# Fanchuana/OPUS-PLLM

Hardware: AMD Instinct MI355X
Metric: proteins_per_sec (higher is better)
Workload: dtype f16; 1 GPU; OPUS-PLLM-llama3_8b shape: batch 64/GPU, 512-residue proteins, 89-id prompt (+8 protein tokens = 96 positions), 32 new tokens, greedy (BASELINE configs[3] per-GPU shard: batch 512 over 8 GPUs); batch_per_gpu=64, residues=512, parallelism=replicas x1 (batch-sharded), all-gather of ids

## Files before the change

### include/opus_pllm.h

```cpp
#ifndef OPUS_PLLM_H
#define OPUS_PLLM_H

#include <stdint.h>

#ifdef __cplusplus
extern "C" {
#endif

#define OPUS_ABI_VERSION 10

enum opus_status {
    OPUS_OK = 0,
    OPUS_EBADARG = -1,
    OPUS_ESHAPE = -2,
    OPUS_EHIP = -3,
    OPUS_ERCCL = -4,
    OPUS_EUNSUPPORTED = -5,
    OPUS_ESTATE = -6
};

enum opus_dtype { OPUS_F16 = 0, OPUS_F32 = 1, OPUS_I32 = 2, OPUS_I64 = 3, OPUS_U8 = 4 };

typedef struct opus_config {
    int32_t enc_layers, enc_dim, enc_heads, enc_ffn, enc_vocab;
// ... 87 lines not shown
int opus_generate_greedy(opus_ctx *ctx, const void *d_embeds, const uint8_t *d_mask, int32_t B, int32_t T,
                         int32_t max_new, const int32_t *eos_ids, int32_t n_eos, int32_t pad_id,
                         int32_t *d_out_ids, int32_t *n_out, void *stream);

int opus_set_stop_sequence(opus_ctx *ctx, const int32_t *ids, int32_t n);

int opus_generate_sample(opus_ctx *ctx, const void *d_embeds, const uint8_t *d_mask, int32_t B, int32_t T,
                         int32_t max_new, const int32_t *eos_ids, int32_t n_eos, int32_t pad_id, float temperature,
                         float top_p, uint64_t seed, int32_t *d_out_ids, int32_t *n_out, void *stream);
int opus_debug_sample(opus_ctx *ctx, const float *d_logits, int32_t B, float temperature, float top_p, uint64_t seed,
                      int32_t step, int32_t *d_tokens, void *stream);

int opus_generate_scored(opus_ctx *ctx, const void *d_embeds, const uint8_t *d_mask, int32_t B, int32_t T, int32_t max_new,
                         const int32_t *eos_ids, int32_t n_eos, int32_t pad_id, float temperature, float top_p, uint64_t seed,
                         int32_t *d_out_ids, int32_t *n_out, float *d_token_logprobs, float *d_scores, float *d_logits,
                         void *stream);
int opus_debug_argmax_lse(opus_ctx *ctx, const float *d_logits, int32_t B, int32_t V, int32_t *d_idx, float *d_lse, void *stream);

int opus_set_logits_processors(opus_ctx *ctx, float repetition_penalty, int32_t no_repeat_ngram_size, int32_t min_new_tokens,
                               const int32_t *bad_ids, const int32_t *bad_offsets, int32_t n_bad);
int opus_debug_logits_process(opus_ctx *ctx, float *d_logits, int32_t B, int32_t V, const int32_t *d_hist, int32_t hist_stride,
                              int32_t hist_len, const int32_t *eos_ids, int32_t n_eos, float repetition_penalty,
                              int32_t no_repeat_ngram_size, int32_t min_new_tokens, const int32_t *bad_ids,
                              const int32_t *bad_offsets, int32_t n_bad, void *stream);

int opus_set_token_constraint(opus_ctx *ctx, int32_t n_states, const int32_t *edge_off, const int32_t *edge_tok,
                              const int32_t *edge_next, int32_t n_edges, const uint8_t *completing, const int32_t *end_ids,
                              int32_t n_end, const int32_t *start, int32_t n_start, void *stream);
int opus_debug_token_constraint(opus_ctx *ctx, float *d_logits, int32_t B, int32_t V, const int32_t *d_hist, int32_t hist_stride,
                                int32_t hist_len, int32_t *d_state_out, void *stream);

int opus_debug_gemm(opus_ctx *ctx, const void *d_A, const void *d_W, const float *d_bias, const float *d_residual,
                    void *d_C, int32_t M, int32_t N, int32_t K, int32_t epi, int32_t out_f32, void *stream);
int opus_debug_gemm_norm(opus_ctx *ctx, const float *d_A, const void *d_W, void *d_C, int32_t M, int32_t N, int32_t K,
                         int32_t epi, int32_t out_f32, float eps, void *stream);
int opus_debug_gemm_slabs(opus_ctx *ctx, const void *d_A, const void *d_W, float *d_slabs, int32_t M, int32_t N, int32_t K,
                          int32_t *ks, void *stream);
int opus_debug_knob(opus_ctx *ctx, const char *name, int32_t value);
int opus_debug_gemm_rowscale(opus_ctx *ctx, const void *d_A, const void *d_W1, float *d_X, const void *d_W2, void *d_C,
                             int32_t M, int32_t N1, int32_t K1, int32_t N2, int32_t epi, float eps, int32_t *fused,
                             void *stream);
int opus_debug_gemm_rope(opus_ctx *ctx, const void *d_A, const void *d_W, const float *d_bias, void *d_out, int32_t M,
                         int32_t D, int32_t K, int32_t T, int32_t heads, int32_t allow_fuse, int32_t *fused, void *stream);
int opus_debug_gemm_ln(opus_ctx *ctx, const void *d_A, const void *d_W1, const float *d_b1, float *d_X, float *d_part, void *d_xh,
                       float *d_stat, const void *d_W2, const float *d_c2, const float *d_colsum, void *d_C, int32_t M, int32_t N1,
                       int32_t K1, int32_t N2, int32_t epi, int32_t rms, float eps, int32_t rope_T, const int32_t *d_rope_pos,
                       int32_t *produced, int32_t *plan, void *stream);
int opus_debug_attention(opus_ctx *ctx, const void *d_Q, const void *d_K, const void *d_V, void *d_O,
                         const int32_t *d_kstart, const int32_t *d_kend, int32_t B, int32_t T, int32_t heads,
                         int32_t group, int32_t head_dim, int32_t causal, float scale, void *stream);

int opus_debug_attn_decode(opus_ctx *ctx, const void *d_qkv, const void *d_k_hist, const void *d_v_hist, const int32_t *d_kstart,
                           int32_t B, int32_t T0, int32_t step, void *d_out, void *d_k_new, void *d_v_new, void *stream);

int opus_check_error(opus_ctx *ctx, void *stream);

int opus_beam_topk(opus_ctx *ctx, const float *d_run_scores, int32_t B, int32_t K, int32_t M, float *d_scores, int32_t *d_idx,
                   void *stream);
int opus_kv_reorder(opus_ctx *ctx, const int32_t *d_src_rows, int32_t R, void *stream);
int opus_beam_sample_topk(opus_ctx *ctx, const float *d_logits, const float *d_run_scores, int32_t B, int32_t K, int32_t M,
                          float temperature, float top_p, uint64_t seed, int32_t step, float *d_scores, int32_t *d_idx, void *stream);
int opus_set_sampling_top_k(opus_ctx *ctx, int32_t k);

int opus_last_logits(opus_ctx *ctx, float *d_out, int32_t B, void *stream);

int64_t opus_stat(opus_ctx *ctx, const char *name);

int opus_timing_enable(opus_ctx *ctx, int32_t on);
int opus_timing_reset(opus_ctx *ctx);
int opus_timing_get(opus_ctx *ctx, const char *kernel_class, const char *phase, double *ms, int64_t *launches, double *bytes,
                    double *flops);
int opus_timing_names(char *buf, int32_t cap);

#ifdef __cplusplus
}
#endif
#endif
```

### opus-pllm_amd/_cabi.py

```python
from __future__ import annotations

import ctypes as C
import os
from typing import Optional

from .config import OpusConfig

_HERE = os.path.dirname(os.path.abspath(__file__))
BF16 = os.environ.get("OPUS_DTYPE", "fp16").lower() in ("bf16", "bfloat16")
LIB_PATH = os.environ.get("OPUS_LIB_PATH") or os.path.join(_HERE, "lib", "libopus_pllm_bf16.so" if BF16 else "libopus_pllm.so")
ABI_VERSION = 10

OPUS_F16, OPUS_F32, OPUS_I32, OPUS_I64, OPUS_U8 = 0, 1, 2, 3, 4


def operand_dtype():
    import torch
    return torch.bfloat16 if BF16 else torch.float16


class OpusError(RuntimeError):
    def __init__(self, code: int, msg: str):
        super().__init__(f"libopus_pllm error {code}: {msg}")
        self.code = code
# ... 19 lines not shown


_P = C.c_void_p
SIGNATURES = {
    "opus_abi_version": (C.c_int, []),
    "opus_operand_dtype": (C.c_int, []),
    "opus_last_error": (C.c_char_p, []),
    "opus_workspace_bytes": (C.c_int64, [C.POINTER(CConfig)]),
    "opus_ctx_create": (C.c_int, [C.POINTER(CConfig), C.c_int, C.POINTER(_P)]),
    "opus_ctx_destroy": (C.c_int, [_P]),
    "opus_bind_weight": (C.c_int, [_P, C.c_char_p, _P, C.c_int, C.c_int, C.POINTER(C.c_int64)]),
    "opus_weights_ready": (C.c_int, [_P]),
    "opus_lora_merge": (C.c_int, [_P, _P, _P, C.c_float, C.c_int64, C.c_int64, C.c_int32, _P]),
    "opus_fill_synth": (C.c_int, [_P, C.c_int, C.c_int64, C.c_int64, C.c_uint64, C.c_float, C.c_float,
                                  C.c_int64, C.c_int64, C.c_int64, C.c_int32, C.c_uint64, C.c_float, C.c_float, _P]),
    "opus_tile_weight": (C.c_int, [_P, _P, C.c_int64, C.c_int64, _P]),
    "opus_esm2_encode": (C.c_int, [_P, _P, _P, C.c_int32, C.c_int32, _P, _P]),
    "opus_esm2_encode_packed": (C.c_int, [_P, _P, C.POINTER(C.c_int32), C.c_int32, _P, _P]),
    "opus_esm2_last_hidden": (C.c_int, [_P, _P, C.c_int32, C.c_int32, _P]),
    "opus_projector_forward": (C.c_int, [_P, _P, C.c_int32, _P, _P, _P]),
    "opus_protein_projector": (C.c_int, [_P, _P, C.c_int32, _P, _P]),
    "opus_switch_projector": (C.c_int, [_P, _P, C.c_int32, _P, _P]),
    "opus_splice_pad": (C.c_int, [_P, _P, _P, C.c_int32, C.c_int32, _P, C.c_int32, C.c_int32, C.c_int32,
                                  _P, _P, _P, C.POINTER(C.c_int32), _P]),
    "opus_llama_prefill": (C.c_int, [_P, _P, _P, C.c_int32, C.c_int32, _P, _P]),
    "opus_llama_decode_step": (C.c_int, [_P, _P, _P, _P]),
    "opus_generate_greedy": (C.c_int, [_P, _P, _P, C.c_int32, C.c_int32, C.c_int32, C.POINTER(C.c_int32),
                                       C.c_int32, C.c_int32, _P, C.POINTER(C.c_int32), _P]),
    "opus_debug_gemm": (C.c_int, [_P, _P, _P, _P, _P, _P, C.c_int32, C.c_int32, C.c_int32, C.c_int32, C.c_int32, _P]),
    "opus_debug_gemm_norm": (C.c_int, [_P, _P, _P, _P, C.c_int32, C.c_int32, C.c_int32, C.c_int32, C.c_int32, C.c_float, _P]),
    "opus_debug_gemm_rope": (C.c_int, [_P, _P, _P, _P, _P, C.c_int32, C.c_int32, C.c_int32, C.c_int32, C.c_int32, C.c_int32, _P, _P]),
    "opus_debug_attention": (C.c_int, [_P, _P, _P, _P, _P, _P, _P, C.c_int32, C.c_int32, C.c_int32, C.c_int32,
                                       C.c_int32, C.c_int32, C.c_float, _P]),
    "opus_generate_sample": (C.c_int, [_P, _P, _P, C.c_int32, C.c_int32, C.c_int32, C.POINTER(C.c_int32), C.c_int32, C.c_int32,
                                       C.c_float, C.c_float, C.c_uint64, _P, C.POINTER(C.c_int32), _P]),
    "opus_debug_sample": (C.c_int, [_P, _P, C.c_int32, C.c_float, C.c_float, C.c_uint64, C.c_int32, _P, _P]),
    "opus_timing_enable": (C.c_int, [_P, C.c_int32]),
    "opus_timing_reset": (C.c_int, [_P]),
    "opus_timing_get": (C.c_int, [_P, C.c_char_p, C.c_char_p, C.POINTER(C.c_double), C.POINTER(C.c_int64),
                                  C.POINTER(C.c_double), C.POINTER(C.c_double)]),
    "opus_timing_names": (C.c_int, [C.c_char_p, C.c_int32]),
    "opus_last_logits": (C.c_int, [_P, _P, C.c_int32, _P]),
    "opus_check_error": (C.c_int, [_P, _P]),
    "opus_beam_topk": (C.c_int, [_P, _P, C.c_int32, C.c_int32, C.c_int32, _P, _P, _P]),
    "opus_kv_reorder": (C.c_int, [_P, _P, C.c_int32, _P]),
    "opus_beam_sample_topk": (C.c_int, [_P, _P, _P, C.c_int32, C.c_int32, C.c_int32, C.c_float, C.c_float, C.c_uint64, C.c_int32,
                                        _P, _P, _P]),
    "opus_set_sampling_top_k": (C.c_int, [_P, C.c_int32]),
    "opus_set_stop_sequence": (C.c_int, [_P, C.POINTER(C.c_int32), C.c_int32]),
    "opus_debug_gemm_slabs": (C.c_int, [_P, _P, _P, _P, C.c_int32, C.c_int32, C.c_int32, C.POINTER(C.c_int32), _P]),
    "opus_debug_knob": (C.c_int, [_P, C.c_char_p, C.c_int32]),
    "opus_stat": (C.c_int64, [_P, C.c_char_p]),
    "opus_debug_attn_decode": (C.c_int, [_P, _P, _P, _P, _P, C.c_int32, C.c_int32, C.c_int32, _P, _P, _P, _P]),
    "opus_llama_forward": (C.c_int, [_P, _P, _P, C.c_int32, C.c_int32, _P, C.c_int32, _P, _P, _P, _P, C.c_int64, _P]),
    "opus_llama_forward_scratch_bytes": (C.c_int64, [C.POINTER(CConfig), C.c_int32, C.c_int32]),
    "opus_llama_prefix": (C.c_int, [_P, _P, _P, C.c_int32, C.c_int32, _P, _P, C.POINTER(C.c_int64), _P]),
    "opus_llama_score_continuations": (C.c_int, [_P, _P, C.c_int32, C.c_int32, _P, _P, _P, C.c_int32, C.c_int64, _P, _P, _P,
                                                 C.c_int64, _P]),
    "opus_llama_score_scratch_bytes": (C.c_int64, [C.POINTER(CConfig), C.c_int32, C.c_int32]),
    "opus_debug_attn_prefix": (C.c_int, [_P, _P, _P, _P, _P, C.c_int32, C.c_int32, C.c_int32, C.c_int32, _P, _P, _P]),
    "opus_llama_score_tree": (C.c_int, [_P, _P, C.c_int32, _P, _P, _P, C.c_int32, _P, C.c_int32, _P, _P, _P, C.c_int32, _P, _P, _P,
                                        C.c_int32, _P, C.c_int32, _P, _P, C.c_int32, C.c_int64, _P, _P, C.c_int64, _P, C.c_int64, _P]),
    "opus_llama_score_tree_scratch_bytes": (C.c_int64, [C.POINTER(CConfig), C.c_int32, C.c_int32, C.c_int32, C.c_int32, C.c_int32,
                                                        C.c_int32]),
    "opus_llama_dec_rows_cap": (C.c_int64, [C.POINTER(CConfig)]),
    "opus_llama_tree_max_depth": (C.c_int32, []),
    "opus_trie_path_sums": (C.c_int, [_P, _P, _P, _P, _P, _P, C.c_int32, C.c_int32, C.c_int32, _P, _P]),
    "opus_debug_attn_tree": (C.c_int, [_P, _P, _P, _P, _P, C.c_int32, C.c_int32, C.c_int32, _P, _P, _P, _P, _P]),
    "opus_debug_xent": (C.c_int, [_P, _P, C.c_int32, C.c_int32, _P, _P, _P, _P]),
    "opus_esm2_contacts_packed": (C.c_int, [_P, _P, C.POINTER(C.c_int32), C.c_int32, _P, _P, _P, C.c_int64, _P]),
    "opus_esm2_contacts_scratch_bytes": (C.c_int64, [C.POINTER(CConfig), C.POINTER(C.c_int32), C.c_int32]),
    "opus_debug_contacts": (C.c_int, [_P, _P, _P, C.c_int64, C.POINTER(C.c_int32), C.c_int32, C.c_int32, C.c_int32, _P, _P, _P, _P,
                                      _P, C.c_int64, _P]),
    "opus_generate_scored": (C.c_int, [_P, _P, _P, C.c_int32, C.c_int32, C.c_int32, C.POINTER(C.c_int32), C.c_int32, C.c_int32,
                                       C.c_float, C.c_float, C.c_uint64, _P, C.POINTER(C.c_int32), _P, _P, _P, _P]),
    "opus_debug_argmax_lse": (C.c_int, [_P, _P, C.c_int32, C.c_int32, _P, _P, _P]),
    "opus_set_logits_processors": (C.c_int, [_P, C.c_float, C.c_int32, C.c_int32, C.POINTER(C.c_int32), C.POINTER(C.c_int32),
                                             C.c_int32]),
    "opus_debug_logits_process": (C.c_int, [_P, _P, C.c_int32, C.c_int32, _P, C.c_int32, C.c_int32, C.POINTER(C.c_int32), C.c_int32,
                                            C.c_float, C.c_int32, C.c_int32, C.POINTER(C.c_int32), C.POINTER(C.c_int32), C.c_int32,
                                            _P]),
    "opus_set_token_constraint": (C.c_int, [_P, C.c_int32, _P, _P, _P, C.c_int32, _P, _P, C.c_int32, _P, C.c_int32, _P]),
    "opus_debug_token_constraint": (C.c_int, [_P, _P, C.c_int32, C.c_int32, _P, C.c_int32, C.c_int32, _P, _P]),
    "opus_debug_gemm_rowscale": (C.c_int, [_P, _P, _P, _P, _P, _P, C.c_int32, C.c_int32, C.c_int32, C.c_int32, C.c_int32,
                                           C.c_float, C.POINTER(C.c_int32), _P]),
    "opus_debug_gemm_ln": (C.c_int, [_P, _P, _P, _P, _P, _P, _P, _P, _P, _P, _P, _P, C.c_int32, C.c_int32, C.c_int32, C.c_int32,
                                     C.c_int32, C.c_int32, C.c_float, C.c_int32, _P, C.POINTER(C.c_int32), C.POINTER(C.c_int32), _P]),
}

_lib: Optional[C.CDLL] = None


def lib() -> C.CDLL:
    global _lib
    if _lib is not None:
        return _lib
    if not os.path.exists(LIB_PATH):
        raise OpusError(-100, f"{LIB_PATH} not found: build it with `python opus-pllm_amd/build.py` "
                              "(hipcc --offload-arch=gfx950); this package has no CPU fallback")
    l = C.CDLL(LIB_PATH)
    for name, (res, args) in SIGNATURES.items():
        fn = getattr(l, name)
        fn.restype = res
        fn.argtypes = args
    v = l.opus_abi_version()
    if v != ABI_VERSION:
# ... 11 lines not shown
```

### opus-pllm_amd/csrc/api.cpp

```cpp
#include "../../include/opus_pllm.h"
#include "common.h"

#include <cmath>
#include <cstdarg>
#include <cstdio>
#include <cstdlib>
#include <cstring>
#include <algorithm>
#include <atomic>
#include <map>
#include <string>
#include <vector>

using namespace opus;

static thread_local char g_err[512] = "";
static int fail(int code, const char *fmt, ...) {
    va_list ap;
    va_start(ap, fmt);
    vsnprintf(g_err, sizeof(g_err), fmt, ap);
    va_end(ap);
    return code;
}
#define HIPC(expr)                                                                                   \
// ... 32 lines not shown
};

struct opus_ctx {
    opus_config cfg;
    int device = 0;
    std::map<std::string, Tensor> w;
    bool resolved = false;
    const half_t *enc_emb = nullptr, *dec_emb = nullptr, *lm_head = nullptr, *proj_w = nullptr, *dec_pos = nullptr;
    const float *enc_lnfw = nullptr, *enc_lnfb = nullptr, *proj_b = nullptr, *dec_lnfw = nullptr, *dec_lnfb = nullptr;
    std::vector<EncLayer> enc;
    std::vector<DecLayer> dec;
    std::vector<const half_t *> sw_w;
    std::vector<const float *> sw_b;
    char *ws = nullptr;
    size_t ws_bytes = 0;
    float *e_x, *e_hid, *p_pool_dummy, *e_part, *e_stat;
    int32_t *e_cu, *e_pos;
    std::vector<int32_t> h_cu;
    half_t *e_xn, *e_qkv, *e_ctx, *e_h1;
    half_t *p_xn, *p_y, *p_z[2];
    float *d_x, *d_xl, *d_logits, *d_pval, *gemm_ws, *d_probs, *d_zpart, *d_spart, *d_part, *d_stat;
    int32_t *d_cand_i, *d_cand_n;
    uint64_t *d_seed;
    int32_t *d_chosen;
    float samp_temp = 0.f, samp_top_p = 1.f;
    int samp_top_k = 0;
    float *d_bthr = nullptr, *d_blse = nullptr;
    int64_t gemm_ws_bytes = 0;
    half_t *d_xn, *d_qkv, *d_ctx, *d_act, *d_xln, *kc, *vc;
    float *cs_enc, *cs_dec, *cs_row;
    int32_t *d_kstart, *d_step, *d_next, *d_fin, *d_nunf, *d_eos, *d_plan, *d_pidx, *d_stop, *d_cnt;
    int n_stop = 0;
    static constexpr int POLL_RING = 4, POLL_LAG = 2;
    int32_t *h_nunf = nullptr;
    hipEvent_t poll_ev[POLL_RING] = {nullptr, nullptr, nullptr, nullptr};
    int64_t cache_sl, cache_sb, cache_sh;
    int cur_B = 0, cur_T = 0;
    bool prefilled = false;
    struct GraphEntry {
        hipGraphExec_t exec = nullptr;
        int B = -1, maxnew = -1, pad = 0, neos = -1;
        const int32_t *out = nullptr;
        float temp = 0.f, top_p = 1.f;
        int outs = 0;
        bool lproc = false;
        bool cons = false;
        uint64_t used = 0;
    };
    static constexpr int MAX_GRAPHS = 4;
    std::vector<GraphEntry> graphs;
    uint64_t graph_clock = 0;
    int64_t graph_instantiations = 0;
    int64_t graph_replays = 0;
    int64_t decode_steps = 0;
    char *gen_mem = nullptr;
    GenOutDesc *d_gen = nullptr;
    GenOutDesc h_gen{};
    float *d_gpsum = nullptr, *d_gthr = nullptr;
    int gen_outs = 0;
    bool lproc_on = false;
    LogitsProcDesc h_lproc{1.0f, 0, 0, 0, {}, {}};
    char *lproc_mem = nullptr;
    LogitsProcDesc *d_lproc = nullptr;
    int32_t *d_lstep = nullptr, *d_ridx = nullptr;
    GenOutDesc *d_gen_raw = nullptr, *d_gen_proc = nullptr;
    float *d_rlse = nullptr, *d_rawh = nullptr;
    bool cons_on = false;
    char *cons_tab = nullptr, *cons_mem = nullptr;
    size_t cons_tab_bytes = 0;
    TokenConstraintDesc *d_cons = nullptr;
    int32_t *d_cstate = nullptr, *d_cstep = nullptr;
    int32_t cons_n_start = 0, cons_max_id = -1;
    half_t *rq_xh = nullptr;
    int rq_done = 0;
    const float *rq_rope_cs = nullptr;
    const int32_t *rq_rope_pos = nullptr;
    int rq_rope_T = 0, rq_rope_cols = 0, rq_rope_qcols = 0, rq_rope_done = 0;
    float rq_rope_qscale = 1.0f;
    int rq_force_wide = 0, rq_slab_only = 0, rq_ks = 1;
    int rq_a_tiled = 0, rq_xh_tiled = 0, rq_c_tiled = 0;
    float *rq_ln_part = nullptr;
    half_t *rq_ln_xh = nullptr;
    int rq_ln_done = 0;
    const float *rq_ln_stat = nullptr, *rq_ln_colsum = nullptr;
    int *rq_pp_plan = nullptr;
    bool xln_tiled = false;
    const float *xh_src = nullptr;
    bool use_row_scale = false;
    float *d_ssq = nullptr;
    int64_t ssq_cap = 0;
    int ssq_nblk = 0;
    float row_eps = 0.f;
    bool timing = false;
    int phase = PH_OTHER;
    std::vector<TimeRec> recs;
    int proj_rows = 0;
    char *proj_big = nullptr;
    half_t *kv_tmp = nullptr;
    int64_t epoch = 0;
    std::vector<int32_t> h_kstart;
};

static std::atomic<int64_t> g_epoch{0};
static void new_epoch(opus_ctx *c) { c->epoch = ++g_epoch; }

struct ContRows {
    const int32_t *nkst;
    AttnPrefixParams attn;
    int nblocks;
};

static size_t align_up(size_t v) { return (v + 255) & ~(size_t)255; }

struct Carver {
    char *base;
    size_t off = 0;
    template <class T>
    T *take(size_t n) {
        T *p = base ? reinterpret_cast<T *>(base + off) : nullptr;
        off += align_up(n * sizeof(T));
        return p;
    }
};

static void carve(opus_ctx *c, char *base, size_t *total) {
    const opus_config &g = c->cfg;
    Carver k{base};
    const size_t Me = (size_t)g.max_batch * g.max_enc_tokens;
    const size_t De = g.enc_dim, Fe = g.enc_ffn;
    c->e_x = k.take<float>(Me * De);
    c->e_hid = k.take<float>(Me * De);
    c->e_xn = k.take<half_t>(Me * De);
    c->e_qkv = k.take<half_t>(Me * 3 * De);
    c->e_ctx = k.take<half_t>(Me * De);
    c->e_h1 = k.take<half_t>(Me * Fe);
    c->e_part = k.take<float>(Me * (De / 64 + 1) * 2);
    c->e_stat = k.take<float>(Me * 2);
    c->e_cu = k.take<int32_t>((size_t)g.max_batch + 4);
    c->e_pos = k.take<int32_t>(Me);
    const size_t B = g.max_batch, H = g.dec_dim, SW = (size_t)g.dec_dim * g.n_prot_tokens;
    const size_t PR = B;
    c->proj_rows = (int)PR;
    c->p_xn = k.take<half_t>(PR * De);
    c->p_y = k.take<half_t>(PR * (size_t)(g.has_protein_projector ? g.proj_dim : g.enc_dim));
    c->p_z[0] = k.take<half_t>(PR * SW);
    c->p_z[1] = k.take<half_t>(PR * SW);
    const size_t B16 = (B + 15) & ~(size_t)15;
    const size_t Md = B * g.max_prompt > B16 ? B * g.max_prompt : B16;
    const size_t QKV = (size_t)(g.dec_heads + 2 * g.dec_kv_heads) * g.dec_head_dim;
    const size_t QD = (size_t)g.dec_heads * g.dec_head_dim;
    c->d_x = k.take<float>(Md * H);
    c->d_xn = k.take<half_t>(Md * H);
    c->d_qkv = k.take<half_t>(Md * QKV);
    c->d_ctx = k.take<half_t>(Md * QD);
    c->d_act = k.take<half_t>(Md * g.dec_ffn);
    c->d_part = k.take<float>(Md * (H / 64 + 1) * 2);
    c->d_stat = k.take<float>(Md * 2);
// ... 270 lines not shown

struct Timed {
    opus_ctx *c;
    hipStream_t s;
    int klass;
    double bytes, flops;
    LaunchEvents ev;
    hipEvent_t b0 = nullptr, b1 = nullptr;
    Timed(opus_ctx *c_, hipStream_t s_, int k, double b, double f = 0.0) : c(c_), s(s_), klass(k), bytes(b), flops(f) {
        if (c->timing) {
            (void)hipEventCreate(&ev.main0); (void)hipEventCreate(&ev.main1);
            (void)hipEventCreate(&ev.aux0); (void)hipEventCreate(&ev.aux1);
            (void)hipEventCreate(&b0); (void)hipEventCreate(&b1);
            (void)hipEventRecord(b0, s);
            tl_launch_ev = &ev;
        }
    }
    ~Timed() {
        if (!c->timing) return;
        tl_launch_ev = nullptr;
        if (ev.main_used) {
            c->recs.push_back(TimeRec{ev.main_class >= 0 ? ev.main_class : klass, c->phase, ev.main0, ev.main1, bytes, flops});
            (void)hipEventDestroy(b0); (void)hipEventDestroy(b1);
        } else {
            (void)hipEventRecord(b1, s);
            c->recs.push_back(TimeRec{klass, c->phase, b0, b1, bytes, flops});
            (void)hipEventDestroy(ev.main0); (void)hipEventDestroy(ev.main1);
        }
        if (ev.aux_used) c->recs.push_back(TimeRec{KC_REDUCE, c->phase, ev.aux0, ev.aux1, ev.aux_bytes, 0.0});
        else { (void)hipEventDestroy(ev.aux0); (void)hipEventDestroy(ev.aux1); }
    }
};

static int gemm_any(opus_ctx *c, hipStream_t s, const half_t *A, const float *Af, float eps, int64_t lda, const half_t *W,
                    int M, int N, int K, const float *bias, int epi, const float *residual, void *C, int64_t ldc,
                    int out_f32) {
    GemmParams p;
    p.A = A; p.Af = Af; p.norm_eps = eps; p.lda = lda; p.W = W; p.M = M; p.N = N; p.K = K; p.bias = bias;
    p.residual = residual; p.ldr = ldc; p.C = C; p.ldc = ldc; p.out_f32 = out_f32; p.epi = epi;
    p.ws = c->gemm_ws; p.ws_bytes = c->gemm_ws_bytes;
    p.xh_out = c->rq_xh; p.ssq_out = c->d_ssq; p.fused_done = &c->rq_done; p.ssq_cap = c->ssq_cap; p.nblk_out = &c->ssq_nblk;
    c->rq_done = 0;
    c->rq_xh = nullptr;
    p.rope_cs = c->rq_rope_cs; p.rope_T = c->rq_rope_T; p.rope_cols = c->rq_rope_cols; p.rope_qcols = c->rq_rope_qcols;
    p.rope_qscale = c->rq_rope_qscale; p.rope_done = &c->rq_rope_done; p.rope_pos = c->rq_rope_pos;
    c->rq_rope_done = 0;
    c->rq_rope_cs = nullptr;
    c->rq_rope_pos = nullptr;
    p.row_ssq = nullptr; p.row_nblk = 0;
    if (c->use_row_scale) { p.row_ssq = c->d_ssq; p.row_nblk = c->ssq_nblk; p.norm_eps = c->row_eps; c->use_row_scale = false; }
    c->rq_ks = 1;
    p.force_wide = c->rq_force_wide; p.slab_only = c->rq_slab_only; p.ks_out = &c->rq_ks;
    c->rq_force_wide = c->rq_slab_only = 0;
    c->rq_ln_done = 0;
    if (c->rq_ln_part) { p.xh_out = c->rq_ln_xh; p.ssq_out = nullptr; p.ln_part = c->rq_ln_part; p.ln_done = &c->rq_ln_done; c->rq_ln_part = nullptr; }
    if (c->rq_ln_stat) { p.ln_stat = c->rq_ln_stat; p.ln_colsum = c->rq_ln_colsum; c->rq_ln_stat = c->rq_ln_colsum = nullptr; }
    p.combine_cnt = c->d_cnt;
    p.pp_plan = c->rq_pp_plan;
    c->rq_pp_plan = nullptr;
    p.a_tiled = c->rq_a_tiled; p.xh_tiled = c->rq_xh_tiled; p.c_tiled = c->rq_c_tiled;
    c->rq_a_tiled = c->rq_xh_tiled = c->rq_c_tiled = 0;
    const int nout = epi == EPI_SILU_GU16 ? N / 2 : N;
    const double bytes = 2.0 * N * K + (Af ? 4.0 : 2.0) * M * K + (double)M * nout * (out_f32 ? 4 : 2) +
                         (residual ? 4.0 * M * nout : 0.0);
    int klass = M <= SKINNY_MAX_M ? KC_SKINNY : KC_TILE;
    hipError_t e;
    {
        Timed t(c, s, klass, bytes, 2.0 * M * N * (double)K);
        e = launch_gemm(p, s, &klass);
    }
    if (e != hipSuccess) return fail(OPUS_EHIP, "gemm M=%d N=%d K=%d failed: %s", M, N, K, hipGetErrorString(e));
    return OPUS_OK;
}
static int gemm(opus_ctx *c, hipStream_t s, const half_t *A, int64_t lda, const half_t *W, int M, int N, int K,
                const float *bias, int epi, const float *residual, void *C, int64_t ldc, int out_f32) {
    return gemm_any(c, s, A, nullptr, 0.f, lda, W, M, N, K, bias, epi, residual, C, ldc, out_f32);
}
static bool fuse_rows() {
    static const bool off = getenv("OPUS_NO_ROW_FUSION") != nullptr;
    return !off;
}
#define KLF(klass, bytes, flops, call)                                                                \
    do {                                                                                              \
        hipError_t e_;                                                                                \
        {                                                                                             \
            Timed t_(c, s, klass, bytes, flops);                                                      \
            e_ = (call);                                                                              \
        }                                                                                             \
        if (e_ != hipSuccess) return fail(OPUS_EHIP, "%s failed: %s", #call, hipGetErrorString(e_)); \
    } while (0)
#define KL(klass, bytes, call) KLF(klass, bytes, 0.0, call)

static int gemm_norm(opus_ctx *c, hipStream_t s, const float *X, float eps, half_t *scratch, const half_t *W, int M, int N,
                     int K, int epi, void *C, int64_t ldc, int out_f32, const float *bias = nullptr) {
    static const bool no_mid = getenv("OPUS_NO_MID_GEMM") != nullptr;
    static const bool mid_v1 = getenv("OPUS_MID_V1") != nullptr;
    if (c->xh_src == X && bias == nullptr && (K & 255) == 0 && gemm_goes_wide(M, N)) {
        c->xh_src = nullptr;
        c->use_row_scale = true;
        c->row_eps = eps;
        return gemm(c, s, scratch, K, W, M, N, K, nullptr, epi, nullptr, C, ldc, out_f32);
    }
    c->xh_src = nullptr;
    const bool wide = M > SKINNY_MAX_M && N >= 16384 && !mid_v1;
    if (M <= SKINNY_MAX_M || (M <= MID_MAX_M && !no_mid && !wide))
        return gemm_any(c, s, nullptr, X, eps, K, W, M, N, K, bias, epi, nullptr, C, ldc, out_f32);
    KL(KC_NORM, 6.0 * M * K, launch_rmsnorm(X, nullptr, eps, M, K, scratch, s));
    return gemm(c, s, scratch, K, W, M, N, K, bias, epi, nullptr, C, ldc, out_f32);
}

static int need_ready(opus_ctx *c) {
    if (!c) return fail(OPUS_EBADARG, "ctx is null");
    OPC(opus_weights_ready(c));
    HIPC(hipSetDevice(c->device));
    return OPUS_OK;
}

extern "C" int opus_lora_merge(void *W, const void *A, const void *B, float scale, int64_t out_f, int64_t in_f,
                               int32_t r, void *stream) {
    if (!W || !A || !B || out_f < 1 || in_f < 1 || r < 1) return fail(OPUS_EBADARG, "lora_merge: bad argument");
    if (in_f % 8) return fail(OPUS_ESHAPE, "lora_merge: in_features must be a multiple of 8");
    HIPC(launch_lora_merge((half_t *)W, (const half_t *)A, (const half_t *)B, scale, out_f, in_f, r, (hipStream_t)stream));
    return OPUS_OK;
}

extern "C" int opus_fill_synth(void *dst, int dtype, int64_t rows, int64_t cols, uint64_t seed, float std, float mean,
                               int64_t row_block, int64_t row_stride, int64_t row_off, int32_t tiled, uint64_t fold_seed,
                               float fold_std, float fold_mean, void *stream) {
    if (!dst || rows < 1 || cols < 1 || (dtype != OPUS_F16 && dtype != OPUS_F32) || row_block < 1 || row_stride < row_block)
        return fail(OPUS_EBADARG, "fill_synth: bad argument");
    if (tiled && (cols % 64 || row_block % 16 || row_stride % 16 || row_off % 16))
        return fail(OPUS_ESHAPE, "fill_synth: tiled layout needs cols %% 64 == 0 and 16-row aligned blocks");
    HIPC(launch_fill_synth(dst, dtype, rows, cols, seed, std, mean, row_block, row_stride, row_off, tiled ? 1 : 0,
                           fold_seed, fold_std, fold_mean, (hipStream_t)stream));
    return OPUS_OK;
}

extern "C" int opus_tile_weight(const void *d_src, void *d_dst, int64_t N, int64_t K, void *stream) {
    if (!d_src || !d_dst || d_src == d_dst) return fail(OPUS_EBADARG, "tile_weight: null or aliased pointers");
    if (N < 16 || K < 64 || N % 16 || K % 64) return fail(OPUS_ESHAPE, "tile_weight: N %% 16 == 0 and K %% 64 == 0 required");
    HIPC(launch_tile_weight((const half_t *)d_src, (half_t *)d_dst, N, K, (hipStream_t)stream));
    return OPUS_OK;
}

struct ContactRun {
    const float *w, *bias;
    float *A, *vec, *part, *sw, *out;
    int n_max;
};

static int contact_layer(opus_ctx *c, hipStream_t s, const ContactRun &ct, int l, int B) {
    const opus_config &g = c->cfg;
    const int D = g.enc_dim, nh = g.enc_heads, hd = D / nh, C = g.enc_layers * nh;
    ContactParams p;
    p.Q = c->e_qkv; p.K = c->e_qkv + D; p.ld = 3 * D; p.cu = c->e_cu; p.B = B; p.heads = nh; p.w = ct.w + l * nh;
    p.A = ct.A; p.accumulate = l > 0; p.rows = ct.vec; p.vld = C; p.c0 = l * nh; p.part = ct.part;
    double n2 = 0.0, nt = 0.0;
    for (int b = 0; b < B; ++b) {
        const double n = c->h_cu[b + 1] - c->h_cu[b] - 2, t = n + 2;
        if (n > 0) { n2 += n * n; nt += n * t; }
    }
    KLF(KC_CONTACT, 8.0 * n2 + 4.0 * (c->h_cu[B]) * D, 2.0 * 2.0 * nt * hd * nh, launch_esm_contact_accum(p, hd, ct.n_max, s));
    KL(KC_CONTACT, 4.0 * n2 / 64.0 * nh * 2.0, launch_esm_contact_colsum(ct.part, c->e_cu, B, nh, ct.n_max, ct.vec, C, l * nh, 1, s));
    return OPUS_OK;
}

static int esm2_encode_rows(opus_ctx *c, hipStream_t s, const int32_t *d_tokens, const int32_t *d_lens, const int32_t *d_cu, int B, int T,
                            int M, float *d_pooled, const ContactRun *ct = nullptr) {
    const opus_config &g = c->cfg;
    c->phase = PH_ENCODE;
    const int D = g.enc_dim, F = g.enc_ffn, nh = g.enc_heads, hd = D / nh;
    const bool packed = d_cu != nullptr;
    HIPC(hipMemsetAsync(c->d_cnt, 0, HANDOFF_ERR * sizeof(int32_t), s));
    if (packed) KL(KC_OTHER, 4.0 * M * D, launch_esm_embed_packed(d_tokens, c->enc_emb, d_cu, B, T, D, c->e_x, c->e_pos, s));
    else KL(KC_OTHER, 4.0 * M * D, launch_esm_embed(d_tokens, c->enc_emb, B, T, D, c->e_x, s));
    static const bool no_ln_env = getenv("OPUS_NO_LN_FUSION") != nullptr;
    const bool no_ln_fusion = no_ln_env || g_knobs.no_ln_fusion;
    const bool qkv_pp = !no_ln_fusion && (D & 255) == 0 && gemm_goes_pp(M, 3 * D);
    const bool fc1_pp = !no_ln_fusion && (D & 255) == 0 && gemm_goes_pp(M, F);
    bool have_stat = false;
    auto finalize = [&]() -> int {
        KL(KC_NORM, 8.0 * M * (D / 64) + 8.0 * M, launch_ln_finalize(c->e_part, M, D / 64, D, g.enc_ln_eps, 0, c->e_stat, s));
        return OPUS_OK;
    };
    double attn_flops = 0.0;
    if (packed) for (int b = 0; b < B; ++b) { const double t = c->h_cu[b + 1] - c->h_cu[b]; attn_flops += 4.0 * t * t * D; }
    else attn_flops = 4.0 * B * (double)T * T * D;
    for (int l = 0; l < g.enc_layers; ++l) {
        const EncLayer &L = c->enc[l];
        if (have_stat && qkv_pp) { c->rq_ln_stat = c->e_stat; c->rq_ln_colsum = L.sqkv; }
        else KL(KC_NORM, 6.0 * M * D, launch_layernorm(c->e_x, nullptr, nullptr, g.enc_ln_eps, M, D, c->e_xn, nullptr, s));
        if (hd == 64) {
            c->rq_rope_cs = c->cs_enc; c->rq_rope_T = packed ? g.max_enc_tokens : T; c->rq_rope_cols = 2 * D; c->rq_rope_qcols = D;
            c->rq_rope_qscale = 1.0f / sqrtf((float)hd);
            c->rq_rope_pos = packed ? c->e_pos : nullptr;
        }
        OPC(gemm(c, s, c->e_xn, D, L.wqkv, M, 3 * D, D, L.bqkv, EPI_NONE, nullptr, c->e_qkv, 3 * D, 0));
        if (!c->rq_rope_done) {
            if (packed) KL(KC_OTHER, 8.0 * M * D, launch_esm_rope(c->e_qkv, c->cs_enc, 1, M, nh, hd, 1.0f / sqrtf((float)hd), s, c->e_pos));
            else KL(KC_OTHER, 8.0 * M * D, launch_esm_rope(c->e_qkv, c->cs_enc, B, T, nh, hd, 1.0f / sqrtf((float)hd), s));
        }
        if (ct) OPC(contact_layer(c, s, *ct, l, B));
        AttnParams a;
        a.Q = c->e_qkv; a.K = c->e_qkv + D; a.V = c->e_qkv + 2 * D;
        a.q_sb = a.k_sb = a.v_sb = packed ? 0 : (int64_t)T * 3 * D;
        a.q_st = a.k_st = a.v_st = 3 * D;
        a.O = c->e_ctx; a.o_sb = packed ? 0 : (int64_t)T * D; a.o_st = D;
        a.kstart = nullptr; a.kend = packed ? nullptr : d_lens; a.cu = d_cu;
        a.B = B; a.T = T; a.heads = nh; a.group = 1; a.head_dim = hd; a.causal = 0; a.scale = 1.0f;
        a.q_trim = packed && l + 1 == g.enc_layers && T > 2 && !g_knobs.enc_full_last_layer ? 1 : 0;
        KLF(KC_ATTN_PREFILL, 8.0 * M * D, attn_flops, launch_attn_prefill(a, s));
        if (fc1_pp) { c->rq_ln_part = c->e_part; c->rq_ln_xh = c->e_xn; }
        OPC(gemm(c, s, c->e_ctx, D, L.wo, M, D, D, L.bo, EPI_NONE, c->e_x, c->e_x, D, 1));
        have_stat = c->rq_ln_done != 0;
        if (have_stat) { OPC(finalize()); c->rq_ln_stat = c->e_stat; c->rq_ln_colsum = L.s1; }
        else KL(KC_NORM, 6.0 * M * D, launch_layernorm(c->e_x, nullptr, nullptr, g.enc_ln_eps, M, D, c->e_xn, nullptr, s));
        OPC(gemm(c, s, c->e_xn, D, L.w1, M, F, D, L.b1, EPI_GELU, nullptr, c->e_h1, F, 0));
        if (qkv_pp && l + 1 < g.enc_layers) { c->rq_ln_part = c->e_part; c->rq_ln_xh = c->e_xn; }
        OPC(gemm(c, s, c->e_h1, F, L.w2, M, D, F, L.b2, EPI_NONE, c->e_x, c->e_x, D, 1));
        have_stat = c->rq_ln_done != 0;
        if (have_stat) OPC(finalize());
    }
    KL(KC_NORM, 8.0 * M * D, launch_layernorm(c->e_x, c->enc_lnfw, c->enc_lnfb, g.enc_ln_eps, M, D, nullptr, c->e_hid, s));
    if (packed) KL(KC_OTHER, 4.0 * M * D, launch_masked_mean_packed(c->e_hid, d_cu, B, D, d_pooled, s));
    else KL(KC_OTHER, 4.0 * M * D, launch_masked_mean(c->e_hid, d_lens, B, T, D, d_pooled, s));
    if (ct) {
        const int C = g.enc_layers * nh;
        double n2 = 0.0, ni = 0.0;
        for (int b = 0; b < B; ++b) { const double n = c->h_cu[b + 1] - c->h_cu[b] - 2; n2 += n * n; ni += n; }
        KL(KC_CONTACT, 4.0 * ni * C, launch_esm_contact_scale(ct->vec, d_cu, B, C, ct->w, ct->sw, s));
        KLF(KC_CONTACT, 12.0 * n2 + 8.0 * ni * C * cdiv((int64_t)ct->n_max, 64), 2.0 * n2 * C,
            launch_esm_contact_finish(ct->A, ct->vec, ct->sw, d_cu, B, C, ct->n_max, ct->bias, ct->out, s));
    }
    return OPUS_OK;
}

extern "C" int opus_esm2_encode(opus_ctx *c, const int32_t *d_tokens, const int32_t *d_lens, int32_t B, int32_t T,
                                float *d_pooled, void *stream) {
    OPC(need_ready(c));
    if (!d_tokens || !d_lens || !d_pooled) return fail(OPUS_EBADARG, "esm2_encode: null pointer");
    const opus_config &g = c->cfg;
    if (B < 1 || B > g.max_batch || T < 3 || T > g.max_enc_tokens)
        return fail(OPUS_ESHAPE, "esm2_encode: B=%d T=%d exceed capacity (%d, %d)", B, T, g.max_batch, g.max_enc_tokens);
    return esm2_encode_rows(c, (hipStream_t)stream, d_tokens, d_lens, nullptr, B, T, B * T, d_pooled);
}

extern "C" int opus_esm2_encode_packed(opus_ctx *c, const int32_t *d_tokens, const int32_t *h_cu, int32_t B, float *d_pooled,
                                       void *stream) {
    OPC(need_ready(c));
    if (!d_tokens || !h_cu || !d_pooled) return fail(OPUS_EBADARG, "esm2_encode_packed: null pointer");
    const opus_config &g = c->cfg;
    if (B < 1 || B > g.max_batch) return fail(OPUS_ESHAPE, "esm2_encode_packed: B=%d exceeds max_batch=%d", B, g.max_batch);
    if (h_cu[0] != 0) return fail(OPUS_EBADARG, "esm2_encode_packed: cu[0] must be 0");
    int Tmax = 0;
    for (int b = 0; b < B; ++b) {
        const int t = h_cu[b + 1] - h_cu[b];
        if (t < 2 || t > g.max_enc_tokens)
            return fail(OPUS_ESHAPE, "esm2_encode_packed: protein %d has %d tokens (2 .. max_enc_tokens=%d)", b, t, g.max_enc_tokens);
        Tmax = t > Tmax ? t : Tmax;
    }
    const int64_t M = h_cu[B];
    if (M > (int64_t)g.max_batch * g.max_enc_tokens) return fail(OPUS_ESHAPE, "esm2_encode_packed: %lld tokens exceed the workspace", (long long)M);
    hipStream_t s = (hipStream_t)stream;
    c->h_cu.assign(h_cu, h_cu + B + 1);
    HIPC(launch_upload_i32(h_cu, B + 1, c->e_cu, s));
    return esm2_encode_rows(c, s, d_tokens, nullptr, c->e_cu, B, Tmax, (int)M, d_pooled);
}

struct ContactScratch {
    int64_t a, vec, part, sw, total;
    int n_max;
};
static ContactScratch contact_scratch(const opus_config &g, const int32_t *h_cu, int B) {
    ContactScratch z{};
// ... 65 lines not shown
    if (contact_accum_lds(heads) > 160 * 1024) return fail(OPUS_ESHAPE, "debug_contacts: %d heads exceed the workgroup's LDS", heads);
    if (h_cu[0] != 0) return fail(OPUS_EBADARG, "debug_contacts: cu[0] must be 0");
    int64_t pq = 0;
    int n_max = 0;
    for (int b = 0; b < B; ++b) {
        const int t = h_cu[b + 1] - h_cu[b];
        if (t < 2) return fail(OPUS_ESHAPE, "debug_contacts: protein %d has %d tokens (at least 2)", b, t);
        pq += (int64_t)(t - 2 + 63) / 64 * (t - 2);
        n_max = std::max(n_max, t - 2);
    }
    const int64_t need = (int64_t)align_up((size_t)(B + 1) * 4) + pq * heads * 4;
    if (scratch_bytes < need) return fail(OPUS_ESHAPE, "debug_contacts: scratch of %lld bytes, %lld needed", (long long)scratch_bytes, (long long)need);
    HIPC(hipSetDevice(c->device));
    hipStream_t s = (hipStream_t)stream;
    int32_t *d_cu = (int32_t *)d_scratch;
    float *part = (float *)((char *)d_scratch + align_up((size_t)(B + 1) * 4));
    HIPC(launch_upload_i32(h_cu, B + 1, d_cu, s));
    ContactParams p;
    p.Q = (const half_t *)d_q; p.K = (const half_t *)d_k; p.ld = ld; p.cu = d_cu; p.B = B; p.heads = heads; p.w = d_w;
    p.A = d_A; p.accumulate = 0; p.rows = d_rows; p.vld = heads; p.c0 = 0; p.part = part;
    HIPC(launch_esm_contact_accum(p, head_dim, n_max, s));
    HIPC(launch_esm_contact_colsum(part, d_cu, B, heads, n_max, d_cols, heads, 0, 0, s));
    return OPUS_OK;
}

extern "C" int opus_esm2_last_hidden(opus_ctx *c, float *d_out, int32_t B, int32_t T, void *stream) {
    if (!c || !d_out) return fail(OPUS_EBADARG, "null pointer");
    if (B < 1 || T < 1 || (int64_t)B * T > (int64_t)c->cfg.max_batch * c->cfg.max_enc_tokens) return fail(OPUS_ESHAPE, "B/T out of range");
    HIPC(hipMemcpyAsync(d_out, c->e_hid, (size_t)B * T * c->cfg.enc_dim * sizeof(float), hipMemcpyDeviceToDevice,
                        (hipStream_t)stream));
    return OPUS_OK;
}

constexpr int BIG_PROJ_ROWS = 4096;
static int ensure_proj_rows(opus_ctx *c, int B) {
    if (B <= c->proj_rows || c->proj_big) return OPUS_OK;
    const opus_config &g = c->cfg;
    const size_t PR = BIG_PROJ_ROWS > g.max_batch ? BIG_PROJ_ROWS : g.max_batch;
    const size_t De = g.enc_dim, Dm = g.has_protein_projector ? g.proj_dim : g.enc_dim, SW = (size_t)g.dec_dim * g.n_prot_tokens;
    const size_t bytes = (align_up(PR * De * 2) + align_up(PR * Dm * 2) + 2 * align_up(PR * SW * 2));
    HIPC(hipMalloc((void **)&c->proj_big, bytes));
    Carver k{c->proj_big};
    c->p_xn = k.take<half_t>(PR * De);
    c->p_y = k.take<half_t>(PR * Dm);
    c->p_z[0] = k.take<half_t>(PR * SW);
    c->p_z[1] = k.take<half_t>(PR * SW);
    c->proj_rows = (int)PR;
    return OPUS_OK;
}

static int protein_projector_rows(opus_ctx *c, hipStream_t s, const float *d_pooled, int B, half_t *d_out) {
    const opus_config &g = c->cfg;
    const int De = g.enc_dim;
    HIPC(hipMemsetAsync(c->d_cnt, 0, HANDOFF_ERR * sizeof(int32_t), s));
    if (!g.has_protein_projector) {
        KL(KC_OTHER, 6.0 * B * De, launch_f2h(d_pooled, (int64_t)B * De, d_out, s));
        return OPUS_OK;
    }
    KL(KC_NORM, 6.0 * B * De, launch_l2norm(d_pooled, B, De, c->p_xn, s));
    return gemm(c, s, c->p_xn, De, c->proj_w, B, g.proj_dim, De, c->proj_b, EPI_NONE, nullptr, d_out, g.proj_dim, 0);
}

static int switch_projector_rows(opus_ctx *c, hipStream_t s, const half_t *in, int B, half_t *d_out) {
    const opus_config &g = c->cfg;
    const int SW = g.dec_dim * g.n_prot_tokens;
    int din = g.has_protein_projector ? g.proj_dim : g.enc_dim;
    for (int i = 0; i < g.switch_depth; ++i) {
        const bool last = i + 1 == g.switch_depth;
        half_t *o = last ? d_out : c->p_z[i & 1];
        OPC(gemm(c, s, in, din, c->sw_w[i], B, SW, din, c->sw_b[i], last ? EPI_NONE : EPI_GELU, nullptr, o, SW, 0));
        in = o;
        din = SW;
    }
    return OPUS_OK;
}

extern "C" int opus_protein_projector(opus_ctx *c, const float *d_pooled, int32_t B, void *d_out, void *stream) {
    OPC(need_ready(c));
    if (!d_pooled || !d_out) return fail(OPUS_EBADARG, "protein_projector: null pointer");
    if (B < 1) return fail(OPUS_ESHAPE, "protein_projector: B=%d", B);
    const opus_config &g = c->cfg;
    const int64_t din = g.enc_dim, dout = g.has_protein_projector ? g.proj_dim : g.enc_dim;
    c->phase = PH_PROJECT;
    OPC(ensure_proj_rows(c, B));
    for (int r0 = 0; r0 < B; r0 += c->proj_rows) {
        const int n = B - r0 < c->proj_rows ? B - r0 : c->proj_rows;
        OPC(protein_projector_rows(c, (hipStream_t)stream, d_pooled + r0 * din, n, (half_t *)d_out + r0 * dout));
    }
    return OPUS_OK;
}

extern "C" int opus_switch_projector(opus_ctx *c, const void *d_in, int32_t B, void *d_out, void *stream) {
    OPC(need_ready(c));
    if (!d_in || !d_out) return fail(OPUS_EBADARG, "switch_projector: null pointer");
    if (B < 1) return fail(OPUS_ESHAPE, "switch_projector: B=%d", B);
    const opus_config &g = c->cfg;
    const int64_t din = g.has_protein_projector ? g.proj_dim : g.enc_dim, SW = (int64_t)g.dec_dim * g.n_prot_tokens;
    c->phase = PH_PROJECT;
    OPC(ensure_proj_rows(c, B));
    for (int r0 = 0; r0 < B; r0 += c->proj_rows) {
        const int n = B - r0 < c->proj_rows ? B - r0 : c->proj_rows;
        OPC(switch_projector_rows(c, (hipStream_t)stream, (const half_t *)d_in + r0 * din, n, (half_t *)d_out + r0 * SW));
    }
    return OPUS_OK;
}

extern "C" int opus_projector_forward(opus_ctx *c, const float *d_pooled, int32_t B, void *d_out, void *d_proj_out,
// ... 82 lines not shown
        4.0 * M * (double)QD * (a.Tp + a.n), a.par ? launch_attn_tree(a, cr.nblocks, s) : launch_attn_prefix(a, cr.nblocks, s));
    return OPUS_OK;
}

static int opt_layer(opus_ctx *c, hipStream_t s, const DecLayer &L, int l, float *x, half_t *xn, int M, int B, int T, bool decode,
                     const ContRows *cont = nullptr) {
    const opus_config &g = c->cfg;
    const int H = g.dec_dim, F = g.dec_ffn, nh = g.dec_heads, nkv = g.dec_kv_heads, hd = g.dec_head_dim;
    const int QKV = (nh + 2 * nkv) * hd, QD = nh * hd;
    KL(KC_NORM, 6.0 * M * H, launch_layernorm(x, L.ln1w, L.ln1b, g.dec_rms_eps, M, H, xn, nullptr, s));
    OPC(gemm(c, s, xn, H, L.wqkv, M, QKV, H, L.bqkv, EPI_NONE, nullptr, c->d_qkv, QKV, 0));
    if (decode) {
        OPC(attn_decode(c, s, l, B, T));
    } else if (cont) {
        KL(KC_OTHER, 4.0 * M * QKV, launch_dec_rope_cache(c->d_qkv, c->cs_dec, cont->nkst, B, T, nh, nkv, hd, nullptr, nullptr, 0, 0, s));
        OPC(attn_prefix(c, s, *cont, l, M));
    } else {
        KL(KC_OTHER, 4.0 * M * QKV,
           launch_dec_rope_cache(c->d_qkv, c->cs_dec, c->d_kstart, B, T, nh, nkv, hd, c->kc + l * c->cache_sl,
                                 c->vc + l * c->cache_sl, c->cache_sb, c->cache_sh, s));
        AttnParams a;
        a.Q = c->d_qkv; a.K = c->d_qkv + QD; a.V = c->d_qkv + QD + nkv * hd;
        a.q_sb = a.k_sb = a.v_sb = (int64_t)T * QKV;
        a.q_st = a.k_st = a.v_st = QKV;
        a.O = c->d_ctx; a.o_sb = (int64_t)T * QD; a.o_st = QD;
        a.kstart = c->d_kstart; a.kend = nullptr;
        a.B = B; a.T = T; a.heads = nh; a.group = nh / nkv; a.head_dim = hd; a.causal = 1;
        a.scale = 1.0f / sqrtf((float)hd);
        KLF(KC_ATTN_PREFILL, 2.0 * M * (QKV + QD), 2.0 * B * (double)T * T * QD, launch_attn_prefill(a, s));
    }
    OPC(gemm(c, s, c->d_ctx, QD, L.wo, M, H, QD, L.bo, EPI_NONE, x, x, H, 1));
    KL(KC_NORM, 6.0 * M * H, launch_layernorm(x, L.ln2w, L.ln2b, g.dec_rms_eps, M, H, xn, nullptr, s));
    if (g.dec_act == 0) {
        OPC(gemm(c, s, xn, H, L.w1, M, F, H, L.b1, EPI_GELU, nullptr, c->d_act, F, 0));
    } else {
        OPC(gemm(c, s, xn, H, L.w1, M, F, H, L.b1, EPI_NONE, nullptr, c->d_act, F, 0));
        KL(KC_OTHER, 4.0 * M * F, launch_relu_h(c->d_act, (int64_t)M * F, s));
    }
    OPC(gemm(c, s, c->d_act, F, L.w2, M, H, F, L.b2, EPI_NONE, x, x, H, 1));
    return OPUS_OK;
}

static int lm_head_opt(opus_ctx *c, hipStream_t s, int B) {
    const opus_config &g = c->cfg;
    KL(KC_NORM, 6.0 * B * g.dec_dim, launch_layernorm(c->d_xl, c->dec_lnfw, c->dec_lnfb, g.dec_rms_eps, B, g.dec_dim, c->d_xln, nullptr, s));
    return gemm(c, s, c->d_xln, g.dec_dim, c->lm_head, B, g.dec_vocab, g.dec_dim, nullptr, EPI_NONE, nullptr, c->d_logits,
                g.dec_vocab, 1);
}

static int prefill_opt(opus_ctx *c, hipStream_t s, const half_t *embeds, const uint8_t *mask, int B, int T, bool all_rows,
                       const ContRows *cont) {
    const opus_config &g = c->cfg;
    const int H = g.dec_dim, M = B * T;
    HIPC(hipMemsetAsync(c->d_cnt, 0, HANDOFF_ERR * sizeof(int32_t), s));
    if (!cont) KL(KC_OTHER, 1.0 * M, launch_mask_to_kstart(mask, B, T, c->d_kstart, s));
    KL(KC_OTHER, 6.0 * M * H, launch_h2f(embeds, c->d_x, (int64_t)M * H, s));
    KL(KC_OTHER, 10.0 * M * H, launch_add_pos(c->d_x, c->dec_pos, cont ? cont->nkst : c->d_kstart, nullptr, 0, B, T, H, g.dec_max_pos + 1, s));
    for (int l = 0; l < g.dec_layers; ++l) OPC(opt_layer(c, s, c->dec[l], l, c->d_x, c->d_xn, M, B, T, false, cont));
    if (all_rows) return OPUS_OK;
    KL(KC_OTHER, 8.0 * B * H, launch_take_last(c->d_x, B, T, H, c->d_xl, s));
    OPC(lm_head_opt(c, s, B));
    OPC(reset_step(c, s, T));
    c->cur_B = B;
    c->cur_T = T;
    c->prefilled = true;
    return OPUS_OK;
}

static int decode_step_opt(opus_ctx *c, hipStream_t s) {
    const opus_config &g = c->cfg;
    const int B = c->cur_B, T = c->cur_T, H = g.dec_dim;
    KL(KC_OTHER, 10.0 * B * H, launch_add_pos(c->d_xl, c->dec_pos, c->d_kstart, c->d_step, -1, B, 1, H, g.dec_max_pos + 1, s));
    for (int l = 0; l < g.dec_layers; ++l) OPC(opt_layer(c, s, c->dec[l], l, c->d_xl, c->d_xln, B, B, T, true));
    OPC(lm_head_opt(c, s, B));
    KL(KC_OTHER, 8.0, launch_step_advance(c->d_step, s));
    return OPUS_OK;
}

static int prefill(opus_ctx *c, hipStream_t s, const half_t *embeds, const uint8_t *mask, int B, int T, bool all_rows = false,
                   const ContRows *cont = nullptr) {
    c->phase = cont ? PH_SCORE : PH_PREFILL;
    if (cont) {
        all_rows = true;
    } else {
        new_epoch(c);
        if (all_rows) {
            c->prefilled = false;
            c->cur_B = 0;
        }
    }
    if (c->cfg.dec_arch == 1) return prefill_opt(c, s, embeds, mask, B, T, all_rows, cont);
    const opus_config &g = c->cfg;
    const int H = g.dec_dim, F = g.dec_ffn, nh = g.dec_heads, nkv = g.dec_kv_heads, hd = g.dec_head_dim;
    const int QKV = (nh + 2 * nkv) * hd, QD = nh * hd;
    const int M = B * T;
    HIPC(hipMemsetAsync(c->d_cnt, 0, HANDOFF_ERR * sizeof(int32_t), s));
    if (!cont) KL(KC_OTHER, 1.0 * M, launch_mask_to_kstart(mask, B, T, c->d_kstart, s));
    KL(KC_OTHER, 6.0 * M * H, launch_h2f(embeds, c->d_x, (int64_t)M * H, s));
    static const bool no_ln_env = getenv("OPUS_NO_LN_FUSION") != nullptr;
    const bool no_ln_fusion = no_ln_env || g_knobs.no_ln_fusion;
    const bool qkv_pp = !no_ln_fusion && (H & 255) == 0 && (QKV & 255) == 0 && gemm_goes_pp(M, QKV);
    const bool gu_pp = !no_ln_fusion && (H & 255) == 0 && (F & 127) == 0 && gemm_goes_pp(M, 2 * F);
    bool have_stat = false, last_rows_done = false;
    auto finalize = [&]() -> int {
        KL(KC_NORM, 8.0 * M * (H / 64) + 8.0 * M, launch_ln_finalize(c->d_part, M, H / 64, H, g.dec_rms_eps, 1, c->d_stat, s));
        return OPUS_OK;
    };
    for (int l = 0; l < g.dec_layers; ++l) {
        const DecLayer &L = c->dec[l];
        if (have_stat && qkv_pp) {
            c->rq_ln_stat = c->d_stat;
            OPC(gemm(c, s, c->d_xn, H, L.wqkv, M, QKV, H, L.bqkv, EPI_NONE, nullptr, c->d_qkv, QKV, 0));
        } else {
            OPC(gemm_norm(c, s, c->d_x, g.dec_rms_eps, c->d_xn, L.wqkv, M, QKV, H, EPI_NONE, c->d_qkv, QKV, 0, L.bqkv));
        }
        if (cont) {
            KL(KC_OTHER, 4.0 * M * QKV, launch_dec_rope_cache(c->d_qkv, c->cs_dec, cont->nkst, B, T, nh, nkv, hd, nullptr, nullptr, 0, 0, s));
            OPC(attn_prefix(c, s, *cont, l, M));
        } else {
            KL(KC_OTHER, 4.0 * M * QKV,
               launch_dec_rope_cache(c->d_qkv, c->cs_dec, c->d_kstart, B, T, nh, nkv, hd, c->kc + l * c->cache_sl,
                                     c->vc + l * c->cache_sl, c->cache_sb, c->cache_sh, s));
            AttnParams a;
            a.Q = c->d_qkv; a.K = c->d_qkv + QD; a.V = c->d_qkv + QD + nkv * hd;
            a.q_sb = a.k_sb = a.v_sb = (int64_t)T * QKV;
            a.q_st = a.k_st = a.v_st = QKV;
            a.O = c->d_ctx; a.o_sb = (int64_t)T * QD; a.o_st = QD;
            a.kstart = c->d_kstart; a.kend = nullptr;
            a.B = B; a.T = T; a.heads = nh; a.group = nh / nkv; a.head_dim = hd; a.causal = 1;
            a.scale = 1.0f / sqrtf((float)hd);
            KLF(KC_ATTN_PREFILL, 2.0 * M * (QKV + QD), 2.0 * B * (double)T * T * QD, launch_attn_prefill(a, s));
        }
        if (l + 1 == g.dec_layers && T > 1 && !all_rows && !g_knobs.misc[7]) {
            half_t *ctx_last = c->d_qkv;
            KL(KC_OTHER, 4.0 * B * QD, launch_take_last(reinterpret_cast<const float *>(c->d_ctx), B, T, QD / 2, reinterpret_cast<float *>(ctx_last), s));
            KL(KC_OTHER, 8.0 * B * H, launch_take_last(c->d_x, B, T, H, c->d_xl, s));
            if (fuse_rows() && B <= 96) c->rq_xh = c->d_xln;
            OPC(gemm(c, s, ctx_last, QD, L.wo, B, H, QD, nullptr, EPI_NONE, c->d_xl, c->d_xl, H, 1));
            c->xh_src = c->rq_done ? c->d_xl : nullptr;
            OPC(gemm_norm(c, s, c->d_xl, g.dec_rms_eps, c->d_xln, L.wgu, B, 2 * F, H, EPI_SILU_GU16, c->d_act, F, 0));
            if (fuse_rows() && B <= 96) c->rq_xh = c->d_xln;
            OPC(gemm(c, s, c->d_act, F, L.wd, B, H, F, nullptr, EPI_NONE, c->d_xl, c->d_xl, H, 1));
            c->xh_src = c->rq_done ? c->d_xl : nullptr;
            c->xln_tiled = false;
            last_rows_done = true;
            break;
        }
        if (gu_pp) { c->rq_ln_part = c->d_part; c->rq_ln_xh = c->d_xn; }
        else if (fuse_rows() && M <= 96) c->rq_xh = c->d_xn;
        OPC(gemm(c, s, c->d_ctx, QD, L.wo, M, H, QD, nullptr, EPI_NONE, c->d_x, c->d_x, H, 1));
        c->xh_src = c->rq_done ? c->d_x : nullptr;
        have_stat = c->rq_ln_done != 0;
        if (have_stat) {
            OPC(finalize());
            c->rq_ln_stat = c->d_stat;
            OPC(gemm(c, s, c->d_xn, H, L.wgu, M, 2 * F, H, nullptr, EPI_SILU_GU16, nullptr, c->d_act, F, 0));
        } else {
            OPC(gemm_norm(c, s, c->d_x, g.dec_rms_eps, c->d_xn, L.wgu, M, 2 * F, H, EPI_SILU_GU16, c->d_act, F, 0));
        }
        if (qkv_pp && l + 1 < g.dec_layers) { c->rq_ln_part = c->d_part; c->rq_ln_xh = c->d_xn; }
        OPC(gemm(c, s, c->d_act, F, L.wd, M, H, F, nullptr, EPI_NONE, c->d_x, c->d_x, H, 1));
        have_stat = c->rq_ln_done != 0;
        if (have_stat) OPC(finalize());
    }
    if (all_rows) {
        c->xh_src = nullptr;
        return OPUS_OK;
    }
    if (!last_rows_done) {
        KL(KC_OTHER, 8.0 * B * H, launch_take_last(c->d_x, B, T, H, c->d_xl, s));
        c->xh_src = nullptr;
    }
    OPC(lm_head(c, s, B));
    OPC(reset_step(c, s, T));
    c->cur_B = B;
    c->cur_T = T;
    c->prefilled = true;
    return OPUS_OK;
}

static int decode_step(opus_ctx *c, hipStream_t s, const int32_t *d_tok) {
    c->phase = PH_DECODE;
    const opus_config &g = c->cfg;
    const int B = c->cur_B, T = c->cur_T;
    const int H = g.dec_dim, F = g.dec_ffn, nh = g.dec_heads, nkv = g.dec_kv_heads, hd = g.dec_head_dim;
    const int QKV = (nh + 2 * nkv) * hd, QD = nh * hd;
    const int ctx_cap = g.max_prompt + g.max_new_tokens;
    const bool rowscale = g.dec_arch == 0 && fuse_rows() && B > SKINNY_MAX_M && B <= MID_MAX_M && (H & 255) == 0;
    const bool qkv_tiled = rowscale && gemm_stream_would(B, QKV, H, 1, 1, 1, c->gemm_ws_bytes);
    const bool wo_tiled = rowscale && gemm_stream_would(B, H, QD, 0, 1, 0, c->gemm_ws_bytes);
    const bool down_tiled = rowscale && (F & 63) == 0 && gemm_stream_would(B, H, F, 0, 1, 0, c->gemm_ws_bytes);
    KL(KC_OTHER, 6.0 * B * H, launch_embed_tokens(d_tok, c->dec_emb, B, H, g.dec_vocab, c->d_xl, rowscale ? c->d_xln : nullptr,
                                                  rowscale ? c->d_ssq : nullptr, qkv_tiled ? 1 : 0, c->cs_dec, c->d_kstart, c->d_step, -1,
                                                  hd / 2, c->cs_row, c->d_cnt, HANDOFF_ERR, s));
    c->xln_tiled = qkv_tiled;
    c->xh_src = rowscale ? c->d_xl : nullptr;
    if (rowscale) c->ssq_nblk = H >> 8;
    if (g.dec_arch == 1) return decode_step_opt(c, s);
    for (int l = 0; l < g.dec_layers; ++l) {
        const DecLayer &L = c->dec[l];
        if (rowscale && c->xh_src == c->d_xl) {
            c->xh_src = nullptr;
            c->rq_force_wide = 1;
            c->rq_slab_only = 1;
            c->use_row_scale = true;
            c->row_eps = g.dec_rms_eps;
            c->rq_a_tiled = c->xln_tiled ? 1 : 0;
            OPC(gemm(c, s, c->d_xln, H, L.wqkv, B, QKV, H, L.bqkv, EPI_NONE, nullptr, c->d_qkv, QKV, 0));
            OPC(attn_decode(c, s, l, B, T, c->rq_ks > 1 ? c->rq_ks : 0, L.bqkv, wo_tiled ? 1 : 0));
        } else {
            OPC(gemm_norm(c, s, c->d_xl, g.dec_rms_eps, c->d_xln, L.wqkv, B, QKV, H, EPI_NONE, c->d_qkv, QKV, 0, L.bqkv));
            OPC(attn_decode(c, s, l, B, T, 0, nullptr, wo_tiled ? 1 : 0));
        }
        c->xln_tiled = false;
        if (fuse_rows() && B <= 96) c->rq_xh = c->d_xln;
        c->rq_a_tiled = wo_tiled ? 1 : 0;
// ... 1019 lines not shown
    if (M < 1 || D < 16 || K < 64 || K % 64 || T < 1 || heads < 1 || D % heads || M % T)
        return fail(OPUS_ESHAPE, "debug_gemm_rope: M %% T == 0, D %% heads == 0, K %% 64 == 0");
    const int hd = D / heads;
    if (hd != c->cfg.enc_dim / c->cfg.enc_heads || T > c->cfg.max_enc_tokens)
        return fail(OPUS_ESHAPE, "debug_gemm_rope: head_dim / T must match the context's encoder rotary table");
    HIPC(hipSetDevice(c->device));
    hipStream_t s = (hipStream_t)stream;
    const float qs = 1.0f / sqrtf((float)hd);
    if (allow_fuse && hd == 64) {
        c->rq_rope_cs = c->cs_enc; c->rq_rope_T = T; c->rq_rope_cols = 2 * D; c->rq_rope_qcols = D; c->rq_rope_qscale = qs;
    }
    OPC(gemm(c, s, (const half_t *)A, K, (const half_t *)W, M, 3 * D, K, bias, EPI_NONE, nullptr, out, 3 * D, 0));
    *fused = c->rq_rope_done;
    if (!c->rq_rope_done) HIPC(launch_esm_rope((half_t *)out, c->cs_enc, M / T, T, heads, hd, qs, s));
    return OPUS_OK;
}

extern "C" int opus_debug_gemm_rowscale(opus_ctx *c, const void *A, const void *W1, float *X, const void *W2, void *Cp, int32_t M,
                                        int32_t N1, int32_t K1, int32_t N2, int32_t epi, float eps, int32_t *fused, void *stream) {
    if (!c || !A || !W1 || !X || !W2 || !Cp || !fused) return fail(OPUS_EBADARG, "debug_gemm_rowscale: null pointer");
    if (M < 1 || N1 < 64 || N1 % 64 || K1 < 64 || K1 % 64 || N2 < 32) return fail(OPUS_ESHAPE, "debug_gemm_rowscale: shape");
    if (epi != EPI_NONE && epi != EPI_SILU_GU16) return fail(OPUS_EBADARG, "debug_gemm_rowscale: epilogue 0 or 2");
    const opus_config &g = c->cfg;
    if ((int64_t)M * N1 > (int64_t)g.max_batch * g.max_prompt * g.dec_dim) return fail(OPUS_ESHAPE, "debug_gemm_rowscale: M * N1 exceeds the scratch");
    HIPC(hipSetDevice(c->device));
    hipStream_t s = (hipStream_t)stream;
    if (fuse_rows() && M <= 96) c->rq_xh = c->d_xn;
    OPC(gemm(c, s, (const half_t *)A, K1, (const half_t *)W1, M, N1, K1, nullptr, EPI_NONE, X, X, N1, 1));
    c->xh_src = c->rq_done ? X : nullptr;
    *fused = c->xh_src != nullptr && (N1 & 255) == 0 && gemm_goes_wide(M, N2) ? 1 : 0;
    const int nout = epi == EPI_SILU_GU16 ? N2 / 2 : N2;
    return gemm_norm(c, s, X, eps, c->d_xn, (const half_t *)W2, M, N2, N1, epi, Cp, nout, 0);
}

extern "C" int opus_debug_gemm_ln(opus_ctx *c, const void *A, const void *W1, const float *b1, float *X, float *part, void *xh,
                                  float *stat, const void *W2, const float *c2, const float *colsum, void *Cp, int32_t M, int32_t N1,
                                  int32_t K1, int32_t N2, int32_t epi, int32_t rms, float eps, int32_t rope_T,
                                  const int32_t *rope_pos, int32_t *produced, int32_t *plan, void *stream) {
    if (!c || !A || !W1 || !X || !part || !xh || !stat || !W2 || !Cp || !produced || !plan)
        return fail(OPUS_EBADARG, "debug_gemm_ln: null pointer");
    if (M < 1 || N1 < 64 || N1 % 64 || K1 < 64 || K1 % 64 || N2 < 32) return fail(OPUS_ESHAPE, "debug_gemm_ln: shape");
    if (epi != EPI_NONE && epi != EPI_GELU && epi != EPI_SILU_GU16) return fail(OPUS_EBADARG, "debug_gemm_ln: epilogue 0, 1 or 2");
    if (epi == EPI_SILU_GU16 && (!rms || c2 || colsum || N2 % 32))
        return fail(OPUS_EBADARG, "debug_gemm_ln: the gate / up epilogue is the RMSNorm form (no bias, no column sums)");
    if (rms ? colsum != nullptr : colsum == nullptr) return fail(OPUS_EBADARG, "debug_gemm_ln: column sums go with LayerNorm only");
    if (rope_pos && rope_T < 1) return fail(OPUS_EBADARG, "debug_gemm_ln: rope_pos needs rope_T");
    if (rope_T > 0 && (epi != EPI_NONE || N2 % 3 || (N2 / 3) % 64 || c->cfg.enc_dim / c->cfg.enc_heads != 64 ||
                       rope_T > c->cfg.max_enc_tokens))
        return fail(OPUS_ESHAPE, "debug_gemm_ln: rotary needs EPI_NONE, N2 = 3 D, head_dim 64 and rope_T within the context's table");
    HIPC(hipSetDevice(c->device));
    hipStream_t s = (hipStream_t)stream;
    c->phase = PH_OTHER;
    for (int i = 0; i < 2 * PP_PLAN_WORDS; ++i) plan[i] = -1;
    HIPC(hipMemsetAsync(c->d_cnt, 0, HANDOFF_ERR * sizeof(int32_t), s));
    if (gemm_goes_pp(M, N1)) { c->rq_ln_part = part; c->rq_ln_xh = (half_t *)xh; }
    c->rq_pp_plan = plan;
    OPC(gemm(c, s, (const half_t *)A, K1, (const half_t *)W1, M, N1, K1, b1, EPI_NONE, X, X, N1, 1));
    *produced = c->rq_ln_done;
    if (!c->rq_ln_done) return OPUS_OK;
    KL(KC_NORM, 8.0 * M * (N1 / 64), launch_ln_finalize(part, M, N1 / 64, N1, eps, rms, stat, s));
    c->rq_ln_stat = stat; c->rq_ln_colsum = colsum;
    c->rq_pp_plan = plan + PP_PLAN_WORDS;
    if (rope_T > 0) {
        const int D = N2 / 3;
        c->rq_rope_cs = c->cs_enc; c->rq_rope_T = rope_T; c->rq_rope_cols = 2 * D; c->rq_rope_qcols = D;
        c->rq_rope_qscale = 0.125f;
        c->rq_rope_pos = rope_pos;
    }
    const int nout = epi == EPI_SILU_GU16 ? N2 / 2 : N2;
    OPC(gemm(c, s, (const half_t *)xh, N1, (const half_t *)W2, M, N2, N1, c2, epi, nullptr, Cp, nout, 0));
    if (rope_T > 0 && !c->rq_rope_done) return fail(OPUS_ESTATE, "debug_gemm_ln: the consumer GEMM did not fuse the rotary");
    return OPUS_OK;
}

extern "C" int opus_debug_gemm_slabs(opus_ctx *c, const void *A, const void *W, float *d_slabs, int32_t M, int32_t N, int32_t K,
                                     int32_t *ks, void *stream) {
    if (!c || !A || !W || !ks) return fail(OPUS_EBADARG, "debug_gemm_slabs: null pointer");
    if (M < 1 || N < 16 || K < 64 || K % 64) return fail(OPUS_ESHAPE, "debug_gemm_slabs: shape");
    const opus_config &g = c->cfg;
    const int64_t QKVd = (int64_t)(g.dec_heads + 2 * g.dec_kv_heads) * g.dec_head_dim;
    if ((int64_t)M * N > (int64_t)g.max_batch * g.max_prompt * QKVd) return fail(OPUS_ESHAPE, "debug_gemm_slabs: M * N exceeds the scratch");
    HIPC(hipSetDevice(c->device));
    hipStream_t s = (hipStream_t)stream;
    c->rq_force_wide = 1;
    c->rq_slab_only = 1;
    c->rq_a_tiled = g_knobs.debug_a_tiled;
    OPC(gemm(c, s, (const half_t *)A, K, (const half_t *)W, M, N, K, nullptr, EPI_NONE, nullptr, c->d_qkv, N, 0));
    *ks = c->rq_ks;
    if (c->rq_ks > 1 && d_slabs)
        HIPC(hipMemcpyAsync(d_slabs, c->gemm_ws, (size_t)c->rq_ks * M * N * sizeof(float), hipMemcpyDeviceToDevice, s));
    return OPUS_OK;
}

extern "C" int opus_beam_topk(opus_ctx *c, const float *d_run_scores, int32_t B, int32_t K, int32_t M, float *d_scores,
                              int32_t *d_idx, void *stream) {
    if (!c || !d_run_scores || !d_scores || !d_idx) return fail(OPUS_EBADARG, "beam_topk: null pointer");
    if (!c->prefilled) return fail(OPUS_ESTATE, "beam_topk before prefill");
    if (B < 1 || K < 1 || B * K != c->cur_B) return fail(OPUS_ESHAPE, "beam_topk: B=%d x K=%d rows, the last step had %d", B, K, c->cur_B);
    if (M < 1 || M > 16) return fail(OPUS_ESHAPE, "beam_topk: 1 <= M <= 16 candidates per row (got %d)", M);
    HIPC(hipSetDevice(c->device));
    hipStream_t s = (hipStream_t)stream;
    c->phase = PH_DECODE;
    KL(KC_OTHER, 12.0 * c->cur_B * c->cfg.dec_vocab,
       launch_beam_topk(c->d_logits, d_run_scores, B, K, c->cfg.dec_vocab, M, c->d_zpart, d_scores, d_idx, s));
    return OPUS_OK;
}

extern "C" int opus_beam_sample_topk(opus_ctx *c, const float *d_logits, const float *d_run_scores, int32_t B, int32_t K, int32_t M,
                                     float temperature, float top_p, uint64_t seed, int32_t step, float *d_scores, int32_t *d_idx,
                                     void *stream) {
    if (!c || !d_run_scores || !d_scores || !d_idx) return fail(OPUS_EBADARG, "beam_sample_topk: null pointer");
    if (!d_logits && !c->prefilled) return fail(OPUS_ESTATE, "beam_sample_topk before prefill");
    if (B < 1 || K < 1 || B * K > c->cfg.max_batch || (!d_logits && B * K != c->cur_B))
// ... 58 lines not shown
                                    int32_t group, int32_t hd, int32_t causal, float scale, void *stream) {
    if (!c || !Q || !K || !V || !O) return fail(OPUS_EBADARG, "debug_attention: null pointer");
    if (B < 1 || T < 1 || heads < 1 || group < 1 || heads % group) return fail(OPUS_ESHAPE, "debug_attention: shape");
    HIPC(hipSetDevice(c->device));
    hipStream_t s = (hipStream_t)stream;
    AttnParams a;
    const int kvh = heads / group;
    a.Q = (const half_t *)Q; a.K = (const half_t *)K; a.V = (const half_t *)V; a.O = (half_t *)O;
    a.q_st = (int64_t)heads * hd; a.q_sb = a.q_st * T;
    a.k_st = a.v_st = (int64_t)kvh * hd; a.k_sb = a.v_sb = a.k_st * T;
    a.o_st = a.q_st; a.o_sb = a.q_sb;
    a.kstart = kstart; a.kend = kend; a.B = B; a.T = T; a.heads = heads; a.group = group; a.head_dim = hd;
    a.causal = causal; a.scale = scale;
    KLF(KC_ATTN_PREFILL, 2.0 * B * T * hd * (2.0 * heads + 2.0 * kvh), (causal ? 2.0 : 4.0) * B * (double)T * T * heads * hd,
        launch_attn_prefill(a, s));
    return OPUS_OK;
}

extern "C" int opus_debug_attn_decode(opus_ctx *c, const void *d_qkv, const void *d_k_hist, const void *d_v_hist,
                                      const int32_t *d_kstart, int32_t B, int32_t T0, int32_t step, void *d_out, void *d_k_new,
                                      void *d_v_new, void *stream) {
    if (!c || !d_qkv || !d_kstart || !d_out) return fail(OPUS_EBADARG, "debug_attn_decode: null pointer");
    const opus_config &g = c->cfg;
    const int L = T0 + step, nkv = g.dec_kv_heads, hd = g.dec_head_dim;
    if (B < 1 || B > g.max_batch || T0 < 1 || T0 > g.max_prompt || step < 0 || step >= g.max_new_tokens)
        return fail(OPUS_ESHAPE, "debug_attn_decode: B=%d T0=%d step=%d exceed the context (%d, %d, %d)", B, T0, step, g.max_batch,
                    g.max_prompt, g.max_new_tokens);
    if (L > 0 && (!d_k_hist || !d_v_hist)) return fail(OPUS_EBADARG, "debug_attn_decode: history is null");
    HIPC(hipSetDevice(c->device));
    hipStream_t s = (hipStream_t)stream;
    const size_t pitch = (size_t)c->cache_sh * sizeof(half_t), roww = (size_t)L * hd * sizeof(half_t);
    HIPC(hipMemcpy2DAsync(c->kc, pitch, d_k_hist, roww, roww, (size_t)B * nkv, hipMemcpyDeviceToDevice, s));
    HIPC(hipMemcpy2DAsync(c->vc, pitch, d_v_hist, roww, roww, (size_t)B * nkv, hipMemcpyDeviceToDevice, s));
    HIPC(hipMemcpyAsync(c->d_kstart, d_kstart, (size_t)B * sizeof(int32_t), hipMemcpyDeviceToDevice, s));
    OPC(reset_step(c, s, T0, step));
    HIPC(launch_embed_tokens(c->d_next, nullptr, B, 0, 1, c->d_xl, nullptr, nullptr, 0, c->cs_dec, c->d_kstart, c->d_step, -1, hd / 2,
                             c->cs_row, nullptr, 0, s));
    AttnDecodeParams a;
    a.qkv = (const half_t *)d_qkv; a.slabs = nullptr; a.ks = 0; a.slab_stride = 0; a.row_ssq = nullptr; a.row_nblk = 0; a.eps = 0.f; a.K = 0;
    a.bias = nullptr;
    a.cs_row = c->cs_row; a.kstart = c->d_kstart; a.step = c->d_step; a.T0 = -1; a.nh = g.dec_heads; a.nkv = nkv;
    a.kc = c->kc; a.vc = c->vc; a.cache_sb = c->cache_sb; a.cache_sh = c->cache_sh;
    a.ctx_cap = g.max_prompt + g.max_new_tokens; a.scale = 1.0f / sqrtf((float)hd); a.out = (half_t *)d_out; a.out_tiled = 0;
    c->phase = PH_DECODE;
    KL(KC_ATTN_DECODE, 4.0 * B * nkv * hd * (L + 1), launch_attn_decode(a, B, hd, s));
    const size_t one = (size_t)hd * sizeof(half_t);
    if (d_k_new) HIPC(hipMemcpy2DAsync(d_k_new, one, c->kc + (size_t)L * hd, pitch, one, (size_t)B * nkv, hipMemcpyDeviceToDevice, s));
    if (d_v_new) HIPC(hipMemcpy2DAsync(d_v_new, one, c->vc + (size_t)L * hd, pitch, one, (size_t)B * nkv, hipMemcpyDeviceToDevice, s));
    c->prefilled = false;
    new_epoch(c);
    return OPUS_OK;
}

extern "C" int opus_debug_knob(opus_ctx *c, const char *name, int32_t value) {
    if (!name) return fail(OPUS_EBADARG, "debug_knob: null name");
    if (c) drop_graphs(c);
    if (!strcmp(name, "no_stream")) g_knobs.no_stream = value;
    else if (!strcmp(name, "debug_a_tiled")) g_knobs.debug_a_tiled = value;
    else if (!strcmp(name, "no_ln_fusion")) g_knobs.no_ln_fusion = value;
    else if (!strcmp(name, "enc_full_last_layer")) g_knobs.enc_full_last_layer = value;
    else if (!strcmp(name, "poison_handoff")) {
        if (!c) return fail(OPUS_EBADARG, "poison_handoff needs a context");
        std::vector<int32_t> h(HANDOFF_ERR, 0);
        if (value) for (int i = 0; i < HANDOFF_ERR; ++i) h[i] = i < 512 ? value : ((i & 1) ? 0 : 1);
        HIPC(hipSetDevice(c->device));
        HIPC(hipDeviceSynchronize());
        HIPC(hipMemcpy(c->d_cnt, h.data(), h.size() * sizeof(int32_t), hipMemcpyHostToDevice));
    }
    else if (!strcmp(name, "pp_gm")) { if (value < 1 || value > 64) return fail(OPUS_EBADARG, "pp_gm out of range"); g_knobs.pp_gm = value; }
    else if (!strncmp(name, "misc", 4) && name[4] >= '0' && name[4] <= '7' && !name[5]) g_knobs.misc[name[4] - '0'] = value;
    else return fail(OPUS_EBADARG, "debug_knob: unknown knob '%s'", name);
    return OPUS_OK;
}

extern "C" int64_t opus_stat(opus_ctx *c, const char *name) {
    if (!c || !name) return -1;
    if (!strcmp(name, "graph_instantiations")) return c->graph_instantiations;
    if (!strcmp(name, "graph_replays")) return c->graph_replays;
    if (!strcmp(name, "graphs_cached")) return (int64_t)c->graphs.size();
    if (!strcmp(name, "decode_steps")) return c->decode_steps;
    return -1;
}

extern "C" int opus_timing_enable(opus_ctx *c, int32_t on) {
    if (!c) return fail(OPUS_EBADARG, "ctx is null");
    c->timing = on != 0;
    return OPUS_OK;
}
extern "C" int opus_timing_reset(opus_ctx *c) {
    if (!c) return fail(OPUS_EBADARG, "ctx is null");
    HIPC(hipDeviceSynchronize());
    timing_clear(c);
    return OPUS_OK;
}
static const char *kclass_names[KC_COUNT] = {"gemm_skinny", "gemm_mid", "gemm_wide", "gemm_ring", "gemm_pp", "gemm_tile", "splitk_reduce",
                                            "attn_prefill", "attn_decode", "norm", "other", "gemm_stream", "contact", "constraint", "logitproc",
                                            "xent"};
static const char *phase_names[PH_COUNT] = {"encode", "project", "splice", "prefill", "decode", "other", "score"};

extern "C" int opus_timing_get(opus_ctx *c, const char *kernel_class, const char *phase, double *ms, int64_t *launches,
                               double *bytes, double *flops) {
    if (!c || !kernel_class || !phase || !ms || !launches || !bytes || !flops) return fail(OPUS_EBADARG, "null argument");
    int k = -1, ph = -1;
    const bool any_k = !strcmp(kernel_class, "*"), any_p = !strcmp(phase, "*");
    for (int i = 0; i < KC_COUNT; ++i) if (!strcmp(kclass_names[i], kernel_class)) k = i;
    for (int i = 0; i < PH_COUNT; ++i) if (!strcmp(phase_names[i], phase)) ph = i;
    if (k < 0 && !any_k) return fail(OPUS_EBADARG, "unknown kernel class '%s'", kernel_class);
    if (ph < 0 && !any_p) return fail(OPUS_EBADARG, "unknown phase '%s'", phase);
    HIPC(hipDeviceSynchronize());
    double t = 0, b = 0, f = 0;
    int64_t n = 0;
    for (auto &r : c->recs) {
        if ((!any_k && r.klass != k) || (!any_p && r.phase != ph)) continue;
        float e = 0;
        HIPC(hipEventElapsedTime(&e, r.e0, r.e1));
        t += e;
        b += r.bytes;
        f += r.flops;
        ++n;
    }
    *ms = t;
    *launches = n;
    *bytes = b;
    *flops = f;
    return OPUS_OK;
}

extern "C" int opus_timing_names(char *buf, int32_t cap) {
    if (!buf || cap < 1) return fail(OPUS_EBADARG, "null buffer");
    std::string out;
    for (int i = 0; i < KC_COUNT; ++i) { out += kclass_names[i]; out += i + 1 < KC_COUNT ? "," : ";"; }
    for (int i = 0; i < PH_COUNT; ++i) { out += phase_names[i]; if (i + 1 < PH_COUNT) out += ","; }
    if ((int)out.size() + 1 > cap) return fail(OPUS_ESHAPE, "buffer too small (%zu needed)", out.size() + 1);
// ... 4 lines not shown
```

### opus-pllm_amd/csrc/attn_prefill.hip

```cpp
#include "common.h"
#include <type_traits>

namespace opus {

constexpr int KB = 64;

template <int HDP>
__device__ __forceinline__ int kswz(int row, int chunk) {
    if (HDP == 128) return chunk ^ (row & 15);
    if (HDP == 64) return chunk ^ ((row >> 1) & 7);
    return chunk;
}
template <int HD>
__device__ __forceinline__ int vswz(int row) {
    if (HD == 128) return (row & 7) << 1;
    if (HD == 64) return ((row >> 1) & 3) << 1;
    if (HD == 32) return ((row >> 2) & 1) << 1;
    return 0;
}

typedef float f2 __attribute__((ext_vector_type(2)));
__device__ __forceinline__ float max3(float a, float b, float c) {
    float r;
    asm("v_max3_f32 %0, %1, %2, %3" : "=v"(r) : "v"(a), "v"(b), "v"(c));
    return r;
}
__device__ __forceinline__ float xor16_max(float x) {
    float a = x, b = x, r;
    asm volatile("s_nop 1\n\tv_permlane16_swap_b32 %0, %1" : "+v"(a), "+v"(b));
    asm("v_max_f32 %0, %1, %2" : "=v"(r) : "v"(a), "v"(b));
    return r;
}
__device__ __forceinline__ void xor32_pair(float x, float &a, float &b) {
    a = x;
    b = x;
    asm volatile("s_nop 1\n\tv_permlane32_swap_b32 %0, %1" : "+v"(a), "+v"(b));
}

typedef short s4v __attribute__((ext_vector_type(4)));
typedef short s8v __attribute__((ext_vector_type(8)));

template <int HD, bool CAUSAL, int QT>
__global__ __launch_bounds__(256) void attn_prefill_kernel(AttnParams p) {
    constexpr int QW = 16 * QT, QB = 4 * QW;
    constexpr int HDP = HD < 32 ? 32 : HD;
    constexpr int KS = HDP / 32;
    constexpr int NO = HD / 16;
    constexpr int CH = HDP / 8;
    constexpr int VC = HD / 8;
    __shared__ __attribute__((aligned(16))) half_t sK[2][KB * HDP];
    __shared__ __attribute__((aligned(16))) half_t sV[2][KB * HD];

    const int tid = threadIdx.x, lane = tid & 63;
    const int wave = __builtin_amdgcn_readfirstlane(tid >> 6);
    const int g = lane >> 4, li = lane & 15;
    const int qtrim = (p.q_trim && p.cu) ? 1 : 0;
    const int nqb = (p.T - 2 * qtrim + QB - 1) / QB;
    const int id = blockIdx.x, slot = id >> 3;
    const int bh = (slot / nqb) * 8 + (id & 7);
    if (bh >= p.B * p.heads) return;
    const int b = bh / p.heads, h = bh % p.heads, hk = h / p.group;
    const int q0 = (slot % nqb) * QB + qtrim, qw = q0 + wave * QW;
    int T = p.T, Tq = p.T;
    int64_t qb_off = (int64_t)b * p.q_sb, kb_off = (int64_t)b * p.k_sb, vb_off = (int64_t)b * p.v_sb, ob_off = (int64_t)b * p.o_sb;
    if (p.cu) {
        const int r0 = p.cu[b];
        T = p.cu[b + 1] - r0;
        Tq = T - qtrim;
        if (q0 >= Tq) return;
        qb_off = (int64_t)r0 * p.q_st; kb_off = (int64_t)r0 * p.k_st; vb_off = (int64_t)r0 * p.v_st; ob_off = (int64_t)r0 * p.o_st;
    }
    const int kstart = (p.kstart && !p.cu) ? p.kstart[b] : 0;
    const int kend = (p.kend && !p.cu) ? p.kend[b] : T;

    const half_t *Qb = p.Q + qb_off + (int64_t)h * HD;
    const half_t *Kb = p.K + kb_off + (int64_t)hk * HD;
    const half_t *Vb = p.V + vb_off + (int64_t)hk * HD;

    h8 qf[QT][KS];
#pragma unroll
    for (int t = 0; t < QT; ++t) {
        int qr = qw + 16 * t + li;
        qr = qr < Tq ? qr : Tq - 1;
        const half_t *src = Qb + (int64_t)qr * p.q_st;
#pragma unroll
        for (int s = 0; s < KS; ++s) {
            const int d = 32 * s + 8 * g;
            qf[t][s] = d < HD ? *reinterpret_cast<const h8 *>(src + d) : h8{0, 0, 0, 0, 0, 0, 0, 0};
        }
    }
    f4 o[QT][NO];
    float mrow[QT], lrow[QT];
#pragma unroll
    for (int t = 0; t < QT; ++t) {
        mrow[t] = -INFINITY;
        lrow[t] = 0.f;
#pragma unroll
        for (int n = 0; n < NO; ++n) o[t][n] = f4{0.f, 0.f, 0.f, 0.f};
    }

    int k_lo = kstart / KB * KB;
    int k_hi = kend;
    if (CAUSAL) {
        const int last_q = (q0 + QB - 1 < T - 1 ? q0 + QB - 1 : T - 1);
        k_hi = k_hi < last_q + 1 ? k_hi : last_q + 1;
    }
    const float sc = p.scale * 1.4426950408889634f;
    const bool wave_live = qw < Tq;

    constexpr int KL = KB * CH / 256;
    constexpr int VN = KB * VC;
    constexpr int VL = VN >= 256 ? VN / 256 : 1;
    static_assert(KL >= 1, "tile too small for 256 threads");
    h8 kreg[KL], vreg[VL];
    const __amdgpu_buffer_rsrc_t krs = __builtin_amdgcn_make_buffer_rsrc((void *)Kb, 0, (int)(((int64_t)(T - 1) * p.k_st + HD) * 2), 0x00020000);
    const __amdgpu_buffer_rsrc_t vrs = __builtin_amdgcn_make_buffer_rsrc((void *)Vb, 0, (int)(((int64_t)(T - 1) * p.v_st + HD) * 2), 0x00020000);
    int koff[KL], voff[VL];
#pragma unroll
    for (int u = 0; u < KL; ++u) {
        const int i = tid + 256 * u, r = i / CH, c = i % CH;
        koff[u] = c * 8 < HD ? (int)((r * p.k_st + c * 8) * 2) : 0x7ffffff0;
    }
#pragma unroll
    for (int u = 0; u < VL; ++u) {
        const int i = tid + 256 * u, r = i / VC, c = i % VC;
        voff[u] = i < VN ? (int)((r * p.v_st + c * 8) * 2) : 0x7ffffff0;
    }
    auto load_tile = [&](int kt) {
        const int kb = kt * (int)p.k_st * 2, vb = kt * (int)p.v_st * 2;
#pragma unroll
        for (int u = 0; u < KL; ++u) kreg[u] = __builtin_bit_cast(h8, __builtin_amdgcn_raw_buffer_load_b128(krs, koff[u] + kb, 0, 0));
#pragma unroll
        for (int u = 0; u < VL; ++u) vreg[u] = __builtin_bit_cast(h8, __builtin_amdgcn_raw_buffer_load_b128(vrs, voff[u] + vb, 0, 0));
    };
    auto store_tile = [&](int buf) {
#pragma unroll
        for (int u = 0; u < KL; ++u) {
            const int i = tid + 256 * u, r = i / CH, c = i % CH;
            *reinterpret_cast<h8 *>(&sK[buf][r * HDP + kswz<HDP>(r, c) * 8]) = kreg[u];
        }
#pragma unroll
        for (int u = 0; u < VL; ++u) {
            const int i = tid + 256 * u, r = i / VC, c = i % VC;
            if (i < VN) *reinterpret_cast<h8 *>(&sV[buf][r * HD + (c ^ vswz<HD>(r)) * 8]) = vreg[u];
        }
    };

    if (k_lo < k_hi) {
        load_tile(k_lo);
        store_tile(0);
        if (k_lo + KB < k_hi) load_tile(k_lo + KB);
    }
    __syncthreads();
    auto tile_body = [&](auto nsub_tag, int kt, int buf) {
        {
            constexpr int NSUB = decltype(nsub_tag)::value, NJ = (NSUB + 1) / 2;
            const half_t *tK = sK[buf], *tV = sV[buf];
            f4 s[QT][4];
#pragma unroll
            for (int n = 0; n < NSUB; ++n) {
                const int r = 16 * n + li;
                h8 kf[KS];
#pragma unroll
                for (int ks = 0; ks < KS; ++ks) kf[ks] = *reinterpret_cast<const h8 *>(tK + r * HDP + kswz<HDP>(r, 4 * ks + g) * 8);
#pragma unroll
                for (int t = 0; t < QT; ++t) {
                    s[t][n] = f4{0.f, 0.f, 0.f, 0.f};
#pragma unroll
                    for (int ks = 0; ks < KS; ++ks) s[t][n] = mfma16(kf[ks], qf[t][ks], s[t][n]);
                }
            }
            const bool interior = kt >= kstart && kt + KB <= kend && (!CAUSAL || kt + KB - 1 <= qw);
            if (__builtin_expect(!interior, 0)) {
#pragma unroll
                for (int t = 0; t < QT; ++t) {
                    const int qi = qw + 16 * t + li;
#pragma unroll
                    for (int n = 0; n < NSUB; ++n)
#pragma unroll
                        for (int r = 0; r < 4; ++r) {
                            const int kj = kt + 16 * n + 4 * g + r;
                            bool vis = kj >= kstart && kj < kend;
                            if (CAUSAL) vis = vis && kj <= qi;
                            s[t][n][r] = vis ? s[t][n][r] : -INFINITY;
                        }
                }
            }
            h8 pf[QT][2];
#pragma unroll
            for (int t = 0; t < QT; ++t) {
                float mx = fmaxf(fmaxf(s[t][0][0], s[t][0][1]), fmaxf(s[t][0][2], s[t][0][3]));
#pragma unroll
                for (int n = 1; n < NSUB; ++n) mx = fmaxf(fmaxf(mx, fmaxf(s[t][n][0], s[t][n][1])), fmaxf(s[t][n][2], s[t][n][3]));
                float ma, mb;
                mx = xor16_max(mx);
                xor32_pair(mx, ma, mb);
                const float mnew = max3(mrow[t], ma, mb);
                const float msafe = mnew == -INFINITY ? 0.f : mnew;
                const float msc = msafe * sc;
                if (!__all(mnew == mrow[t])) {
                    const float alpha = __builtin_amdgcn_exp2f((mrow[t] - msafe) * sc);
                    lrow[t] *= alpha;
#pragma unroll
                    for (int n = 0; n < NO; ++n) o[t][n] *= alpha;
                    mrow[t] = mnew;
                }
                const f2 sc2 = f2{sc, sc}, msc2 = f2{msc, msc};
                f2 rs2 = f2{0.f, 0.f};
#pragma unroll
                for (int n = 0; n < NSUB; ++n)
#pragma unroll
                    for (int r = 0; r < 4; r += 2) {
                        const f2 a = f2{s[t][n][r], s[t][n][r + 1]} * sc2 - msc2;
                        const f2 e = f2{__builtin_amdgcn_exp2f(a[0]), __builtin_amdgcn_exp2f(a[1])};
                        s[t][n][r] = e[0];
                        s[t][n][r + 1] = e[1];
                        rs2 += e;
                    }
                lrow[t] += rs2[0] + rs2[1];
#pragma unroll
                for (int j = 0; j < NJ; ++j) {
                    const bool two = 2 * j + 1 < NSUB;
                    pf[t][j] = h8{(half_t)s[t][2 * j][0], (half_t)s[t][2 * j][1], (half_t)s[t][2 * j][2], (half_t)s[t][2 * j][3],
                                  two ? (half_t)s[t][two ? 2 * j + 1 : 0][0] : (half_t)0.f, two ? (half_t)s[t][two ? 2 * j + 1 : 0][1] : (half_t)0.f,
                                  two ? (half_t)s[t][two ? 2 * j + 1 : 0][2] : (half_t)0.f, two ? (half_t)s[t][two ? 2 * j + 1 : 0][3] : (half_t)0.f};
                }
            }
#pragma unroll
            for (int n = 0; n < NO; ++n)
#pragma unroll
                for (int j = 0; j < NJ; ++j) {
                    const int r0 = 16 * (2 * j) + 4 * g + (li >> 2), r1 = r0 + 16;
                    const int cc = 2 * n + ((li & 3) >> 1), off = (li & 1) * 4;
                    const s4v lo = __builtin_amdgcn_ds_read_tr16_b64_v4i16(
                        (__attribute__((address_space(3))) s4v *)(tV + r0 * HD + (cc ^ vswz<HD>(r0)) * 8 + off));
                    const s4v hi = __builtin_amdgcn_ds_read_tr16_b64_v4i16(
                        (__attribute__((address_space(3))) s4v *)(tV + r1 * HD + (cc ^ vswz<HD>(r1)) * 8 + off));
                    const s8v both = s8v{lo[0], lo[1], lo[2], lo[3], hi[0], hi[1], hi[2], hi[3]};
                    const h8 vf = __builtin_bit_cast(h8, both);
#pragma unroll
                    for (int t = 0; t < QT; ++t) o[t][n] = mfma16(vf, pf[t][j], o[t][n]);
                }
        }
    };
    auto run = [&](auto live_tag) {
        constexpr bool LIVE = decltype(live_tag)::value;
        int kt = k_lo, buf = 0;
        for (; k_hi - kt > 32; kt += KB, buf ^= 1) {
            if constexpr (LIVE) tile_body(std::integral_constant<int, 4>{}, kt, buf);
            if (kt + KB < k_hi) {
                store_tile(buf ^ 1);
                if (kt + 2 * KB < k_hi) load_tile(kt + 2 * KB);
            }
            __syncthreads();
        }
        if constexpr (LIVE) {
            if (kt < k_hi) {
                if (k_hi - kt > 16) tile_body(std::integral_constant<int, 2>{}, kt, buf);
                else tile_body(std::integral_constant<int, 1>{}, kt, buf);
            }
        }
    };
    if (wave_live) run(std::true_type{});
    else run(std::false_type{});

    if (!wave_live) return;
#pragma unroll
    for (int t = 0; t < QT; ++t) {
        float l = lrow[t];
        l += __shfl_xor(l, 16, 64);
        l += __shfl_xor(l, 32, 64);
        const int qi = qw + 16 * t + li;
        if (qi >= Tq) continue;
        const float inv = l > 0.f ? 1.0f / l : 0.f;
        half_t *dst = p.O + ob_off + (int64_t)qi * p.o_st + (int64_t)h * HD;
#pragma unroll
        for (int n = 0; n < NO; ++n)
            *reinterpret_cast<h4 *>(dst + 16 * n + 4 * g) =
                h4{(half_t)(o[t][n][0] * inv), (half_t)(o[t][n][1] * inv), (half_t)(o[t][n][2] * inv), (half_t)(o[t][n][3] * inv)};
    }
}

template <int HD, int QT>
static hipError_t launch_qt(const AttnParams &p, hipStream_t s) {
    const int nqb = cdiv(p.T - ((p.q_trim && p.cu) ? 2 : 0), 64 * QT);
    dim3 grid(((p.B * p.heads + 7) / 8) * 8 * nqb);
    if (p.causal) OPUS_LAUNCH(KC_ATTN_PREFILL, (attn_prefill_kernel<HD, true, QT>), grid, dim3(256), 0, s, p);
    else OPUS_LAUNCH(KC_ATTN_PREFILL, (attn_prefill_kernel<HD, false, QT>), grid, dim3(256), 0, s, p);
    return hipGetLastError();
}
template <int HD>
static hipError_t launch_hd(const AttnParams &p, hipStream_t s) {
    bool one = !(HD <= 64 && (int64_t)p.B * p.heads * cdiv(p.T, 128) >= 512);
    if (g_knobs.misc[3]) one = !one;
    return one ? launch_qt<HD, 1>(p, s) : launch_qt<HD, 2>(p, s);
}

hipError_t launch_attn_prefill(const AttnParams &p, hipStream_t s) {
    if (p.T <= 0 || p.B <= 0) return hipErrorInvalidValue;
    if ((p.o_st & 3) || (p.o_sb & 3) || (p.q_st & 7) || (p.k_st & 7) || (p.v_st & 7) || (p.q_sb & 7) || (p.k_sb & 7) || (p.v_sb & 7))
        return hipErrorInvalidValue;
    if ((int64_t)p.T * (p.k_st > p.v_st ? p.k_st : p.v_st) * 2 >= (1ll << 31)) return hipErrorInvalidValue;
    switch (p.head_dim) {
        case 16: return launch_hd<16>(p, s);
        case 32: return launch_hd<32>(p, s);
        case 64: return launch_hd<64>(p, s);
        case 128: return launch_hd<128>(p, s);
    }
    return hipErrorInvalidValue;
}

}
```

### opus-pllm_amd/csrc/common.h

```cpp
#pragma once
#include <hip/hip_runtime.h>
#include <hip/hip_ext.h>
#include <stdint.h>

namespace opus {

#ifdef OPUS_BF16
typedef __bf16 half_t;
typedef __bf16 h8 __attribute__((ext_vector_type(8)));
typedef __bf16 h4 __attribute__((ext_vector_type(4)));
typedef __bf16 h2 __attribute__((ext_vector_type(2)));
#else
typedef _Float16 half_t;
typedef _Float16 h8 __attribute__((ext_vector_type(8)));
typedef _Float16 h4 __attribute__((ext_vector_type(4)));
typedef _Float16 h2 __attribute__((ext_vector_type(2)));
#endif
typedef float f4 __attribute__((ext_vector_type(4)));
__device__ __forceinline__ f4 mfma16(h8 a, h8 b, f4 c) {
#ifdef OPUS_BF16
    return __builtin_amdgcn_mfma_f32_16x16x32_bf16(a, b, c, 0, 0, 0);
#else
    return __builtin_amdgcn_mfma_f32_16x16x32_f16(a, b, c, 0, 0, 0);
#endif
}

enum Epi { EPI_NONE = 0, EPI_GELU = 1, EPI_SILU_GU16 = 2 };
__device__ __forceinline__ int kpart_begin(int n, int part, int parts) {
    return parts == 1 ? (part ? n : 0) : (int)((unsigned)(n * part) / (unsigned)parts);
}
#define OPUS_ARGS_ONE_BATCH(p)                                                                                                        \
    asm volatile("" ::"s"((p).A), "s"((p).Af), "s"((p).W), "s"((p).C), "s"((p).bias), "s"((p).residual), "s"((p).ws), "s"((p).xh_out),  \
                 "s"((p).ssq_out), "s"((p).row_ssq), "s"((p).lda), "s"((p).ldc), "s"((p).ldr), "s"((p).M), "s"((p).N), "s"((p).K),     \
                 "s"((p).out_f32), "s"((p).norm_eps), "s"((p).row_nblk), "s"((p).no_rot), "s"((p).c_tiled))
constexpr int SKINNY_MAX_M_CAP = 16;
int skinny_max_m();
#define SKINNY_MAX_M skinny_max_m()
constexpr int MID_MAX_M = 64;
enum KClass { KC_SKINNY = 0, KC_MID, KC_WIDE, KC_RING, KC_PP, KC_TILE, KC_REDUCE, KC_ATTN_PREFILL, KC_ATTN_DECODE, KC_NORM,
              KC_OTHER, KC_STREAM, KC_CONTACT, KC_CONSTRAINT, KC_LOGITPROC, KC_XENT, KC_COUNT };
enum Phase { PH_ENCODE = 0, PH_PROJECT, PH_SPLICE, PH_PREFILL, PH_DECODE, PH_OTHER, PH_SCORE, PH_COUNT };

struct LaunchEvents {
    hipEvent_t main0 = nullptr, main1 = nullptr, aux0 = nullptr, aux1 = nullptr;
    int main_class = -1;
    bool main_used = false, aux_used = false;
    double aux_bytes = 0.0;
};
extern thread_local LaunchEvents *tl_launch_ev;
#define OPUS_LAUNCH(klass, kernel, grid, block, lds, stream, ...)                                                        \
    do {                                                                                                                  \
        ::opus::LaunchEvents *ev_ = ::opus::tl_launch_ev;                                                                 \
        if (ev_ && (klass) != ::opus::KC_REDUCE && !ev_->main_used) {                                                     \
            ev_->main_used = true;                                                                                        \
            ev_->main_class = (klass);                                                                                    \
            hipExtLaunchKernelGGL(kernel, grid, block, lds, stream, ev_->main0, ev_->main1, 0, __VA_ARGS__);              \
        } else if (ev_ && (klass) == ::opus::KC_REDUCE && !ev_->aux_used) {                                               \
            ev_->aux_used = true;                                                                                         \
            hipExtLaunchKernelGGL(kernel, grid, block, lds, stream, ev_->aux0, ev_->aux1, 0, __VA_ARGS__);                \
        } else {                                                                                                          \
            hipLaunchKernelGGL(kernel, grid, block, lds, stream, __VA_ARGS__);                                            \
        }                                                                                                                 \
    } while (0)
hipError_t ensure_dyn_lds(const void *fn, size_t bytes);

__device__ __forceinline__ void rotate_pair(float a, float b, float c, float sn, float &lo, float &hi) {
    lo = __builtin_fmaf(a, c, -__fmul_rn(b, sn));
    hi = __builtin_fmaf(b, c, __fmul_rn(a, sn));
    asm volatile("" : "+v"(lo), "+v"(hi));
}

__host__ __device__ __forceinline__ int64_t tiled_off(int row, int k, int K) {
    return ((int64_t)(row >> 4) * (K >> 6) + (k >> 6)) * 1024 + ((k & 63) >> 5) * 512 + ((((k & 31) >> 3) << 4) + (row & 15)) * 8 + (k & 7);
}

constexpr int HANDOFF_WORDS = 1024, HANDOFF_ERR = 1023;
constexpr int HANDOFF_SPIN_LIMIT = 1 << 19;

struct GemmParams {
    const half_t *A;
    const float *Af;
    float norm_eps;
    int64_t lda;
    const half_t *W;
    int M, N, K;
    const float *bias;
    const float *residual;
    int64_t ldr;
    void *C;
    int64_t ldc;
    int out_f32;
    int epi;
    float *ws;
    int64_t ws_bytes;
    half_t *xh_out;
    float *ssq_out;
    int *fused_done;
    const float *row_ssq;
    int row_nblk;
    int64_t ssq_cap = 0;
    int *nblk_out = nullptr;
    int slab_only = 0;
    int *ks_out = nullptr;
    int force_wide = 0;
    const float *rope_cs = nullptr;
    const int32_t *rope_pos = nullptr;
    int rope_T = 0, rope_cols = 0, rope_qcols = 0;
    float rope_qscale = 1.0f;
    int *rope_done = nullptr;
    int a_tiled = 0, xh_tiled = 0, c_tiled = 0;
    int *combine_cnt = nullptr;
    float *ln_part = nullptr;
    int *ln_done = nullptr;
    const float *ln_stat = nullptr;
    const float *ln_colsum = nullptr;
    int pp_gm = 8;
    int stagger = 0;
    int no_rot = 0;
    long long *trace = nullptr;
    int *pp_plan = nullptr;
};
constexpr int PP_PLAN_WORDS = 5;
enum PpTail { PP_TAIL_NONE = 0, PP_TAIL_PAIR = 1, PP_TAIL_REDUCE = 2 };

struct AttnParams {
    const half_t *Q, *K, *V;
    int64_t q_sb, q_st, k_sb, k_st, v_sb, v_st;
    half_t *O;
    int64_t o_sb, o_st;
    const int32_t *kstart;
    const int32_t *kend;
    int B, T, heads, group, head_dim, causal;
    float scale;
    const int32_t *cu = nullptr;
    int q_trim = 0;
};

hipError_t launch_gemm(const GemmParams &p, hipStream_t s, int *klass);
hipError_t launch_splitk_reduce(const GemmParams &p, int ks, hipStream_t s);
bool gemm_stream_ok(const GemmParams &p);
bool gemm_stream_would(int M, int N, int K, int slab_only, int a_tiled, int row_scale, int64_t ws_bytes);
hipError_t launch_gemm_stream(const GemmParams &p, hipStream_t s);
struct Knobs {
    int no_stream = 0;
    int no_ln_fusion = 0;
    int debug_a_tiled = 0;
    int pp_gm = 8;
    int enc_full_last_layer = 0;
    int misc[8] = {0, 0, 0, 0, 0, 0, 0, 0};
};
extern Knobs g_knobs;
template <int NWAVES, int ROWS>
__device__ __forceinline__ void block_row_rstd(const float *__restrict__ ssq, int M, int nblk, float inv_k, float eps, float *out,
                                               int wave, int lane) {
    constexpr int RW = (ROWS + NWAVES - 1) / NWAVES;
    float part[RW];
#pragma unroll
    for (int r = 0; r < RW; ++r) part[r] = 0.f;
    for (int j0 = 0; j0 < nblk; j0 += 256) {
        float t[RW][4];
#pragma unroll
        for (int r = 0; r < RW; ++r) {
            int row = wave + NWAVES * r;
            row = row < M ? row : M - 1;
#pragma unroll
            for (int u = 0; u < 4; ++u) {
                const int j = j0 + 64 * u + lane;
                t[r][u] = ssq[(int64_t)row * nblk + (j < nblk ? j : nblk - 1)];
                t[r][u] = j < nblk ? t[r][u] : 0.f;
            }
        }
#pragma unroll
        for (int r = 0; r < RW; ++r) part[r] += (t[r][0] + t[r][1]) + (t[r][2] + t[r][3]);
    }
#pragma unroll
    for (int r = 0; r < RW; ++r) {
        float q = part[r];
#pragma unroll
        for (int o = 32; o > 0; o >>= 1) q += __shfl_xor(q, o, 64);
        const int row = wave + NWAVES * r;
        if (lane == 0 && row < ROWS) out[row] = rsqrtf(q * inv_k + eps);
    }
}
bool gemm_goes_wide(int M, int N);
bool gemm_goes_pp(int M, int N);
hipError_t launch_attn_prefill(const AttnParams &p, hipStream_t s);
struct AttnPrefixParams {
    const half_t *kc, *vc;
    int64_t cache_sb, cache_sh;
    const int32_t *kstart;
    int Tp;
    const half_t *qkv;
    int n;
    const int32_t *list, *off, *blocks;
    half_t *out;
    int nh, nkv, hd;
    float scale;
    const int32_t *par = nullptr;
// ... 172 lines not shown
```

### opus-pllm_amd/csrc/elementwise.hip

```cpp
#include "common.h"

namespace opus {

__global__ __launch_bounds__(256) void esm_embed_kernel(const int32_t *__restrict__ tok, const half_t *__restrict__ emb,
                                                        int T, int D, float *__restrict__ x, const int32_t *__restrict__ cu,
                                                        int32_t *__restrict__ pos) {
    __shared__ int s_cnt[2];
    const int b = blockIdx.y;
    int64_t r0 = (int64_t)b * T;
    if (cu) {
        r0 = cu[b];
        T = cu[b + 1] - cu[b];
        if ((int)blockIdx.x * 16 >= T) return;
    }
    const int32_t *row = tok + r0;
    if (threadIdx.x < 2) s_cnt[threadIdx.x] = 0;
    __syncthreads();
    int nm = 0, nv = 0;
    for (int t = threadIdx.x; t < T; t += 256) {
        const int v = row[t];
        nm += (v == 32);
        nv += (v != 1);
    }
    atomicAdd(&s_cnt[0], nm);
    atomicAdd(&s_cnt[1], nv);
    __syncthreads();
    const float scale = (1.0f - 0.15f * 0.8f) / (1.0f - (float)s_cnt[0] / (float)s_cnt[1]);
    const int t0 = blockIdx.x * 16;
    const int nvec = D >> 3;
    for (int i = threadIdx.x; i < 16 * nvec; i += 256) {
        const int t = t0 + i / nvec, c = i % nvec;
        if (t >= T) break;
        const int v = row[t];
        float o[8];
        if (v == 1 || v == 32) {
#pragma unroll
            for (int j = 0; j < 8; ++j) o[j] = 0.f;
        } else {
            const h8 e = *reinterpret_cast<const h8 *>(emb + (int64_t)v * D + c * 8);
#pragma unroll
            for (int j = 0; j < 8; ++j) o[j] = (float)e[j] * scale;
        }
        float4 *dst = reinterpret_cast<float4 *>(x + (r0 + t) * D + c * 8);
        dst[0] = make_float4(o[0], o[1], o[2], o[3]);
        dst[1] = make_float4(o[4], o[5], o[6], o[7]);
        if (pos && c == 0) pos[r0 + t] = t;
    }
}

hipError_t launch_esm_embed(const int32_t *tok, const half_t *emb, int B, int T, int D, float *x, hipStream_t s) {
    hipLaunchKernelGGL(esm_embed_kernel, dim3(cdiv(T, 16), B), dim3(256), 0, s, tok, emb, T, D, x, nullptr, nullptr);
    return hipGetLastError();
}
hipError_t launch_esm_embed_packed(const int32_t *tok, const half_t *emb, const int32_t *cu, int B, int Tmax, int D, float *x,
                                   int32_t *pos, hipStream_t s) {
    if (!cu || !pos) return hipErrorInvalidValue;
    hipLaunchKernelGGL(esm_embed_kernel, dim3(cdiv(Tmax, 16), B), dim3(256), 0, s, tok, emb, Tmax, D, x, cu, pos);
    return hipGetLastError();
}

__device__ __forceinline__ void rope8(half_t *base, int half, const float *cs, float scale) {
    h8 lo = *reinterpret_cast<h8 *>(base);
    h8 hi = *reinterpret_cast<h8 *>(base + half);
    h8 olo, ohi;
#pragma unroll
    for (int j = 0; j < 8; ++j) {
        const float c = cs[2 * j], sn = cs[2 * j + 1];
        const float a = (float)lo[j] * scale, b = (float)hi[j] * scale;
        float rl, rh;
        rotate_pair(a, b, c, sn, rl, rh);
        olo[j] = (half_t)rl;
        ohi[j] = (half_t)rh;
    }
    *reinterpret_cast<h8 *>(base) = olo;
    *reinterpret_cast<h8 *>(base + half) = ohi;
}

__global__ __launch_bounds__(256) void esm_rope_kernel(half_t *__restrict__ qkv, const float *__restrict__ cs, int T,
                                                       int heads, int hd, float qscale, int64_t total, const int32_t *__restrict__ pos) {
    const int64_t i = (int64_t)blockIdx.x * 256 + threadIdx.x;
    if (i >= total) return;
    const int half = hd >> 1, vph = half >> 3;
    const int v = (int)(i % vph);
    int64_t r = i / vph;
    const int h = (int)(r % heads); r /= heads;
    const int which = (int)(r & 1);
    const int64_t row = r >> 1;
    const int t = pos ? pos[row] : (int)(row % T);
    const int D = heads * hd;
    half_t *base = qkv + row * (3 * (int64_t)D) + which * D + h * hd + v * 8;
    rope8(base, half, cs + ((int64_t)t * half + v * 8) * 2, which == 0 ? qscale : 1.0f);
}

hipError_t launch_esm_rope(half_t *qkv, const float *cs, int B, int T, int heads, int hd, float qscale, hipStream_t s, const int32_t *pos) {
    if (hd & 15) return hipErrorInvalidValue;
    const int64_t total = (int64_t)B * T * 2 * heads * (hd >> 4);
    hipLaunchKernelGGL(esm_rope_kernel, dim3(cdiv(total, 256)), dim3(256), 0, s, qkv, cs, T, heads, hd, qscale, total, pos);
    return hipGetLastError();
}

__global__ __launch_bounds__(256) void dec_rope_cache_kernel(half_t *__restrict__ qkv, const float *__restrict__ cs,
                                                             const int32_t *__restrict__ kstart, int T, int nh, int nkv,
                                                             int hd, half_t *__restrict__ kc, half_t *__restrict__ vc,
                                                             int64_t cache_sb, int64_t cache_sh, int64_t total) {
    const int64_t i = (int64_t)blockIdx.x * 256 + threadIdx.x;
    if (i >= total) return;
    const int half = hd >> 1, vph = half >> 3;
    const int v = (int)(i % vph);
    int64_t r = i / vph;
    const int hh = (int)(r % (nh + nkv)); r /= (nh + nkv);
    const int64_t row = r;
    const int b = (int)(row / T), t = (int)(row % T);
    int pos = t - kstart[b];
    pos = pos < 0 ? 0 : pos;
    const int64_t ld = (int64_t)(nh + 2 * nkv) * hd;
    half_t *base = qkv + row * ld + (int64_t)hh * hd + v * 8;
    rope8(base, half, cs + ((int64_t)pos * half + v * 8) * 2, 1.0f);
    if (hh >= nh && kc) {
        const int kh = hh - nh;
        half_t *kd = kc + b * cache_sb + kh * cache_sh + (int64_t)t * hd + v * 8;
        half_t *vd = vc + b * cache_sb + kh * cache_sh + (int64_t)t * hd + v * 8;
        const half_t *vs = base + (int64_t)nkv * hd;
        *reinterpret_cast<h8 *>(kd) = *reinterpret_cast<h8 *>(base);
        *reinterpret_cast<h8 *>(kd + half) = *reinterpret_cast<h8 *>(base + half);
        *reinterpret_cast<h8 *>(vd) = *reinterpret_cast<const h8 *>(vs);
        *reinterpret_cast<h8 *>(vd + half) = *reinterpret_cast<const h8 *>(vs + half);
    }
}
// ... 925 lines not shown
```

### opus-pllm_amd/csrc/gemm.hip

```cpp
#include "common.h"
#include <cstdlib>
#include <map>
#include <type_traits>
#include <mutex>
#include <utility>

namespace opus {

thread_local LaunchEvents *tl_launch_ev = nullptr;
static Knobs knobs_from_env() {
    Knobs k;
    for (int i = 0; i < 8; ++i) {
        char name[32];
        snprintf(name, sizeof(name), "OPUS_KNOB_MISC%d", i);
        if (const char *v = getenv(name)) k.misc[i] = atoi(v);
    }
    return k;
}
Knobs g_knobs = knobs_from_env();

hipError_t ensure_dyn_lds(const void *fn, size_t bytes) {
    static std::mutex mu;
    static std::map<std::pair<int, const void *>, size_t> done;
    int dev = 0;
    hipError_t e = hipGetDevice(&dev);
    if (e != hipSuccess) return e;
    std::lock_guard<std::mutex> lock(mu);
    size_t &have = done[std::make_pair(dev, fn)];
    if (bytes <= have) return hipSuccess;
    e = hipFuncSetAttribute(fn, hipFuncAttributeMaxDynamicSharedMemorySize, (int)bytes);
    if (e == hipSuccess) have = bytes;
    return e;
}

__device__ __forceinline__ float gelu_erf(float x) {
    const float z = fabsf(x) * 0.70710678118654752f;
    const float t = __builtin_amdgcn_rcpf(1.0f + 0.3275911f * z);
    const float poly = t * (0.254829592f + t * (-0.284496736f + t * (1.421413741f + t * (-1.453152027f + t * 1.061405429f))));
    const float erf_abs = 1.0f - poly * __expf(-z * z);
    return 0.5f * x * (1.0f + copysignf(erf_abs, x));
}
__device__ __forceinline__ float silu(float x) { return x * __builtin_amdgcn_rcpf(1.0f + __expf(-x)); }

template <int MT, int EPI, bool NORM, bool ALDS>
__global__ __launch_bounds__(1024) void gemm_skinny_kernel(GemmParams p) {
    extern __shared__ __attribute__((aligned(16))) float red[];
    OPUS_ARGS_ONE_BATCH(p);
    constexpr int PB = EPI == EPI_SILU_GU16 ? 2 : 1;
    const int tid = threadIdx.x;
    const int lane = tid & 63;
    const int wave = __builtin_amdgcn_readfirstlane(tid >> 6);
    const int nwaves = blockDim.x >> 6;
    const int wpp = nwaves / PB;
    const int pl = PB == 1 ? 0 : wave / wpp, kpart = wave - pl * wpp;
    const int chunks = p.K >> 6;
    const int npanels = (p.N + 15) >> 4;
    int panel = blockIdx.x * PB + pl;
    panel = panel < npanels ? panel : npanels - 1;
    const int c0 = kpart_begin(chunks, kpart, wpp);
    const int c1 = kpart_begin(chunks, kpart + 1, wpp);
    const int g = lane >> 4, li = lane & 15;
    float *rss = red + nwaves * MT * 256;
    float *wss = rss + nwaves * MT * 16;
    half_t *xs = reinterpret_cast<half_t *>(wss + 256);

    const half_t *wp = p.W + ((int64_t)panel * chunks) * 1024 + lane * 8;
    f4 acc[MT];
    float ssq[MT];
#pragma unroll
// ... 716 lines not shown
        if (s < KS) stage_load(s);
    wait_glds(issued_upto(NS - 1));
    __builtin_amdgcn_s_barrier();
    read_frags(0, a0, b0);
    for (int ks = 0; ks < KS; ks += 2) {
        step(ks, a0, b0, a1, b1);
        if (ks + 1 < KS) step(ks + 1, a1, b1, a0, b0);
    }

    if (ksplit > 1) {
        float *slab = p.ws + (int64_t)ky * p.M * p.N;
#pragma unroll
        for (int i = 0; i < TM; ++i) {
            const int m = m0 + wm * (16 * TM) + i * 16 + li;
            if (m >= p.M) continue;
#pragma unroll
            for (int j = 0; j < TN; ++j) {
                const int nb = n0 + wn * (16 * TN) + j * 16 + 4 * g;
                if ((p.N & 3) == 0 && nb + 3 < p.N) {
                    *reinterpret_cast<float4 *>(slab + (int64_t)m * p.N + nb) = make_float4(acc[i][j][0], acc[i][j][1], acc[i][j][2], acc[i][j][3]);
                } else {
#pragma unroll
                    for (int r = 0; r < 4; ++r)
                        if (nb + r < p.N) slab[(int64_t)m * p.N + nb + r] = acc[i][j][r];
                }
            }
        }
        return;
    }
#pragma unroll
    for (int i = 0; i < TM; ++i) {
        const int m = m0 + wm * (16 * TM) + i * 16 + li;
        if (m >= p.M) continue;
        if (EPI == EPI_SILU_GU16) {
#pragma unroll
            for (int jj = 0; jj < TN / 2; ++jj)
                store4<EPI>(p, m, n0 + wn * (16 * TN) + jj * 32 + 4 * g, acc[i][2 * jj], acc[i][2 * jj + 1]);
        } else {
#pragma unroll
            for (int j = 0; j < TN; ++j) store4<EPI>(p, m, n0 + wn * (16 * TN) + j * 16 + 4 * g, acc[i][j], acc[i][j]);
        }
    }
}

constexpr int PP_DIST = 6;

__host__ __device__ __forceinline__ void pp_tile_coords(int id, int tiles_m, int tiles_n, int &tm, int &tn, int GM = 8) {
    const int per_group = GM * tiles_n;
    const int grp = id / per_group, rem_id = id - grp * per_group;
    const int rows_here = (tiles_m - grp * GM) < GM ? (tiles_m - grp * GM) : GM;
    tm = grp * GM + rem_id % rows_here;
    tn = rem_id / rows_here;
}
template <int EPI, bool LNA>
__device__ __forceinline__ void pp_finish(const GemmParams &p, f4 (&acc)[8][4], char *smem, const int wave, const int m0, const int n0,
                                          const int bid, const int full_tiles, const int tail_split, const int kpart, const bool partial);
template <int EPI, bool LNA>
__device__ __forceinline__ void pp_epilogue(const GemmParams &p, f4 (&acc)[8][4], char *smem, const int wave, const int m0, const int n0,
                                            const char *pair_slab);
template <int EPI, bool LNA = false>
__global__ __launch_bounds__(512) void gemm_pp_kernel(GemmParams p, int tiles_m, int tiles_n, int full_tiles, int tail_split) {
    extern __shared__ __attribute__((aligned(16))) char smem[];
    constexpr int HT = 16384;
    const int tid = threadIdx.x, lane = tid & 63;
    const int wave = __builtin_amdgcn_readfirstlane(tid >> 6);
    const int wr = wave >> 2, wc = wave & 3;
    const int g = lane >> 4, li = lane & 15;
    if (p.stagger > 0 && blockIdx.x < 256 && ((blockIdx.x >> 3) & 1))
        for (int i = 0; i < p.stagger; ++i) __builtin_amdgcn_s_sleep(127);
    if (p.trace && tid == 0) p.trace[blockIdx.x * 4] = wall_clock64();
    int bid = blockIdx.x, kpart = 0;
    const bool partial = bid >= full_tiles;
    if (!partial) {
        const int nwg = full_tiles, q = nwg >> 3, rr = nwg & 7, xcd = bid & 7;
        bid = (xcd < rr ? xcd * (q + 1) : rr * (q + 1) + (xcd - rr) * q) + (bid >> 3);
    } else {
        const int j = bid - full_tiles;
        bid = full_tiles + j / tail_split;
        kpart = j % tail_split;
    }
    int tm, tn;
    pp_tile_coords(bid, tiles_m, tiles_n, tm, tn, p.pp_gm);
    const int m0 = tm * 256, n0 = tn * 256;
    const int KT_all = p.K >> 6;
    const int kt0 = partial ? (int)((int64_t)KT_all * kpart / tail_split) : 0;
    const int kt1 = partial ? (int)((int64_t)KT_all * (kpart + 1) / tail_split) : KT_all;
    const int KT = kt1 - kt0, NH = 4 * KT;
    const int npanels = (p.N + 15) >> 4;

    typedef const __attribute__((address_space(1))) void *gptr_t;
    typedef __attribute__((address_space(3))) void *lptr_t;
    unsigned offA[2][2], offB[2][2];
#pragma unroll
    for (int j = 0; j < 2; ++j) {
        const int q = 2 * wave + j;
        const int lr = 8 * q + (lane >> 3);
        const int chunk = (lane & 7) ^ ((lr >> 1) & 7);
#pragma unroll
        for (int rh = 0; rh < 2; ++rh) {
            int row = m0 + (lr >> 6) * 128 + rh * 64 + (lr & 63);
            row = row < p.M ? row : p.M - 1;
            offA[j][rh] = (unsigned)(((int64_t)row * p.lda + chunk * 8) * 2);
        }
        const int pi = q >> 1, s = q & 1;
#pragma unroll
        for (int ch = 0; ch < 2; ++ch) {
            int pn = (n0 >> 4) + (pi >> 1) * 4 + ch * 2 + (pi & 1);
            pn = pn < npanels ? pn : npanels - 1;
            offB[j][ch] = (unsigned)((((int64_t)pn * KT_all) * 1024 + s * 512 + lane * 8) * 2);
        }
    }
    const char *baseA = reinterpret_cast<const char *>(p.A) + (int64_t)kt0 * 128;
    const char *baseB = reinterpret_cast<const char *>(p.W) + (int64_t)kt0 * 2048;
// ... 54 lines not shown
                                    mfma16(bf[ct][s], af[rt][s], acc[4 * rhh + rt][2 * chh + ct]);
                }
        __builtin_amdgcn_s_setprio(0);
    };
    constexpr int D = PP_DIST;
    auto feed = [&](int phi) {
        if (phi + D < NH) {
            issue_half(phi + D);
            vmcnt_wait<2 * (D - 2)>();
        } else {
            const int left = NH - 1 - (phi + 2);
            if (left >= 3) vmcnt_wait<6>();
            else if (left == 2) vmcnt_wait<4>();
            else if (left == 1) vmcnt_wait<2>();
            else vmcnt_wait<0>();
        }
    };

#pragma unroll
    for (int h = 0; h < D; ++h)
        if (h < NH) issue_half(h);
    if (NH >= D) vmcnt_wait<2 * (D - 4)>();
    else vmcnt_wait<0>();
    __builtin_amdgcn_s_barrier();
    if (p.trace && tid == 0) p.trace[blockIdx.x * 4 + 1] = wall_clock64();
    if (wr == 1) __builtin_amdgcn_s_barrier();
    read_a(0, 0, a0);

    for (int kt = 0; kt < KT; ++kt) {
        const int phi = 4 * kt;
        read_b(kt, 0, b0);
        feed(phi);
        __builtin_amdgcn_s_barrier();
        mfma_quadrant(0, 0, a0, b0);
        __builtin_amdgcn_s_barrier();
        read_b(kt, 1, b1);
        feed(phi + 1);
        __builtin_amdgcn_s_barrier();
        mfma_quadrant(0, 1, a0, b1);
        __builtin_amdgcn_s_barrier();
        read_a(kt, 1, a1);
        feed(phi + 2);
        __builtin_amdgcn_s_barrier();
        mfma_quadrant(1, 1, a1, b1);
        __builtin_amdgcn_s_barrier();
        if (kt + 1 < KT) read_a(kt + 1, 0, a0);
        feed(phi + 3);
        __builtin_amdgcn_s_barrier();
        mfma_quadrant(1, 0, a1, b0);
        __builtin_amdgcn_s_barrier();
    }
    if (wr == 0) __builtin_amdgcn_s_barrier();
    if (p.trace && tid == 0) p.trace[blockIdx.x * 4 + 2] = wall_clock64();
    pp_finish<EPI, LNA>(p, acc, smem, wave, m0, n0, bid, full_tiles, tail_split, kpart, partial);
}

template <int EPI, bool LNA>
__device__ __forceinline__ void pp_finish(const GemmParams &p, f4 (&acc)[8][4], char *smem, const int wave, const int m0, const int n0,
                                          const int bid, const int full_tiles, const int tail_split, const int kpart, const bool partial) {
    int lane;
    asm volatile("v_mbcnt_lo_u32_b32 %0, -1, 0\n\tv_mbcnt_hi_u32_b32 %0, -1, %0" : "=v"(lane));
    const int tid = wave * 64 + lane;
    const int wr = wave >> 2, wc = wave & 3;
    const int g = lane >> 4, li = lane & 15;

    const char *pair_slab = nullptr;
    if (partial && tail_split == 2 && p.combine_cnt) {
        typedef unsigned int u4p __attribute__((ext_vector_type(4)));
        const int tt = bid - full_tiles;
        int *cnt = p.combine_cnt + 512 + 2 * tt;
        int *word = reinterpret_cast<int *>(smem);
        if (tid == 0) *word = __hip_atomic_fetch_add(cnt, 1, __ATOMIC_RELAXED, __HIP_MEMORY_SCOPE_AGENT);
        __syncthreads();
        const int order = *word;
        __syncthreads();
        if (order > 1 && tid == 0)
            __hip_atomic_store(p.combine_cnt + HANDOFF_ERR, 1, __ATOMIC_RELAXED, __HIP_MEMORY_SCOPE_AGENT);
        const __amdgpu_buffer_rsrc_t srs = __builtin_amdgcn_make_buffer_rsrc((void *)(p.ws + ((int64_t)tt << 16)), 0, 1 << 18, 0x00020000);
        if (order == 0) {
#pragma unroll
            for (int i = 0; i < 8; ++i)
#pragma unroll
                for (int j = 0; j < 4; ++j)
                    __builtin_amdgcn_raw_buffer_store_b128(__builtin_bit_cast(u4p, acc[i][j]), srs, ((i * 4 + j) * 512 + tid) * 16, 0, 16);
            asm volatile("s_waitcnt vmcnt(0)" ::: "memory");
            __syncthreads();
            if (tid == 0) __hip_atomic_store(cnt + 1, 1, __ATOMIC_RELAXED, __HIP_MEMORY_SCOPE_AGENT);
            return;
        }
        if (tid == 0) {
            int spins = 0;
            while (__hip_atomic_load(cnt + 1, __ATOMIC_RELAXED, __HIP_MEMORY_SCOPE_AGENT) == 0) {
                __builtin_amdgcn_s_sleep(4);
                if (++spins > HANDOFF_SPIN_LIMIT) {
                    __hip_atomic_store(p.combine_cnt + HANDOFF_ERR, 1, __ATOMIC_RELAXED, __HIP_MEMORY_SCOPE_AGENT);
                    break;
                }
            }
            __hip_atomic_store(cnt, 0, __ATOMIC_RELAXED, __HIP_MEMORY_SCOPE_AGENT);
            __hip_atomic_store(cnt + 1, 0, __ATOMIC_RELAXED, __HIP_MEMORY_SCOPE_AGENT);
        }
        __syncthreads();
        pair_slab = reinterpret_cast<const char *>(p.ws + ((int64_t)tt << 16));
    } else if (partial) {
        float *slab = p.ws + (((int64_t)(bid - full_tiles) * tail_split + kpart) << 16);
#pragma unroll
        for (int i = 0; i < 8; ++i) {
            const int r = wr * 128 + i * 16 + li;
#pragma unroll
            for (int j = 0; j < 4; ++j)
                *reinterpret_cast<float4 *>(slab + r * 256 + wc * 64 + j * 16 + 4 * g) = make_float4(acc[i][j][0], acc[i][j][1], acc[i][j][2], acc[i][j][3]);
        }
        return;
    }
    pp_epilogue<EPI, LNA>(p, acc, smem, wave, m0, n0, pair_slab);
}

template <int EPI, bool LNA>
__device__ __forceinline__ void pp_epilogue(const GemmParams &p, f4 (&acc)[8][4], char *smem, const int wave, const int m0, const int n0,
                                            const char *pair_slab) {
    int lane;
    asm volatile("v_mbcnt_lo_u32_b32 %0, -1, 0\n\tv_mbcnt_hi_u32_b32 %0, -1, %0" : "=v"(lane));
    const int tid = wave * 64 + lane;
    const int wr = wave >> 2, wc = wave & 3;
    const int g = lane >> 4, li = lane & 15;
    constexpr int NO = EPI == EPI_SILU_GU16 ? 32 : 64;
    const int nlim = EPI == EPI_SILU_GU16 ? p.N / 2 : p.N;
    const int nw0 = EPI == EPI_SILU_GU16 ? (n0 >> 1) + wc * 32 : n0 + wc * 64;
    const bool rows16 = ((p.ldc & 7) == 0) && ((p.ldr & 3) == 0) && nw0 + NO <= nlim;
    const __amdgpu_buffer_rsrc_t psrs = __builtin_amdgcn_make_buffer_rsrc((void *)pair_slab, 0, pair_slab ? 1 << 18 : 0, 0x00020000);
    auto pair_load = [&](int i, int j) {
        return __builtin_bit_cast(f4, __builtin_amdgcn_raw_buffer_load_b128(psrs, ((i * 4 + j) * 512 + tid) * 16, 0, 16));
    };
    if (!rows16) {
#pragma unroll
        for (int i = 0; i < 8; ++i) {
            f4 av[4];
#pragma unroll
            for (int j = 0; j < 4; ++j) av[j] = acc[i][j];
            if (pair_slab) {
#pragma unroll
                for (int j = 0; j < 4; ++j) av[j] += pair_load(i, j);
            }
            const int m = m0 + wr * 128 + i * 16 + li;
            if (m >= p.M) continue;
            if (EPI == EPI_SILU_GU16) {
#pragma unroll
                for (int jj = 0; jj < 2; ++jj) store4<EPI>(p, m, n0 + wc * 64 + jj * 32 + 4 * g, av[2 * jj], av[2 * jj + 1]);
            } else {
#pragma unroll
                for (int j = 0; j < 4; ++j) store4<EPI>(p, m, n0 + wc * 64 + j * 16 + 4 * g, av[j], av[j]);
            }
        }
        return;
    }
    float *patch = reinterpret_cast<float *>(smem + wave * 16384);
    constexpr bool XSW = NO == 64;
    constexpr int PS = XSW ? NO : NO + 4;
    auto pidx = [&](int r, int c) { return XSW ? r * PS + ((((c >> 2) ^ (r & 15)) << 2) | (c & 3)) : r * PS + c; };
    float bz[16];
#pragma unroll
    for (int q = 0; q < 16; ++q) bz[q] = 0.f;
    if (p.bias && !LNA && EPI == EPI_SILU_GU16) {
        if (EPI == EPI_SILU_GU16) {
#pragma unroll
            for (int jj = 0; jj < 2; ++jj)
#pragma unroll
                for (int r = 0; r < 4; ++r) {
                    const int nb = n0 + wc * 64 + jj * 32 + 4 * g + r;
                    bz[jj * 8 + r] = p.bias[nb];
                    bz[jj * 8 + 4 + r] = p.bias[nb + 16];
// ... 147 lines not shown
                            v[r] = silu(gate) * up;
                        }
                        *reinterpret_cast<f4 *>(pu + pidx(li, jj * 16 + 4 * g)) = v;
                    }
                } else {
                    f4 b4[4], c4[LNA ? 4 : 1];
#pragma unroll
                    for (int j = 0; j < 4; ++j) {
                        b4[j] = *reinterpret_cast<const f4 *>(cb + j * 16 + 4 * g);
                        if constexpr (LNA) c4[j] = *reinterpret_cast<const f4 *>(cb + 64 + j * 16 + 4 * g);
                    }
#pragma unroll
                    for (int j = 0; j < 4; ++j) {
                        f4 v = av[j];
#pragma unroll
                        for (int r = 0; r < 4; ++r) {
                            if constexpr (LNA) v[r] = __builtin_fmaf(lst[ib & 1][u].y, v[r] - lst[ib & 1][u].x * c4[j][r], b4[j][r]);
                            else v[r] += b4[j][r];
                            if (EPI == EPI_GELU) v[r] = gelu_erf(v[r]);
                        }
                        *reinterpret_cast<f4 *>(pu + pidx(li, j * 16 + 4 * g)) = v;
                    }
                }
            }
            __builtin_amdgcn_fence(__ATOMIC_RELEASE, "wavefront");
            asm volatile("s_waitcnt lgkmcnt(0)" ::: "memory");
            __builtin_amdgcn_fence(__ATOMIC_ACQUIRE, "wavefront");
#pragma unroll
            for (int u = 0; u < RB; ++u) {
                const int i = ib * RB + u;
                const float *pu = patch + u * PIMG;
                float4 (&rcur)[NR] = rbuf[ib & 1][u];
                const int tr0 = wr * 128 + i * 16;
                const bool f32_out = MODE == M_GENERIC ? p.out_f32 != 0 : RES;
                if (f32_out) {
#pragma unroll
                    for (int ps = 0; ps < 16 / RPP32; ++ps) {
                        const int r = ps * RPP32 + lane / LPR32, c = (lane % LPR32) * 4;
                        f4 v = *reinterpret_cast<const f4 *>(pu + pidx(r, c));
                        if constexpr (RES || MODE == M_GENERIC) {
                            const float4 rr = rcur[ps];
                            v[0] += rr.x; v[1] += rr.y; v[2] += rr.z; v[3] += rr.w;
                        }
                        __builtin_amdgcn_raw_buffer_store_b128(__builtin_bit_cast(u4v, v), crs, ((tr0 + r) * (int)p.ldc + nw0 + c) * 4, 0, 0);
                        if constexpr (MODE == M_F32RES_LN) {
                            const h4 xh = h4{(half_t)v[0], (half_t)v[1], (half_t)v[2], (half_t)v[3]};
                            __builtin_amdgcn_raw_buffer_store_b64(__builtin_bit_cast(u2v, xh), xrs, ((tr0 + r) * p.N + nw0 + c) * 2, 0, 0);
                            float s1 = (v[0] + v[1]) + (v[2] + v[3]);
                            float s2 = (v[0] * v[0] + v[1] * v[1]) + (v[2] * v[2] + v[3] * v[3]);
#pragma unroll
                            for (int o = 1; o < LPR32; o <<= 1) { s1 += __shfl_xor(s1, o, 64); s2 += __shfl_xor(s2, o, 64); }
                            const float2 st = make_float2(s1, s2);
                            const int poff = (lane % LPR32) == 0 ? ((tr0 + r) * (p.N >> 6) + (nw0 >> 6)) * 8 : 0x7ffffff0;
                            __builtin_amdgcn_raw_buffer_store_b64(__builtin_bit_cast(u2v, st), prs, poff, 0, 0);
                        }
                    }
                } else if (CS || (MODE == M_GENERIC && rope_on)) {
                    if constexpr (ROPE_OK) {
                        const int r = lane >> 2, c = (lane & 3) * 8;
                        const f4 l0 = *reinterpret_cast<const f4 *>(pu + pidx(r, c)), l1 = *reinterpret_cast<const f4 *>(pu + pidx(r, c + 4));
                        const f4 h0 = *reinterpret_cast<const f4 *>(pu + pidx(r, c + 32)), h1 = *reinterpret_cast<const f4 *>(pu + pidx(r, c + 36));
                        const float qs = nw0 < p.rope_qcols ? p.rope_qscale : 1.0f;
                        const float csv[16] = {rcur[0].x, rcur[0].y, rcur[0].z, rcur[0].w, rcur[1].x, rcur[1].y, rcur[1].z, rcur[1].w,
                                               rcur[2].x, rcur[2].y, rcur[2].z, rcur[2].w, rcur[3].x, rcur[3].y, rcur[3].z, rcur[3].w};
                        h8 olo, ohi;
#pragma unroll
                        for (int e = 0; e < 8; ++e) {
                            const float a = (float)(half_t)(e < 4 ? l0[e] : l1[e - 4]) * qs, b = (float)(half_t)(e < 4 ? h0[e] : h1[e - 4]) * qs;
                            const float cc = csv[2 * e], sn = csv[2 * e + 1];
                            float rl, rh;
                            rotate_pair(a, b, cc, sn, rl, rh);
                            olo[e] = (half_t)rl;
                            ohi[e] = (half_t)rh;
                        }
                        const int off = ((tr0 + r) * (int)p.ldc + nw0 + c) * 2;
                        __builtin_amdgcn_raw_buffer_store_b128(__builtin_bit_cast(u4v, olo), crs, off, 0, 0);
                        __builtin_amdgcn_raw_buffer_store_b128(__builtin_bit_cast(u4v, ohi), crs, off + 64, 0, 0);
                    }
                } else {
#pragma unroll
                    for (int ps = 0; ps < 16 / RPP16; ++ps) {
                        const int r = ps * RPP16 + lane / LPR16, c = (lane % LPR16) * 8;
                        f4 lo = *reinterpret_cast<const f4 *>(pu + pidx(r, c)), hi = *reinterpret_cast<const f4 *>(pu + pidx(r, c + 4));
                        if constexpr (MODE == M_GENERIC) {
                            const float4 r0 = rcur[2 * ps], r1 = rcur[2 * ps + 1];
                            lo[0] += r0.x; lo[1] += r0.y; lo[2] += r0.z; lo[3] += r0.w;
                            hi[0] += r1.x; hi[1] += r1.y; hi[2] += r1.z; hi[3] += r1.w;
                        }
                        const h8 o = h8{(half_t)lo[0], (half_t)lo[1], (half_t)lo[2], (half_t)lo[3], (half_t)hi[0], (half_t)hi[1], (half_t)hi[2], (half_t)hi[3]};
                        __builtin_amdgcn_raw_buffer_store_b128(__builtin_bit_cast(u4v, o), crs, ((tr0 + r) * (int)p.ldc + nw0 + c) * 2, 0, 0);
                    }
                }
            }
            asm volatile("s_waitcnt lgkmcnt(0)" ::: "memory");
            if constexpr (PAIR) {
                if (ib + 1 < 8 / RB) prefetch(ib + 1);
            }
        }
    };
    typedef std::false_type NP;
    typedef std::true_type WP;
    if constexpr (LNA) {
        if (rope_on) run(std::integral_constant<int, ROPE_OK ? M_ROPE : M_F16>{}, NP{});
        else if (pair_slab) run(std::integral_constant<int, M_F16>{}, WP{});
        else run(std::integral_constant<int, M_F16>{}, NP{});
    } else if constexpr (EPI != EPI_NONE) {
        if (!p.out_f32 && !p.residual) {
            if (pair_slab) run(std::integral_constant<int, M_F16>{}, WP{});
            else run(std::integral_constant<int, M_F16>{}, NP{});
        } else run(std::integral_constant<int, M_GENERIC>{}, NP{});
    } else {
        if (rope_on) run(std::integral_constant<int, M_ROPE>{}, NP{});
        else if (!p.out_f32 && !p.residual) {
            if (pair_slab) run(std::integral_constant<int, M_F16>{}, WP{});
            else run(std::integral_constant<int, M_F16>{}, NP{});
        } else if (p.out_f32 && p.residual && p.ln_part) {
            if (pair_slab) run(std::integral_constant<int, M_F32RES_LN>{}, WP{});
            else run(std::integral_constant<int, M_F32RES_LN>{}, NP{});
        } else if (p.out_f32 && p.residual) {
            if (pair_slab) run(std::integral_constant<int, M_F32RES>{}, WP{});
            else run(std::integral_constant<int, M_F32RES>{}, NP{});
        } else run(std::integral_constant<int, M_GENERIC>{}, NP{});
    }
    if (p.trace && tid == 0) {
        asm volatile("s_waitcnt vmcnt(0)" ::: "memory");
        p.trace[blockIdx.x * 4 + 3] = wall_clock64();
    }
}

template <int EPI>
__global__ __launch_bounds__(256) void pp_tail_reduce_kernel(GemmParams p, int tiles_m, int tiles_n, int full_tiles, int tail_split) {
    int tm, tn;
    pp_tile_coords(full_tiles + blockIdx.x, tiles_m, tiles_n, tm, tn, p.pp_gm);
    const int lane = threadIdx.x & 63, wave = threadIdx.x >> 6;
    const int col = 4 * lane, n = tn * 256 + col;
    const float *base = p.ws + ((int64_t)blockIdx.x * tail_split << 16) + col;
    f4 bias4 = f4{0.f, 0.f, 0.f, 0.f}, bias_up = f4{0.f, 0.f, 0.f, 0.f};
    const bool gate_lane = (col & 31) < 16;
    if (p.bias) {
#pragma unroll
        for (int c = 0; c < 4; ++c) {
            if (n + c < p.N) bias4[c] = p.bias[n + c];
            if (EPI == EPI_SILU_GU16 && gate_lane && n + 16 + c < p.N) bias_up[c] = p.bias[n + 16 + c];
        }
    }
    constexpr int RW = 8;
    f4 csum = f4{0.f, 0.f, 0.f, 0.f};
    if (p.ln_stat && p.ln_colsum) {
#pragma unroll
        for (int c = 0; c < 4; ++c)
            if (n + c < p.N) csum[c] = p.ln_colsum[n + c];
    }
    f4 v[RW];
#pragma unroll
    for (int i = 0; i < RW; ++i) v[i] = f4{0.f, 0.f, 0.f, 0.f};
    const int r0 = blockIdx.y * 32 + wave * RW;
    for (int k0 = 0; k0 < tail_split; k0 += 4) {
        float4 t[4][RW];
#pragma unroll
        for (int u = 0; u < 4; ++u) {
            const int kk = k0 + u < tail_split ? k0 + u : tail_split - 1;
#pragma unroll
            for (int i = 0; i < RW; ++i) t[u][i] = *reinterpret_cast<const float4 *>(base + ((int64_t)kk << 16) + (r0 + i) * 256);
        }
#pragma unroll
        for (int u = 0; u < 4; ++u) {
            if (k0 + u >= tail_split) continue;
#pragma unroll
            for (int i = 0; i < RW; ++i) { v[i][0] += t[u][i].x; v[i][1] += t[u][i].y; v[i][2] += t[u][i].z; v[i][3] += t[u][i].w; }
        }
    }
// ... 32 lines not shown
            live = live && n < p.N;
        }
        if (!live) continue;
        const int nlim = EPI == EPI_SILU_GU16 ? p.N / 2 : p.N;
        if (vec_ok) {
            if (p.residual) {
                const float4 rr = rres[i];
                x[0] += rr.x; x[1] += rr.y; x[2] += rr.z; x[3] += rr.w;
            }
            if (p.out_f32) *reinterpret_cast<float4 *>(reinterpret_cast<float *>(p.C) + (int64_t)m * p.ldc + no) = make_float4(x[0], x[1], x[2], x[3]);
            else *reinterpret_cast<h4 *>(reinterpret_cast<half_t *>(p.C) + (int64_t)m * p.ldc + no) = h4{(half_t)x[0], (half_t)x[1], (half_t)x[2], (half_t)x[3]};
            if (EPI == EPI_NONE && p.ln_part) {
                *reinterpret_cast<h4 *>(p.xh_out + (int64_t)m * p.N + no) = h4{(half_t)x[0], (half_t)x[1], (half_t)x[2], (half_t)x[3]};
                float s1 = (x[0] + x[1]) + (x[2] + x[3]);
                float s2 = (x[0] * x[0] + x[1] * x[1]) + (x[2] * x[2] + x[3] * x[3]);
#pragma unroll
                for (int o = 1; o < 16; o <<= 1) { s1 += __shfl_xor(s1, o, 64); s2 += __shfl_xor(s2, o, 64); }
                if ((lane & 15) == 0) reinterpret_cast<float2 *>(p.ln_part)[(int64_t)m * (p.N >> 6) + (no >> 6)] = make_float2(s1, s2);
            }
        } else {
#pragma unroll
            for (int c = 0; c < 4; ++c) {
                if (no + c >= nlim) continue;
                float y = x[c];
                if (p.residual) y += p.residual[(int64_t)m * p.ldr + no + c];
                if (p.out_f32) reinterpret_cast<float *>(p.C)[(int64_t)m * p.ldc + no + c] = y;
                else reinterpret_cast<half_t *>(p.C)[(int64_t)m * p.ldc + no + c] = (half_t)y;
            }
        }
    }
}

template <int EPI>
static hipError_t launch_pp(const GemmParams &p_in, hipStream_t s) {
    if (p_in.row_ssq) return hipErrorInvalidValue;
    if ((int64_t)p_in.M * p_in.lda * 2 >= (1ll << 32) || (int64_t)p_in.N * p_in.K * 2 >= (1ll << 32)) return hipErrorInvalidValue;
    GemmParams p = p_in;
    const bool lna = p.ln_stat != nullptr;
    if (lna && (p.out_f32 || p.residual || (p.N & 255) || (p.ldc & 7) || (EPI == EPI_SILU_GU16 && (p.bias || p.ln_colsum)))) return hipErrorInvalidValue;
    const bool lnp = p.ln_part && p.xh_out && p.ln_done && EPI == EPI_NONE && p.out_f32 && (p.N & 255) == 0 && (p.ldc & 7) == 0 &&
                     (p.ldr & 3) == 0 && p.residual;
    if (lnp) *p.ln_done = 1;
    else p.ln_part = nullptr;
    p.stagger = g_knobs.misc[5];
    p.pp_gm = g_knobs.pp_gm;
    void (*kern)(GemmParams, int, int, int, int) = gemm_pp_kernel<EPI, false>;
    if (lna) kern = gemm_pp_kernel<EPI, true>;
    const int bm = cdiv(p.M, 256), bn = cdiv(p.N, 256);
    hipError_t ea = ensure_dyn_lds(reinterpret_cast<const void *>(kern), 8 * 16384);
    if (ea != hipSuccess) return ea;
    const int T = bm * bn, KT = p.K >> 6;
    int full = T, split = 1;
    static const bool no_tail = getenv("OPUS_NO_PP_TAIL") != nullptr;
    static const bool no_rope_fuse = getenv("OPUS_NO_ROPE_FUSION") != nullptr;
    const bool rope = p.rope_cs && p.rope_done && !no_rope_fuse && EPI == EPI_NONE && !p.out_f32 && !p.residual && (p.ldc & 7) == 0 &&
                      (p.N & 255) == 0 && (p.rope_cols & 63) == 0 && (p.rope_qcols & 63) == 0 && p.rope_T > 0;
    if (rope) *p.rope_done = 1;
    else p.rope_cs = nullptr;
    const int R = T % 256;
    if (!no_tail && !rope && p.ws && T > 256 && R > 0 && R <= 128) {
        int sp = 256 / R;
        sp = sp > 8 ? 8 : sp;
        if (sp > KT / 4) sp = KT / 4;
        while (sp > 1 && ((int64_t)R * sp << 18) > p.ws_bytes) --sp;
        const double t_tile = 1.5 * KT + 12.0, gain = t_tile * (1.0 - 1.0 / sp), cost = (sp == 2 && p.combine_cnt && !g_knobs.misc[6]) ? 22.0 : 30.0;
        if (sp > 1 && gain > cost) { full = T - R; split = sp; }
    }
    const int tail = T - full;
    static const bool trace = getenv("OPUS_PP_TRACE") != nullptr;
    if (trace) {
        static long long *tb = nullptr;
        const int nwg = full + tail * split;
        if (!tb) (void)hipMalloc((void **)&tb, (size_t)(1 << 16) * 4 * sizeof(long long));
        if (tb && nwg <= (1 << 16)) {
            GemmParams q = p;
            q.trace = tb;
            hipLaunchKernelGGL(kern, dim3(nwg), dim3(512), 8 * 16384, s, q, bm, bn, full, split);
            (void)hipStreamSynchronize(s);
            std::vector<long long> h((size_t)nwg * 4);
            (void)hipMemcpy(h.data(), tb, h.size() * sizeof(long long), hipMemcpyDeviceToHost);
            long long t0 = h[0], t1 = h[3];
            double pro = 0, mainl = 0, epi = 0;
            for (int i = 0; i < nwg; ++i) {
                t0 = std::min(t0, h[4 * i]); t1 = std::max(t1, h[4 * i + 3]);
                if (i < full) { pro += h[4 * i + 1] - h[4 * i]; mainl += h[4 * i + 2] - h[4 * i + 1]; epi += h[4 * i + 3] - h[4 * i + 2]; }
            }
            fprintf(stderr, "[pp trace] M=%d N=%d K=%d epi=%d wg=%d (full %d): kernel %.1f us; per full tile: prologue %.2f us, main %.2f us, epilogue %.2f us\n",
                    p.M, p.N, p.K, EPI, nwg, full, (t1 - t0) * 0.01, pro / full * 0.01, mainl / full * 0.01, epi / full * 0.01);
            for (int r0 = 0; r0 < nwg; r0 += 256) {
                double st = 0, en = 0; int n = 0;
                for (int i = r0; i < nwg && i < r0 + 256; ++i, ++n) { st += h[4 * i] - t0; en += h[4 * i + 3] - t0; }
                fprintf(stderr, "   wg %5d..: mean start %.1f us, mean end %.1f us\n", r0, st / n * 0.01, en / n * 0.01);
            }
        }
    }
    const bool pair_mode = (!p.out_f32 && !p.residual) || (EPI == EPI_NONE && p.out_f32 && p.residual);
    const bool pair = split == 2 && p.combine_cnt && !g_knobs.misc[6] && pair_mode && (p.ldc & 7) == 0 && (p.ldr & 3) == 0 && (p.N & 255) == 0;
    if (!pair) p.combine_cnt = nullptr;
    if (p.pp_plan) {
        p.pp_plan[0] = full; p.pp_plan[1] = tail; p.pp_plan[2] = split;
        p.pp_plan[3] = split == 1 ? PP_TAIL_NONE : pair ? PP_TAIL_PAIR : PP_TAIL_REDUCE;
        p.pp_plan[4] = rope ? 1 : 0;
    }
    OPUS_LAUNCH(KC_PP, kern, dim3(full + tail * split), dim3(512), 8 * 16384, s, p, bm, bn, full, split);
    hipError_t e = hipGetLastError();
    if (e != hipSuccess || split == 1 || pair) return e;
    if (tl_launch_ev) tl_launch_ev->aux_bytes = ((double)tail * split * 65536 * 4) + (double)tail * 65536 * (p.out_f32 ? 4 : 2);
    OPUS_LAUNCH(KC_REDUCE, (pp_tail_reduce_kernel<EPI>), dim3(tail, 8), dim3(256), 0, s, p, bm, bn, full, split);
    return hipGetLastError();
}

template <int EPI>
__global__ __launch_bounds__(256) void splitk_reduce_kernel(GemmParams p, int ksplit) {
    const int nout = EPI == EPI_SILU_GU16 ? p.N / 2 : p.N;
    const int64_t i = (int64_t)blockIdx.x * 256 + threadIdx.x;
    if (i >= (int64_t)p.M * nout) return;
    const int m = (int)(i / nout), no = (int)(i % nout);
    const int64_t slab = (int64_t)p.M * p.N;
    float rstd = 1.0f;
    if (p.Af) {
        float q = 0.f;
        for (int k = 0; k < ksplit; ++k) q += p.ws[ksplit * slab + (int64_t)k * p.M + m];
        rstd = rsqrtf(q / (float)p.K + p.norm_eps);
    } else if (p.row_ssq) {
        const float *src = p.row_ssq + (int64_t)m * p.row_nblk;
        float q0 = 0.f, q1 = 0.f, q2 = 0.f, q3 = 0.f;
        int j = 0;
        for (; j + 4 <= p.row_nblk; j += 4) { q0 += src[j]; q1 += src[j + 1]; q2 += src[j + 2]; q3 += src[j + 3]; }
        for (; j < p.row_nblk; ++j) q0 += src[j];
        rstd = rsqrtf(((q0 + q1) + (q2 + q3)) / (float)p.K + p.norm_eps);
    }
    float v;
    if (EPI == EPI_SILU_GU16) {
        const int n = (no >> 4) * 32 + (no & 15);
        float gate = 0.f, up = 0.f;
        for (int k0 = 0; k0 < ksplit; k0 += 8) {
            float tg[8], tu[8];
#pragma unroll
            for (int u = 0; u < 8; ++u) {
                const int kk = k0 + u < ksplit ? k0 + u : ksplit - 1;
                tg[u] = p.ws[kk * slab + (int64_t)m * p.N + n];
                tu[u] = p.ws[kk * slab + (int64_t)m * p.N + n + 16];
            }
#pragma unroll
            for (int u = 0; u < 8; ++u)
                if (k0 + u < ksplit) { gate += tg[u]; up += tu[u]; }
        }
        gate *= rstd;
        up *= rstd;
        if (p.bias) { gate += p.bias[n]; up += p.bias[n + 16]; }
        v = silu(gate) * up;
// ... 544 lines not shown
```

### opus-pllm_amd/csrc/norm.hip

```cpp
#include "common.h"

namespace opus {

constexpr int NV_MAX = 20;

__device__ __forceinline__ float wave_sum(float v) {
#pragma unroll
    for (int o = 32; o > 0; o >>= 1) v += __shfl_xor(v, o, 64);
    return v;
}

template <int MODE, int NV>
__global__ __launch_bounds__(256) void rownorm_kernel(const float *__restrict__ x, const float *__restrict__ w,
                                                      const float *__restrict__ b, float eps, int64_t rows, int D,
                                                      half_t *__restrict__ out_h, float *__restrict__ out_f) {
    const int lane = threadIdx.x & 63;
    const int64_t row = (int64_t)blockIdx.x * 4 + (threadIdx.x >> 6);
    if (row >= rows) return;
    const float4 *xr = reinterpret_cast<const float4 *>(x + row * D);
    const int nvec = D >> 2;
    float4 v[NV];
    float s = 0.f;
#pragma unroll
    for (int i = 0; i < NV; ++i) {
// ... 38 lines not shown
            if (out_h) {
                h4 o = {(half_t)y.x, (half_t)y.y, (half_t)y.z, (half_t)y.w};
                reinterpret_cast<h4 *>(out_h + row * D)[c] = o;
            }
            if (out_f) reinterpret_cast<float4 *>(out_f + row * D)[c] = y;
        }
    }
}

template <int MODE>
static hipError_t launch_rownorm(const float *x, const float *w, const float *b, float eps, int64_t rows, int D, half_t *out_h,
                                 float *out_f, hipStream_t s) {
    if (D > NV_MAX * 256 || (D & 3)) return hipErrorInvalidValue;
    const dim3 grid(cdiv(rows, 4)), block(256);
    if (D <= 5 * 256) OPUS_LAUNCH(KC_NORM, (rownorm_kernel<MODE, 5>), grid, block, 0, s, x, w, b, eps, rows, D, out_h, out_f);
    else if (D <= 10 * 256) OPUS_LAUNCH(KC_NORM, (rownorm_kernel<MODE, 10>), grid, block, 0, s, x, w, b, eps, rows, D, out_h, out_f);
    else if (D <= 16 * 256) OPUS_LAUNCH(KC_NORM, (rownorm_kernel<MODE, 16>), grid, block, 0, s, x, w, b, eps, rows, D, out_h, out_f);
    else OPUS_LAUNCH(KC_NORM, (rownorm_kernel<MODE, 20>), grid, block, 0, s, x, w, b, eps, rows, D, out_h, out_f);
    return hipGetLastError();
}
hipError_t launch_layernorm(const float *x, const float *w, const float *b, float eps, int64_t rows, int D,
                            half_t *out_h, float *out_f, hipStream_t s) {
    return launch_rownorm<0>(x, w, b, eps, rows, D, out_h, out_f, s);
}
hipError_t launch_rmsnorm(const float *x, const float *w, float eps, int64_t rows, int D, half_t *out, hipStream_t s) {
    return launch_rownorm<1>(x, w, nullptr, eps, rows, D, out, nullptr, s);
}
hipError_t launch_l2norm(const float *x, int64_t rows, int D, half_t *out, hipStream_t s) {
    return launch_rownorm<2>(x, nullptr, nullptr, 0.f, rows, D, out, nullptr, s);
}

__global__ __launch_bounds__(256) void ln_finalize_kernel(const float2 *__restrict__ part, int64_t rows, int nslab, float inv_d,
                                                          float eps, int rms, float2 *__restrict__ stat) {
    const int q = threadIdx.x & 15;
    int64_t m = (int64_t)blockIdx.x * 16 + (threadIdx.x >> 4);
    const bool live = m < rows;
    m = live ? m : rows - 1;
    const float2 *src = part + m * nslab;
    float s1 = 0.f, s2 = 0.f;
    for (int j0 = 0; j0 < nslab; j0 += 64) {
        float2 t[4];
#pragma unroll
        for (int u = 0; u < 4; ++u) {
            const int j = j0 + 16 * u + q;
            t[u] = src[j < nslab ? j : nslab - 1];
            if (j >= nslab) t[u] = make_float2(0.f, 0.f);
        }
        s1 += (t[0].x + t[1].x) + (t[2].x + t[3].x);
        s2 += (t[0].y + t[1].y) + (t[2].y + t[3].y);
    }
#pragma unroll
    for (int o = 1; o < 16; o <<= 1) { s1 += __shfl_xor(s1, o, 64); s2 += __shfl_xor(s2, o, 64); }
    if (!live || q) return;
    if (rms) {
        stat[m] = make_float2(0.f, rsqrtf(s2 * inv_d + eps));
        return;
    }
    const float mu = s1 * inv_d;
    const float var = fmaxf(s2 * inv_d - mu * mu, 0.f);
    stat[m] = make_float2(mu, rsqrtf(var + eps));
}
hipError_t launch_ln_finalize(const float *part, int64_t rows, int nslab, int D, float eps, int rms, float *stat, hipStream_t s) {
    hipLaunchKernelGGL(ln_finalize_kernel, dim3(cdiv(rows, 16)), dim3(256), 0, s, reinterpret_cast<const float2 *>(part), rows, nslab,
                       1.0f / (float)D, eps, rms, reinterpret_cast<float2 *>(stat));
    return hipGetLastError();
}

__global__ __launch_bounds__(256) void f2h_kernel(const float *__restrict__ x, int64_t n4, half_t *__restrict__ out) {
    const int64_t i = (int64_t)blockIdx.x * 256 + threadIdx.x;
    if (i >= n4) return;
    const float4 v = reinterpret_cast<const float4 *>(x)[i];
    reinterpret_cast<h4 *>(out)[i] = h4{(half_t)v.x, (half_t)v.y, (half_t)v.z, (half_t)v.w};
}
hipError_t launch_f2h(const float *x, int64_t n, half_t *out, hipStream_t s) {
    if (n & 3) return hipErrorInvalidValue;
    hipLaunchKernelGGL(f2h_kernel, dim3(cdiv(n >> 2, 256)), dim3(256), 0, s, x, n >> 2, out);
    return hipGetLastError();
}

__global__ __launch_bounds__(256) void masked_mean_kernel(const float *__restrict__ h, const int32_t *__restrict__ lens,
                                                          int T, int D, float *__restrict__ out, const int32_t *__restrict__ cu) {
    const int b = blockIdx.y;
    const int d = blockIdx.x * 256 + threadIdx.x;
    if (d >= D) return;
    const int n = (cu ? cu[b + 1] - cu[b] : lens[b]) - 2;
    const float *p = h + ((cu ? (int64_t)cu[b] : (int64_t)b * T) + 1) * D + d;
    float s8[8] = {0.f, 0.f, 0.f, 0.f, 0.f, 0.f, 0.f, 0.f};
    int t = 0;
    for (; t + 8 <= n; t += 8) {
#pragma unroll
        for (int k = 0; k < 8; ++k) s8[k] += p[(int64_t)(t + k) * D];
    }
    for (int k = 0; t < n; ++t, ++k) s8[k] += p[(int64_t)t * D];
    const float s = ((s8[0] + s8[1]) + (s8[2] + s8[3])) + ((s8[4] + s8[5]) + (s8[6] + s8[7]));
    out[(int64_t)b * D + d] = s / (float)n;
}

hipError_t launch_masked_mean(const float *h, const int32_t *lens, int B, int T, int D, float *out, hipStream_t s) {
    hipLaunchKernelGGL(masked_mean_kernel, dim3(cdiv(D, 256), B), dim3(256), 0, s, h, lens, T, D, out, nullptr);
    return hipGetLastError();
}
hipError_t launch_masked_mean_packed(const float *h, const int32_t *cu, int B, int D, float *out, hipStream_t s) {
    if (!cu) return hipErrorInvalidValue;
    hipLaunchKernelGGL(masked_mean_kernel, dim3(cdiv(D, 256), B), dim3(256), 0, s, h, nullptr, 0, D, out, cu);
    return hipGetLastError();
}

}
```

Baseline: 258.0 proteins/s.

## Fuse RoPE/KV-cache write into prefill attention and add last-arriver LN finalize

Prefill attention now applies rotary embedding and writes the K/V cache inside the attention kernel for head_dim 128, removing the separate rope/cache kernel launch and its memory round trip. Separately, an opt-in last-arriver path has the final GEMM block per row tile reduce the layernorm partials and write the stats, skipping the standalone finalize launch; it relies on atomic counters. A debug entry point and knobs are added for testing both paths.

Result: no change. 258.0 proteins/s, median of 2 (+0.0%).

```diff
diff --git a/include/opus_pllm.h b/include/opus_pllm.h
--- a/include/opus_pllm.h
+++ b/include/opus_pllm.h
@@ -163,6 +163,8 @@
 
 int opus_debug_attn_decode(opus_ctx *ctx, const void *d_qkv, const void *d_k_hist, const void *d_v_hist, const int32_t *d_kstart,
                            int32_t B, int32_t T0, int32_t step, void *d_out, void *d_k_new, void *d_v_new, void *stream);
+int opus_debug_prefill_attn(opus_ctx *ctx, const void *d_qkv, const int32_t *d_kstart, int32_t B, int32_t T, void *d_out,
+                            void *d_k_cache, void *d_v_cache, void *stream);
 
 int opus_check_error(opus_ctx *ctx, void *stream);
 
diff --git a/opus-pllm_amd/_cabi.py b/opus-pllm_amd/_cabi.py
--- a/opus-pllm_amd/_cabi.py
+++ b/opus-pllm_amd/_cabi.py
@@ -95,6 +95,7 @@
     "opus_debug_knob": (C.c_int, [_P, C.c_char_p, C.c_int32]),
     "opus_stat": (C.c_int64, [_P, C.c_char_p]),
     "opus_debug_attn_decode": (C.c_int, [_P, _P, _P, _P, _P, C.c_int32, C.c_int32, C.c_int32, _P, _P, _P, _P]),
+    "opus_debug_prefill_attn": (C.c_int, [_P, _P, _P, C.c_int32, C.c_int32, _P, _P, _P, _P]),
     "opus_llama_forward": (C.c_int, [_P, _P, _P, C.c_int32, C.c_int32, _P, C.c_int32, _P, _P, _P, _P, C.c_int64, _P]),
     "opus_llama_forward_scratch_bytes": (C.c_int64, [C.POINTER(CConfig), C.c_int32, C.c_int32]),
     "opus_llama_prefix": (C.c_int, [_P, _P, _P, C.c_int32, C.c_int32, _P, _P, C.POINTER(C.c_int64), _P]),
diff --git a/opus-pllm_amd/csrc/api.cpp b/opus-pllm_amd/csrc/api.cpp
--- a/opus-pllm_amd/csrc/api.cpp
+++ b/opus-pllm_amd/csrc/api.cpp
@@ -108,6 +108,7 @@
     uint64_t graph_clock = 0;
     int64_t graph_instantiations = 0;
     int64_t graph_replays = 0;
+    int64_t ln_fin_launches = 0;
     int64_t decode_steps = 0;
     char *gen_mem = nullptr;
     GenOutDesc *d_gen = nullptr;
@@ -138,6 +139,9 @@
     float *rq_ln_part = nullptr;
     half_t *rq_ln_xh = nullptr;
     int rq_ln_done = 0;
+    float *rq_ln_fin = nullptr;
+    float rq_ln_eps = 0.f;
+    int rq_ln_rms = 0, rq_ln_fin_done = 0;
     const float *rq_ln_stat = nullptr, *rq_ln_colsum = nullptr;
     int *rq_pp_plan = nullptr;
     bool xln_tiled = false;
@@ -159,6 +163,9 @@
 
 static std::atomic<int64_t> g_epoch{0};
 static void new_epoch(opus_ctx *c) { c->epoch = ++g_epoch; }
+static hipError_t zero_handoff(opus_ctx *c, hipStream_t s) {
+    return hipMemsetAsync(c->d_cnt, 0, HANDOFF_ERR * sizeof(int32_t), s);
+}
 
 struct ContRows {
     const int32_t *nkst;
@@ -535,8 +542,12 @@
     c->rq_ks = 1;
     p.force_wide = c->rq_force_wide; p.slab_only = c->rq_slab_only; p.ks_out = &c->rq_ks;
     c->rq_force_wide = c->rq_slab_only = 0;
-    c->rq_ln_done = 0;
-    if (c->rq_ln_part) { p.xh_out = c->rq_ln_xh; p.ssq_out = nullptr; p.ln_part = c->rq_ln_part; p.ln_done = &c->rq_ln_done; c->rq_ln_part = nullptr; }
+    c->rq_ln_done = c->rq_ln_fin_done = 0;
+    if (c->rq_ln_part) {
+        p.xh_out = c->rq_ln_xh; p.ssq_out = nullptr; p.ln_part = c->rq_ln_part; p.ln_done = &c->rq_ln_done; c->rq_ln_part = nullptr;
+        p.ln_stat_out = c->rq_ln_fin; p.ln_eps = c->rq_ln_eps; p.ln_rms = c->rq_ln_rms; p.ln_cnt = c->d_cnt; p.ln_fin_done = &c->rq_ln_fin_done;
+    }
+    c->rq_ln_fin = nullptr;
     if (c->rq_ln_stat) { p.ln_stat = c->rq_ln_stat; p.ln_colsum = c->rq_ln_colsum; c->rq_ln_stat = c->rq_ln_colsum = nullptr; }
     p.combine_cnt = c->d_cnt;
     p.pp_plan = c->rq_pp_plan;
@@ -546,13 +557,15 @@
     const int nout = epi == EPI_SILU_GU16 ? N / 2 : N;
     const double bytes = 2.0 * N * K + (Af ? 4.0 : 2.0) * M * K + (double)M * nout * (out_f32 ? 4 : 2) +
                          (residual ? 4.0 * M * nout : 0.0);
+    const double ln_bytes = p.ln_stat_out && g_knobs.ln_last_arriver ? 8.0 * M * (N / 64) + 8.0 * M : 0.0;
     int klass = M <= SKINNY_MAX_M ? KC_SKINNY : KC_TILE;
     hipError_t e;
     {
-        Timed t(c, s, klass, bytes, 2.0 * M * N * (double)K);
+        Timed t(c, s, klass, bytes + ln_bytes, 2.0 * M * N * (double)K);
         e = launch_gemm(p, s, &klass);
     }
     if (e != hipSuccess) return fail(OPUS_EHIP, "gemm M=%d N=%d K=%d failed: %s", M, N, K, hipGetErrorString(e));
+    if (c->rq_ln_fin_done) ++c->ln_fin_launches;
     return OPUS_OK;
 }
 static int gemm(opus_ctx *c, hipStream_t s, const half_t *A, int64_t lda, const half_t *W, int M, int N, int K,
@@ -654,7 +667,7 @@
     c->phase = PH_ENCODE;
     const int D = g.enc_dim, F = g.enc_ffn, nh = g.enc_heads, hd = D / nh;
     const bool packed = d_cu != nullptr;
-    HIPC(hipMemsetAsync(c->d_cnt, 0, HANDOFF_ERR * sizeof(int32_t), s));
+    HIPC(zero_handoff(c, s));
     if (packed) KL(KC_OTHER, 4.0 * M * D, launch_esm_embed_packed(d_tokens, c->enc_emb, d_cu, B, T, D, c->e_x, c->e_pos, s));
     else KL(KC_OTHER, 4.0 * M * D, launch_esm_embed(d_tokens, c->enc_emb, B, T, D, c->e_x, s));
     static const bool no_ln_env = getenv("OPUS_NO_LN_FUSION") != nullptr;
@@ -693,16 +706,16 @@
         a.B = B; a.T = T; a.heads = nh; a.group = 1; a.head_dim = hd; a.causal = 0; a.scale = 1.0f;
         a.q_trim = packed && l + 1 == g.enc_layers && T > 2 && !g_knobs.enc_full_last_layer ? 1 : 0;
         KLF(KC_ATTN_PREFILL, 8.0 * M * D, attn_flops, launch_attn_prefill(a, s));
-        if (fc1_pp) { c->rq_ln_part = c->e_part; c->rq_ln_xh = c->e_xn; }
+        if (fc1_pp) { c->rq_ln_part = c->e_part; c->rq_ln_xh = c->e_xn; c->rq_ln_fin = c->e_stat; c->rq_ln_eps = g.enc_ln_eps; c->rq_ln_rms = 0; }
         OPC(gemm(c, s, c->e_ctx, D, L.wo, M, D, D, L.bo, EPI_NONE, c->e_x, c->e_x, D, 1));
         have_stat = c->rq_ln_done != 0;
-        if (have_stat) { OPC(finalize()); c->rq_ln_stat = c->e_stat; c->rq_ln_colsum = L.s1; }
+        if (have_stat) { if (!c->rq_ln_fin_done) OPC(finalize()); c->rq_ln_stat = c->e_stat; c->rq_ln_colsum = L.s1; }
         else KL(KC_NORM, 6.0 * M * D, launch_layernorm(c->e_x, nullptr, nullptr, g.enc_ln_eps, M, D, c->e_xn, nullptr, s));
         OPC(gemm(c, s, c->e_xn, D, L.w1, M, F, D, L.b1, EPI_GELU, nullptr, c->e_h1, F, 0));
-        if (qkv_pp && l + 1 < g.enc_layers) { c->rq_ln_part = c->e_part; c->rq_ln_xh = c->e_xn; }
+        if (qkv_pp && l + 1 < g.enc_layers) { c->rq_ln_part = c->e_part; c->rq_ln_xh = c->e_xn; c->rq_ln_fin = c->e_stat; c->rq_ln_eps = g.enc_ln_eps; c->rq_ln_rms = 0; }
         OPC(gemm(c, s, c->e_h1, F, L.w2, M, D, F, L.b2, EPI_NONE, c->e_x, c->e_x, D, 1));
         have_stat = c->rq_ln_done != 0;
-        if (have_stat) OPC(finalize());
+        if (have_stat && !c->rq_ln_fin_done) OPC(finalize());
     }
     KL(KC_NORM, 8.0 * M * D, launch_layernorm(c->e_x, c->enc_lnfw, c->enc_lnfb, g.enc_ln_eps, M, D, nullptr, c->e_hid, s));
     if (packed) KL(KC_OTHER, 4.0 * M * D, launch_masked_mean_packed(c->e_hid, d_cu, B, D, d_pooled, s));
@@ -874,7 +887,7 @@
 static int protein_projector_rows(opus_ctx *c, hipStream_t s, const float *d_pooled, int B, half_t *d_out) {
     const opus_config &g = c->cfg;
     const int De = g.enc_dim;
-    HIPC(hipMemsetAsync(c->d_cnt, 0, HANDOFF_ERR * sizeof(int32_t), s));
+    HIPC(zero_handoff(c, s));
     if (!g.has_protein_projector) {
         KL(KC_OTHER, 6.0 * B * De, launch_f2h(d_pooled, (int64_t)B * De, d_out, s));
         return OPUS_OK;
@@ -1063,7 +1076,7 @@
                        const ContRows *cont) {
     const opus_config &g = c->cfg;
     const int H = g.dec_dim, M = B * T;
-    HIPC(hipMemsetAsync(c->d_cnt, 0, HANDOFF_ERR * sizeof(int32_t), s));
+    HIPC(zero_handoff(c, s));
     if (!cont) KL(KC_OTHER, 1.0 * M, launch_mask_to_kstart(mask, B, T, c->d_kstart, s));
     KL(KC_OTHER, 6.0 * M * H, launch_h2f(embeds, c->d_x, (int64_t)M * H, s));
     KL(KC_OTHER, 10.0 * M * H, launch_add_pos(c->d_x, c->dec_pos, cont ? cont->nkst : c->d_kstart, nullptr, 0, B, T, H, g.dec_max_pos + 1, s));
@@ -1088,6 +1101,27 @@
     return OPUS_OK;
 }
 
+static int prefill_attn(opus_ctx *c, hipStream_t s, half_t *qkv, int l, int B, int T, half_t *out) {
+    const opus_config &g = c->cfg;
+    const int nh = g.dec_heads, nkv = g.dec_kv_heads, hd = g.dec_head_dim;
+    const int QKV = (nh + 2 * nkv) * hd, QD = nh * hd;
+    const double M = (double)B * T;
+    half_t *kc = c->kc + l * c->cache_sl, *vc = c->vc + l * c->cache_sl;
+    const bool fused = hd == 128 && !g_knobs.no_rope_fusion;
+    if (!fused) KL(KC_OTHER, 4.0 * M * QKV, launch_dec_rope_cache(qkv, c->cs_dec, c->d_kstart, B, T, nh, nkv, hd, kc, vc, c->cache_sb, c->cache_sh, s));
+    AttnParams a;
+    a.Q = qkv; a.K = qkv + QD; a.V = qkv + QD + nkv * hd;
+    a.q_sb = a.k_sb = a.v_sb = (int64_t)T * QKV;
+    a.q_st = a.k_st = a.v_st = QKV;
+    a.O = out; a.o_sb = (int64_t)T * QD; a.o_st = QD;
+    a.kstart = c->d_kstart; a.kend = nullptr;
+    a.B = B; a.T = T; a.heads = nh; a.group = nh / nkv; a.head_dim = hd; a.causal = 1;
+    a.scale = 1.0f / sqrtf((float)hd);
+    if (fused) { a.rope_cs = c->cs_dec; a.kc = kc; a.vc = vc; a.cache_sb = c->cache_sb; a.cache_sh = c->cache_sh; }
+    KLF(KC_ATTN_PREFILL, 2.0 * M * (QKV + QD) + (fused ? 4.0 * M * nkv * hd : 0.0), 2.0 * B * (double)T * T * QD, launch_attn_prefill(a, s));
+    return OPUS_OK;
+}
+
 static int prefill(opus_ctx *c, hipStream_t s, const half_t *embeds, const uint8_t *mask, int B, int T, bool all_rows = false,
                    const ContRows *cont = nullptr) {
     c->phase = cont ? PH_SCORE : PH_PREFILL;
@@ -1105,7 +1139,7 @@
     const int H = g.dec_dim, F = g.dec_ffn, nh = g.dec_heads, nkv = g.dec_kv_heads, hd = g.dec_head_dim;
     const int QKV = (nh + 2 * nkv) * hd, QD = nh * hd;
     const int M = B * T;
-    HIPC(hipMemsetAsync(c->d_cnt, 0, HANDOFF_ERR * sizeof(int32_t), s));
+    HIPC(zero_handoff(c, s));
     if (!cont) KL(KC_OTHER, 1.0 * M, launch_mask_to_kstart(mask, B, T, c->d_kstart, s));
     KL(KC_OTHER, 6.0 * M * H, launch_h2f(embeds, c->d_x, (int64_t)M * H, s));
     static const bool no_ln_env = getenv("OPUS_NO_LN_FUSION") != nullptr;
@@ -1129,18 +1163,7 @@
             KL(KC_OTHER, 4.0 * M * QKV, launch_dec_rope_cache(c->d_qkv, c->cs_dec, cont->nkst, B, T, nh, nkv, hd, nullptr, nullptr, 0, 0, s));
             OPC(attn_prefix(c, s, *cont, l, M));
         } else {
-            KL(KC_OTHER, 4.0 * M * QKV,
-               launch_dec_rope_cache(c->d_qkv, c->cs_dec, c->d_kstart, B, T, nh, nkv, hd, c->kc + l * c->cache_sl,
-                                     c->vc + l * c->cache_sl, c->cache_sb, c->cache_sh, s));
-            AttnParams a;
-            a.Q = c->d_qkv; a.K = c->d_qkv + QD; a.V = c->d_qkv + QD + nkv * hd;
-            a.q_sb = a.k_sb = a.v_sb = (int64_t)T * QKV;
-            a.q_st = a.k_st = a.v_st = QKV;
-            a.O = c->d_ctx; a.o_sb = (int64_t)T * QD; a.o_st = QD;
-            a.kstart = c->d_kstart; a.kend = nullptr;
-            a.B = B; a.T = T; a.heads = nh; a.group = nh / nkv; a.head_dim = hd; a.causal = 1;
-            a.scale = 1.0f / sqrtf((float)hd);
-            KLF(KC_ATTN_PREFILL, 2.0 * M * (QKV + QD), 2.0 * B * (double)T * T * QD, launch_attn_prefill(a, s));
+            OPC(prefill_attn(c, s, c->d_qkv, l, B, T, c->d_ctx));
         }
         if (l + 1 == g.dec_layers && T > 1 && !all_rows && !g_knobs.misc[7]) {
             half_t *ctx_last = c->d_qkv;
@@ -1157,22 +1180,22 @@
             last_rows_done = true;
             break;
         }
-        if (gu_pp) { c->rq_ln_part = c->d_part; c->rq_ln_xh = c->d_xn; }
+        if (gu_pp) { c->rq_ln_part = c->d_part; c->rq_ln_xh = c->d_xn; c->rq_ln_fin = c->d_stat; c->rq_ln_eps = g.dec_rms_eps; c->rq_ln_rms = 1; }
         else if (fuse_rows() && M <= 96) c->rq_xh = c->d_xn;
         OPC(gemm(c, s, c->d_ctx, QD, L.wo, M, H, QD, nullptr, EPI_NONE, c->d_x, c->d_x, H, 1));
         c->xh_src = c->rq_done ? c->d_x : nullptr;
         have_stat = c->rq_ln_done != 0;
         if (have_stat) {
-            OPC(finalize());
+            if (!c->rq_ln_fin_done) OPC(finalize());
             c->rq_ln_stat = c->d_stat;
             OPC(gemm(c, s, c->d_xn, H, L.wgu, M, 2 * F, H, nullptr, EPI_SILU_GU16, nullptr, c->d_act, F, 0));
         } else {
             OPC(gemm_norm(c, s, c->d_x, g.dec_rms_eps, c->d_xn, L.wgu, M, 2 * F, H, EPI_SILU_GU16, c->d_act, F, 0));
         }
-        if (qkv_pp && l + 1 < g.dec_layers) { c->rq_ln_part = c->d_part; c->rq_ln_xh = c->d_xn; }
+        if (qkv_pp && l + 1 < g.dec_layers) { c->rq_ln_part = c->d_part; c->rq_ln_xh = c->d_xn; c->rq_ln_fin = c->d_stat; c->rq_ln_eps = g.dec_rms_eps; c->rq_ln_rms = 1; }
         OPC(gemm(c, s, c->d_act, F, L.wd, M, H, F, nullptr, EPI_NONE, c->d_x, c->d_x, H, 1));
         have_stat = c->rq_ln_done != 0;
-        if (have_stat) OPC(finalize());
+        if (have_stat && !c->rq_ln_fin_done) OPC(finalize());
     }
     if (all_rows) {
         c->xh_src = nullptr;
@@ -2298,13 +2321,16 @@
     hipStream_t s = (hipStream_t)stream;
     c->phase = PH_OTHER;
     for (int i = 0; i < 2 * PP_PLAN_WORDS; ++i) plan[i] = -1;
-    HIPC(hipMemsetAsync(c->d_cnt, 0, HANDOFF_ERR * sizeof(int32_t), s));
-    if (gemm_goes_pp(M, N1)) { c->rq_ln_part = part; c->rq_ln_xh = (half_t *)xh; }
+    if (!g_knobs.keep_handoff) HIPC(zero_handoff(c, s));
+    if (gemm_goes_pp(M, N1)) {
+        c->rq_ln_part = part; c->rq_ln_xh = (half_t *)xh;
+        c->rq_ln_fin = stat; c->rq_ln_eps = eps; c->rq_ln_rms = rms;
+    }
     c->rq_pp_plan = plan;
     OPC(gemm(c, s, (const half_t *)A, K1, (const half_t *)W1, M, N1, K1, b1, EPI_NONE, X, X, N1, 1));
     *produced = c->rq_ln_done;
     if (!c->rq_ln_done) return OPUS_OK;
-    KL(KC_NORM, 8.0 * M * (N1 / 64), launch_ln_finalize(part, M, N1 / 64, N1, eps, rms, stat, s));
+    if (!c->rq_ln_fin_done) KL(KC_NORM, 8.0 * M * (N1 / 64), launch_ln_finalize(part, M, N1 / 64, N1, eps, rms, stat, s));
     c->rq_ln_stat = stat; c->rq_ln_colsum = colsum;
     c->rq_pp_plan = plan + PP_PLAN_WORDS;
     if (rope_T > 0) {
@@ -2469,17 +2495,42 @@
     return OPUS_OK;
 }
 
+extern "C" int opus_debug_prefill_attn(opus_ctx *c, const void *d_qkv, const int32_t *d_kstart, int32_t B, int32_t T, void *d_out,
+                                       void *d_k_cache, void *d_v_cache, void *stream) {
+    if (!c || !d_qkv || !d_kstart || !d_out || !d_k_cache || !d_v_cache) return fail(OPUS_EBADARG, "debug_prefill_attn: null pointer");
+    const opus_config &g = c->cfg;
+    if (g.dec_arch == 1) return fail(OPUS_ESTATE, "debug_prefill_attn: a Llama-type decoder is needed");
+    if (B < 1 || B > g.max_batch || T < 1 || T > g.max_prompt)
+        return fail(OPUS_ESHAPE, "debug_prefill_attn: B=%d T=%d exceed the context (%d, %d)", B, T, g.max_batch, g.max_prompt);
+    const int nh = g.dec_heads, nkv = g.dec_kv_heads, hd = g.dec_head_dim, QKV = (nh + 2 * nkv) * hd;
+    HIPC(hipSetDevice(c->device));
+    hipStream_t s = (hipStream_t)stream;
+    HIPC(hipMemcpyAsync(c->d_qkv, d_qkv, (size_t)B * T * QKV * sizeof(half_t), hipMemcpyDeviceToDevice, s));
+    HIPC(hipMemcpyAsync(c->d_kstart, d_kstart, (size_t)B * sizeof(int32_t), hipMemcpyDeviceToDevice, s));
+    c->phase = PH_PREFILL;
+    c->prefilled = false;
+    new_epoch(c);
+    OPC(prefill_attn(c, s, c->d_qkv, 0, B, T, (half_t *)d_out));
+    const size_t pitch = (size_t)c->cache_sh * sizeof(half_t), roww = (size_t)T * hd * sizeof(half_t);
+    HIPC(hipMemcpy2DAsync(d_k_cache, roww, c->kc, pitch, roww, (size_t)B * nkv, hipMemcpyDeviceToDevice, s));
+    HIPC(hipMemcpy2DAsync(d_v_cache, roww, c->vc, pitch, roww, (size_t)B * nkv, hipMemcpyDeviceToDevice, s));
+    return OPUS_OK;
+}
+
 extern "C" int opus_debug_knob(opus_ctx *c, const char *name, int32_t value) {
     if (!name) return fail(OPUS_EBADARG, "debug_knob: null name");
     if (c) drop_graphs(c);
     if (!strcmp(name, "no_stream")) g_knobs.no_stream = value;
     else if (!strcmp(name, "debug_a_tiled")) g_knobs.debug_a_tiled = value;
     else if (!strcmp(name, "no_ln_fusion")) g_knobs.no_ln_fusion = value;
+    else if (!strcmp(name, "no_rope_fusion")) g_knobs.no_rope_fusion = value;
+    else if (!strcmp(name, "ln_last_arriver")) g_knobs.ln_last_arriver = value;
+    else if (!strcmp(name, "keep_handoff")) g_knobs.keep_handoff = value;
     else if (!strcmp(name, "enc_full_last_layer")) g_knobs.enc_full_last_layer = value;
     else if (!strcmp(name, "poison_handoff")) {
         if (!c) return fail(OPUS_EBADARG, "poison_handoff needs a context");
         std::vector<int32_t> h(HANDOFF_ERR, 0);
-        if (value) for (int i = 0; i < HANDOFF_ERR; ++i) h[i] = i < 512 ? value : ((i & 1) ? 0 : 1);
+        if (value) for (int i = 0; i < HANDOFF_ERR; ++i) h[i] = (i < 512 || i >= HANDOFF_LN) ? value : ((i & 1) ? 0 : 1);
         HIPC(hipSetDevice(c->device));
         HIPC(hipDeviceSynchronize());
         HIPC(hipMemcpy(c->d_cnt, h.data(), h.size() * sizeof(int32_t), hipMemcpyHostToDevice));
@@ -2496,6 +2547,7 @@
     if (!strcmp(name, "graph_replays")) return c->graph_replays;
     if (!strcmp(name, "graphs_cached")) return (int64_t)c->graphs.size();
     if (!strcmp(name, "decode_steps")) return c->decode_steps;
+    if (!strcmp(name, "ln_fin_launches")) return c->ln_fin_launches;
     return -1;
 }
 
diff --git a/opus-pllm_amd/csrc/attn_prefill.hip b/opus-pllm_amd/csrc/attn_prefill.hip
--- a/opus-pllm_amd/csrc/attn_prefill.hip
+++ b/opus-pllm_amd/csrc/attn_prefill.hip
@@ -40,8 +40,9 @@
 typedef short s4v __attribute__((ext_vector_type(4)));
 typedef short s8v __attribute__((ext_vector_type(8)));
 
-template <int HD, bool CAUSAL, int QT>
+template <int HD, bool CAUSAL, int QT, bool ROPE = false>
 __global__ __launch_bounds__(256) void attn_prefill_kernel(AttnParams p) {
+    static_assert(!ROPE || (HD == 128 && CAUSAL && QT == 1), "the fused rotary is the Llama prefill form");
     constexpr int QW = 16 * QT, QB = 4 * QW;
     constexpr int HDP = HD < 32 ? 32 : HD;
     constexpr int KS = HDP / 32;
@@ -78,6 +79,7 @@
     const half_t *Vb = p.V + vb_off + (int64_t)hk * HD;
 
     h8 qf[QT][KS];
+    f4 qcs[ROPE ? QT : 1][ROPE ? KS / 2 : 1][4];
 #pragma unroll
     for (int t = 0; t < QT; ++t) {
         int qr = qw + 16 * t + li;
@@ -87,6 +89,15 @@
         for (int s = 0; s < KS; ++s) {
             const int d = 32 * s + 8 * g;
             qf[t][s] = d < HD ? *reinterpret_cast<const h8 *>(src + d) : h8{0, 0, 0, 0, 0, 0, 0, 0};
+        }
+        if constexpr (ROPE) {
+            const int pos = qr > kstart ? qr - kstart : 0;
+#pragma unroll
+            for (int s = 0; s < KS / 2; ++s) {
+                const f4 *csp = reinterpret_cast<const f4 *>(p.rope_cs + ((int64_t)pos * (HD / 2) + 32 * s + 8 * g) * 2);
+#pragma unroll
+                for (int j = 0; j < 4; ++j) qcs[t][s][j] = csp[j];
+            }
         }
     }
     f4 o[QT][NO];
@@ -116,9 +127,30 @@
     const __amdgpu_buffer_rsrc_t krs = __builtin_amdgcn_make_buffer_rsrc((void *)Kb, 0, (int)(((int64_t)(T - 1) * p.k_st + HD) * 2), 0x00020000);
     const __amdgpu_buffer_rsrc_t vrs = __builtin_amdgcn_make_buffer_rsrc((void *)Vb, 0, (int)(((int64_t)(T - 1) * p.v_st + HD) * 2), 0x00020000);
     int koff[KL], voff[VL];
+    auto kpiece = [&](int u, int &r, int &c) {
+        if constexpr (ROPE) {
+            const int i = tid + 256 * (u >> 1);
+            r = i / (CH / 2);
+            c = i % (CH / 2) + (CH / 2) * (u & 1);
+        } else {
+            const int i = tid + 256 * u;
+            r = i / CH;
+            c = i % CH;
+        }
+    };
+    constexpr int NCS = ROPE ? KL / 2 : 1;
+    f4 csreg[NCS][4];
+    bool append = false;
+    half_t *kcb = nullptr, *vcb = nullptr;
+    if constexpr (ROPE) {
+        append = p.kc != nullptr && h % p.group == 0 && slot % nqb == nqb - 1;
+        kcb = p.kc + b * p.cache_sb + hk * p.cache_sh;
+        vcb = p.vc + b * p.cache_sb + hk * p.cache_sh;
+    }
 #pragma unroll
     for (int u = 0; u < KL; ++u) {
-        const int i = tid + 256 * u, r = i / CH, c = i % CH;
+        int r, c;
+        kpiece(u, r, c);
         koff[u] = c * 8 < HD ? (int)((r * p.k_st + c * 8) * 2) : 0x7ffffff0;
     }
 #pragma unroll
@@ -132,11 +164,57 @@
         for (int u = 0; u < KL; ++u) kreg[u] = __builtin_bit_cast(h8, __builtin_amdgcn_raw_buffer_load_b128(krs, koff[u] + kb, 0, 0));
 #pragma unroll
         for (int u = 0; u < VL; ++u) vreg[u] = __builtin_bit_cast(h8, __builtin_amdgcn_raw_buffer_load_b128(vrs, voff[u] + vb, 0, 0));
-    };
-    auto store_tile = [&](int buf) {
+        if constexpr (ROPE) {
+#pragma unroll
+            for (int v = 0; v < NCS; ++v) {
+                int r, c;
+                kpiece(2 * v, r, c);
+                int row = kt + r;
+                row = row < T ? row : T - 1;
+                const int pos = row > kstart ? row - kstart : 0;
+                const f4 *csp = reinterpret_cast<const f4 *>(p.rope_cs + ((int64_t)pos * (HD / 2) + c * 8) * 2);
+#pragma unroll
+                for (int j = 0; j < 4; ++j) csreg[v][j] = csp[j];
+            }
+        }
+    };
+    auto rotate_tile = [&]() {
+        if constexpr (ROPE) {
+#pragma unroll
+            for (int v = 0; v < NCS; ++v) {
+                float cs[16];
+#pragma unroll
+                for (int j = 0; j < 4; ++j) {
+                    cs[4 * j] = csreg[v][j][0]; cs[4 * j + 1] = csreg[v][j][1]; cs[4 * j + 2] = csreg[v][j][2]; cs[4 * j + 3] = csreg[v][j][3];
+                }
+                rope8_regs(kreg[2 * v], kreg[2 * v + 1], cs, 1.0f);
+            }
+        }
+    };
+    auto append_tile = [&](int kt) {
+        if constexpr (ROPE) {
+#pragma unroll
+            for (int u = 0; u < KL; ++u) {
+                int r, c;
+                kpiece(u, r, c);
+                if (kt + r < T) *reinterpret_cast<h8 *>(kcb + (kt + r) * HD + c * 8) = kreg[u];
+            }
+#pragma unroll
+            for (int u = 0; u < VL; ++u) {
+                const int i = tid + 256 * u, r = i / VC, c = i % VC;
+                if (kt + r < T) *reinterpret_cast<h8 *>(vcb + (kt + r) * HD + c * 8) = vreg[u];
+            }
+        }
+    };
+    auto store_tile = [&](int buf, int kt) {
+        if constexpr (ROPE) {
+            rotate_tile();
+            if (append) append_tile(kt);
+        }
 #pragma unroll
         for (int u = 0; u < KL; ++u) {
-            const int i = tid + 256 * u, r = i / CH, c = i % CH;
+            int r, c;
+            kpiece(u, r, c);
             *reinterpret_cast<h8 *>(&sK[buf][r * HDP + kswz<HDP>(r, c) * 8]) = kreg[u];
         }
 #pragma unroll
@@ -146,9 +224,30 @@
         }
     };
 
+    if constexpr (ROPE) {
+        if (append)
+            for (int kt = 0; kt < k_lo && kt < T; kt += KB) {
+                load_tile(kt);
+                rotate_tile();
+                append_tile(kt);
+            }
+    }
     if (k_lo < k_hi) {
         load_tile(k_lo);
-        store_tile(0);
+        if constexpr (ROPE) {
+#pragma unroll
+            for (int t = 0; t < QT; ++t)
+#pragma unroll
+                for (int s = 0; s < KS / 2; ++s) {
+                    float cs[16];
+#pragma unroll
+                    for (int j = 0; j < 4; ++j) {
+                        cs[4 * j] = qcs[t][s][j][0]; cs[4 * j + 1] = qcs[t][s][j][1]; cs[4 * j + 2] = qcs[t][s][j][2]; cs[4 * j + 3] = qcs[t][s][j][3];
+                    }
+                    rope8_regs(qf[t][s], qf[t][s + KS / 2], cs, 1.0f);
+                }
+        }
+        store_tile(0, k_lo);
         if (k_lo + KB < k_hi) load_tile(k_lo + KB);
     }
     __syncthreads();
@@ -249,7 +348,7 @@
         for (; k_hi - kt > 32; kt += KB, buf ^= 1) {
             if constexpr (LIVE) tile_body(std::integral_constant<int, 4>{}, kt, buf);
             if (kt + KB < k_hi) {
-                store_tile(buf ^ 1);
+                store_tile(buf ^ 1, kt + KB);
                 if (kt + 2 * KB < k_hi) load_tile(kt + 2 * KB);
             }
             __syncthreads();
@@ -285,6 +384,12 @@
 static hipError_t launch_qt(const AttnParams &p, hipStream_t s) {
     const int nqb = cdiv(p.T - ((p.q_trim && p.cu) ? 2 : 0), 64 * QT);
     dim3 grid(((p.B * p.heads + 7) / 8) * 8 * nqb);
+    if constexpr (HD == 128 && QT == 1) {
+        if (p.rope_cs) {
+            OPUS_LAUNCH(KC_ATTN_PREFILL, (attn_prefill_kernel<HD, true, QT, true>), grid, dim3(256), 0, s, p);
+            return hipGetLastError();
+        }
+    }
     if (p.causal) OPUS_LAUNCH(KC_ATTN_PREFILL, (attn_prefill_kernel<HD, true, QT>), grid, dim3(256), 0, s, p);
     else OPUS_LAUNCH(KC_ATTN_PREFILL, (attn_prefill_kernel<HD, false, QT>), grid, dim3(256), 0, s, p);
     return hipGetLastError();
@@ -293,6 +398,10 @@
 static hipError_t launch_hd(const AttnParams &p, hipStream_t s) {
     bool one = !(HD <= 64 && (int64_t)p.B * p.heads * cdiv(p.T, 128) >= 512);
     if (g_knobs.misc[3]) one = !one;
+    if (p.rope_cs) {
+        if (HD != 128 || !p.causal || p.cu || !p.kstart || p.kend || (p.kc != nullptr) != (p.vc != nullptr) || p.heads % p.group) return hipErrorInvalidValue;
+        one = true;
+    }
     return one ? launch_qt<HD, 1>(p, s) : launch_qt<HD, 2>(p, s);
 }
 
diff --git a/opus-pllm_amd/csrc/common.h b/opus-pllm_amd/csrc/common.h
--- a/opus-pllm_amd/csrc/common.h
+++ b/opus-pllm_amd/csrc/common.h
@@ -69,12 +69,32 @@
     hi = __builtin_fmaf(b, c, __fmul_rn(a, sn));
     asm volatile("" : "+v"(lo), "+v"(hi));
 }
+__device__ __forceinline__ float2 ln_stat_of(float s1, float s2, float inv_d, float eps, int rms) {
+    if (rms) return make_float2(0.f, rsqrtf(__builtin_fmaf(inv_d, s2, eps)));
+    const float mu = __fmul_rn(s1, inv_d);
+    const float var = fmaxf(__builtin_fmaf(-mu, mu, __fmul_rn(s2, inv_d)), 0.f);
+    return make_float2(mu, rsqrtf(__fadd_rn(var, eps)));
+}
+__device__ __forceinline__ void rope8_regs(h8 &lo, h8 &hi, const float *cs, float scale) {
+    h8 olo, ohi;
+#pragma unroll
+    for (int j = 0; j < 8; ++j) {
+        const float c = cs[2 * j], sn = cs[2 * j + 1];
+        const float a = (float)lo[j] * scale, b = (float)hi[j] * scale;
+        float rl, rh;
+        rotate_pair(a, b, c, sn, rl, rh);
+        olo[j] = (half_t)rl;
+        ohi[j] = (half_t)rh;
+    }
+    lo = olo;
+    hi = ohi;
+}
 
 __host__ __device__ __forceinline__ int64_t tiled_off(int row, int k, int K) {
     return ((int64_t)(row >> 4) * (K >> 6) + (k >> 6)) * 1024 + ((k & 63) >> 5) * 512 + ((((k & 31) >> 3) << 4) + (row & 15)) * 8 + (k & 7);
 }
 
-constexpr int HANDOFF_WORDS = 1024, HANDOFF_ERR = 1023;
+constexpr int HANDOFF_WORDS = 1024, HANDOFF_ERR = 1023, HANDOFF_LN = 768;
 constexpr int HANDOFF_SPIN_LIMIT = 1 << 19;
 
 struct GemmParams {
@@ -112,6 +132,11 @@
     int *combine_cnt = nullptr;
     float *ln_part = nullptr;
     int *ln_done = nullptr;
+    float *ln_stat_out = nullptr;
+    float ln_eps = 0.f, ln_inv_d = 0.f;
+    int ln_rms = 0;
+    int *ln_cnt = nullptr;
+    int *ln_fin_done = nullptr;
     const float *ln_stat = nullptr;
     const float *ln_colsum = nullptr;
     int pp_gm = 8;
@@ -134,6 +159,9 @@
     float scale;
     const int32_t *cu = nullptr;
     int q_trim = 0;
+    const float *rope_cs = nullptr;
+    half_t *kc = nullptr, *vc = nullptr;
+    int64_t cache_sb = 0, cache_sh = 0;
 };
 
 hipError_t launch_gemm(const GemmParams &p, hipStream_t s, int *klass);
@@ -144,6 +172,9 @@
 struct Knobs {
     int no_stream = 0;
     int no_ln_fusion = 0;
+    int ln_last_arriver = 0;
+    int keep_handoff = 0;
+    int no_rope_fusion = 0;
     int debug_a_tiled = 0;
     int pp_gm = 8;
     int enc_full_last_layer = 0;
diff --git a/opus-pllm_amd/csrc/elementwise.hip b/opus-pllm_amd/csrc/elementwise.hip
--- a/opus-pllm_amd/csrc/elementwise.hip
+++ b/opus-pllm_amd/csrc/elementwise.hip
@@ -62,18 +62,9 @@
 __device__ __forceinline__ void rope8(half_t *base, int half, const float *cs, float scale) {
     h8 lo = *reinterpret_cast<h8 *>(base);
     h8 hi = *reinterpret_cast<h8 *>(base + half);
-    h8 olo, ohi;
-#pragma unroll
-    for (int j = 0; j < 8; ++j) {
-        const float c = cs[2 * j], sn = cs[2 * j + 1];
-        const float a = (float)lo[j] * scale, b = (float)hi[j] * scale;
-        float rl, rh;
-        rotate_pair(a, b, c, sn, rl, rh);
-        olo[j] = (half_t)rl;
-        ohi[j] = (half_t)rh;
-    }
-    *reinterpret_cast<h8 *>(base) = olo;
-    *reinterpret_cast<h8 *>(base + half) = ohi;
+    rope8_regs(lo, hi, cs, scale);
+    *reinterpret_cast<h8 *>(base) = lo;
+    *reinterpret_cast<h8 *>(base + half) = hi;
 }
 
 __global__ __launch_bounds__(256) void esm_rope_kernel(half_t *__restrict__ qkv, const float *__restrict__ cs, int T,
diff --git a/opus-pllm_amd/csrc/gemm.hip b/opus-pllm_amd/csrc/gemm.hip
--- a/opus-pllm_amd/csrc/gemm.hip
+++ b/opus-pllm_amd/csrc/gemm.hip
@@ -15,6 +15,8 @@
         snprintf(name, sizeof(name), "OPUS_KNOB_MISC%d", i);
         if (const char *v = getenv(name)) k.misc[i] = atoi(v);
     }
+    k.no_rope_fusion = getenv("OPUS_NO_ROPE_FUSION") != nullptr;
+    k.ln_last_arriver = getenv("OPUS_LN_LAST_ARRIVER") != nullptr;
     return k;
 }
 Knobs g_knobs = knobs_from_env();
@@ -837,13 +839,13 @@
     tm = grp * GM + rem_id % rows_here;
     tn = rem_id / rows_here;
 }
-template <int EPI, bool LNA>
+template <int EPI, bool LNA, bool LNFIN>
 __device__ __forceinline__ void pp_finish(const GemmParams &p, f4 (&acc)[8][4], char *smem, const int wave, const int m0, const int n0,
                                           const int bid, const int full_tiles, const int tail_split, const int kpart, const bool partial);
-template <int EPI, bool LNA>
+template <int EPI, bool LNA, bool LNFIN>
 __device__ __forceinline__ void pp_epilogue(const GemmParams &p, f4 (&acc)[8][4], char *smem, const int wave, const int m0, const int n0,
                                             const char *pair_slab);
-template <int EPI, bool LNA = false>
+template <int EPI, bool LNA = false, bool LNFIN = false>
 __global__ __launch_bounds__(512) void gemm_pp_kernel(GemmParams p, int tiles_m, int tiles_n, int full_tiles, int tail_split) {
     extern __shared__ __attribute__((aligned(16))) char smem[];
     constexpr int HT = 16384;
@@ -1004,10 +1006,10 @@
     }
     if (wr == 0) __builtin_amdgcn_s_barrier();
     if (p.trace && tid == 0) p.trace[blockIdx.x * 4 + 2] = wall_clock64();
-    pp_finish<EPI, LNA>(p, acc, smem, wave, m0, n0, bid, full_tiles, tail_split, kpart, partial);
-}
-
-template <int EPI, bool LNA>
+    pp_finish<EPI, LNA, LNFIN>(p, acc, smem, wave, m0, n0, bid, full_tiles, tail_split, kpart, partial);
+}
+
+template <int EPI, bool LNA, bool LNFIN>
 __device__ __forceinline__ void pp_finish(const GemmParams &p, f4 (&acc)[8][4], char *smem, const int wave, const int m0, const int n0,
                                           const int bid, const int full_tiles, const int tail_split, const int kpart, const bool partial) {
     int lane;
@@ -1065,10 +1067,58 @@
         }
         return;
     }
-    pp_epilogue<EPI, LNA>(p, acc, smem, wave, m0, n0, pair_slab);
-}
-
-template <int EPI, bool LNA>
+    pp_epilogue<EPI, LNA, LNFIN>(p, acc, smem, wave, m0, n0, pair_slab);
+}
+
+__device__ __forceinline__ void pp_ln_finish(const GemmParams &p, char *smem, const int wave, const int m0) {
+    int lane;
+    asm volatile("v_mbcnt_lo_u32_b32 %0, -1, 0\n\tv_mbcnt_hi_u32_b32 %0, -1, %0" : "=v"(lane));
+    const int tid = wave * 64 + lane;
+    asm volatile("s_waitcnt vmcnt(0)" ::: "memory");
+    __syncthreads();
+    int *cnt = p.ln_cnt + HANDOFF_LN + (m0 >> 8);
+    int *word = reinterpret_cast<int *>(smem);
+    if (tid == 0) *word = __hip_atomic_fetch_add(cnt, 1, __ATOMIC_RELAXED, __HIP_MEMORY_SCOPE_AGENT);
+    __syncthreads();
+    const int order = *word, tiles_n = p.N >> 8;
+    if (order != tiles_n - 1) {
+        if (order >= tiles_n && tid == 0) __hip_atomic_store(p.ln_cnt + HANDOFF_ERR, 1, __ATOMIC_RELAXED, __HIP_MEMORY_SCOPE_AGENT);
+        return;
+    }
+    if (tid == 0) __hip_atomic_store(cnt, 0, __ATOMIC_RELAXED, __HIP_MEMORY_SCOPE_AGENT);
+    const int nslab = p.N >> 6, rows_left = p.M - m0 < 256 ? p.M - m0 : 256;
+    const __amdgpu_buffer_rsrc_t prs = __builtin_amdgcn_make_buffer_rsrc(
+        reinterpret_cast<char *>(p.ln_part) + (int64_t)m0 * nslab * 8, 0, (int)((int64_t)rows_left * nslab * 8), 0x00020000);
+    const int q = tid & 15, r0 = tid >> 4;
+    float s1[8], s2[8];
+#pragma unroll
+    for (int ps = 0; ps < 8; ++ps) s1[ps] = s2[ps] = 0.f;
+    for (int j0 = 0; j0 < nslab; j0 += 64) {
+        float2 t[8][4];
+#pragma unroll
+        for (int ps = 0; ps < 8; ++ps)
+#pragma unroll
+            for (int u = 0; u < 4; ++u) {
+                const int j = j0 + 16 * u + q;
+                const int off = j < nslab ? ((ps * 32 + r0) * nslab + j) * 8 : 0x7ffffff0;
+                t[ps][u] = __builtin_bit_cast(float2, __builtin_amdgcn_raw_buffer_load_b64(prs, off, 0, 16));
+            }
+#pragma unroll
+        for (int ps = 0; ps < 8; ++ps) {
+            s1[ps] += (t[ps][0].x + t[ps][1].x) + (t[ps][2].x + t[ps][3].x);
+            s2[ps] += (t[ps][0].y + t[ps][1].y) + (t[ps][2].y + t[ps][3].y);
+        }
+    }
+#pragma unroll
+    for (int ps = 0; ps < 8; ++ps) {
+#pragma unroll
+        for (int o = 1; o < 16; o <<= 1) { s1[ps] += __shfl_xor(s1[ps], o, 64); s2[ps] += __shfl_xor(s2[ps], o, 64); }
+        const int r = ps * 32 + r0;
+        if (q == 0 && r < rows_left) reinterpret_cast<float2 *>(p.ln_stat_out)[m0 + r] = ln_stat_of(s1[ps], s2[ps], p.ln_inv_d, p.ln_eps, p.ln_rms);
+    }
+}
+
+template <int EPI, bool LNA, bool LNFIN>
 __device__ __forceinline__ void pp_epilogue(const GemmParams &p, f4 (&acc)[8][4], char *smem, const int wave, const int m0, const int n0,
                                             const char *pair_slab) {
     int lane;
@@ -1322,7 +1372,7 @@
                             for (int o = 1; o < LPR32; o <<= 1) { s1 += __shfl_xor(s1, o, 64); s2 += __shfl_xor(s2, o, 64); }
                             const float2 st = make_float2(s1, s2);
                             const int poff = (lane % LPR32) == 0 ? ((tr0 + r) * (p.N >> 6) + (nw0 >> 6)) * 8 : 0x7ffffff0;
-                            __builtin_amdgcn_raw_buffer_store_b64(__builtin_bit_cast(u2v, st), prs, poff, 0, 0);
+                            __builtin_amdgcn_raw_buffer_store_b64(__builtin_bit_cast(u2v, st), prs, poff, 0, LNFIN ? 16 : 0);
                         }
                     }
                 } else if (CS || (MODE == M_GENERIC && rope_on)) {
@@ -1387,6 +1437,7 @@
         } else if (p.out_f32 && p.residual && p.ln_part) {
             if (pair_slab) run(std::integral_constant<int, M_F32RES_LN>{}, WP{});
             else run(std::integral_constant<int, M_F32RES_LN>{}, NP{});
+            if constexpr (LNFIN) pp_ln_finish(p, smem, wave, m0);
         } else if (p.out_f32 && p.residual) {
             if (pair_slab) run(std::integral_constant<int, M_F32RES>{}, WP{});
             else run(std::integral_constant<int, M_F32RES>{}, NP{});
@@ -1525,7 +1576,7 @@
     const int T = bm * bn, KT = p.K >> 6;
     int full = T, split = 1;
     static const bool no_tail = getenv("OPUS_NO_PP_TAIL") != nullptr;
-    static const bool no_rope_fuse = getenv("OPUS_NO_ROPE_FUSION") != nullptr;
+    const bool no_rope_fuse = g_knobs.no_rope_fusion != 0;
     const bool rope = p.rope_cs && p.rope_done && !no_rope_fuse && EPI == EPI_NONE && !p.out_f32 && !p.residual && (p.ldc & 7) == 0 &&
                       (p.N & 255) == 0 && (p.rope_cols & 63) == 0 && (p.rope_qcols & 63) == 0 && p.rope_T > 0;
     if (rope) *p.rope_done = 1;
@@ -1570,6 +1621,15 @@
     const bool pair_mode = (!p.out_f32 && !p.residual) || (EPI == EPI_NONE && p.out_f32 && p.residual);
     const bool pair = split == 2 && p.combine_cnt && !g_knobs.misc[6] && pair_mode && (p.ldc & 7) == 0 && (p.ldr & 3) == 0 && (p.N & 255) == 0;
     if (!pair) p.combine_cnt = nullptr;
+    const bool lnfin = EPI == EPI_NONE && !lna && lnp && p.ln_stat_out && p.ln_cnt && p.ln_fin_done && g_knobs.ln_last_arriver &&
+                       (split == 1 || pair) && bm <= HANDOFF_ERR - HANDOFF_LN && (int64_t)256 * (p.N >> 6) * 8 < (1ll << 31);
+    if (lnfin) {
+        *p.ln_fin_done = 1;
+        p.ln_inv_d = 1.0f / (float)p.N;
+        if constexpr (EPI == EPI_NONE) kern = gemm_pp_kernel<EPI_NONE, false, true>;
+        ea = ensure_dyn_lds(reinterpret_cast<const void *>(kern), 8 * 16384);
+        if (ea != hipSuccess) return ea;
+    } else p.ln_stat_out = nullptr;
     if (p.pp_plan) {
         p.pp_plan[0] = full; p.pp_plan[1] = tail; p.pp_plan[2] = split;
         p.pp_plan[3] = split == 1 ? PP_TAIL_NONE : pair ? PP_TAIL_PAIR : PP_TAIL_REDUCE;
diff --git a/opus-pllm_amd/csrc/norm.hip b/opus-pllm_amd/csrc/norm.hip
--- a/opus-pllm_amd/csrc/norm.hip
+++ b/opus-pllm_amd/csrc/norm.hip
@@ -114,13 +114,7 @@
 #pragma unroll
     for (int o = 1; o < 16; o <<= 1) { s1 += __shfl_xor(s1, o, 64); s2 += __shfl_xor(s2, o, 64); }
     if (!live || q) return;
-    if (rms) {
-        stat[m] = make_float2(0.f, rsqrtf(s2 * inv_d + eps));
-        return;
-    }
-    const float mu = s1 * inv_d;
-    const float var = fmaxf(s2 * inv_d - mu * mu, 0.f);
-    stat[m] = make_float2(mu, rsqrtf(var + eps));
+    stat[m] = ln_stat_of(s1, s2, inv_d, eps, rms);
 }
 hipError_t launch_ln_finalize(const float *part, int64_t rows, int nslab, int D, float eps, int rms, float *stat, hipStream_t s) {
     hipLaunchKernelGGL(ln_finalize_kernel, dim3(cdiv(rows, 16)), dim3(256), 0, s, reinterpret_cast<const float2 *>(part), rows, nslab,
```
